# matthewygf/Tiresias

Measured on AMD Instinct MI355X. Metric: avg JCT + makespan on NSDI'19 Microsoft trace, 8×MI355X cluster, lower is better.
Workload: dtype bf16

## Files before the change

### csrc/bindings/ops.cpp

```cpp
#include <array>
#include <ATen/ATen.h>
#include <c10/hip/HIPStream.h>
#include <torch/library.h>

#include <functional>
#include <map>
#include <mutex>
#include <sstream>
#include <tuple>
#include <vector>

#include "tam/kernels.h"
#include "tam/launch.h"
#include "tam/gemm8p.h"

using at::Tensor;
using c10::optional;

namespace {

hipStream_t cur_stream(const Tensor& t) {
  return c10::hip::getCurrentHIPStream(t.device().index()).stream();
}

// ... 287 lines not shown
      t[0] = std::min(t[0], time_ms(s, [&] { run_mfma(a, a_kmajor, b, b_kmajor, M, N, K, es, allow_split, 0); }));
      for (const auto& c : cands) {
        const float ms = time_ms(s, [&] { run_p8(a, a_kmajor, b, b_kmajor, M, N, K, es, allow_split, c.first,
                                                 c.second); });
        if (ms < t[3]) { t[3] = ms; p8c = c; }
      }
      if (dma_ok)
        t[2] = std::min(t[2], time_ms(s, [&] { run_mfma(a, a_kmajor, b, b_kmajor, M, N, K, es, allow_split, 2); }));
      if (lib_ok && round == 0) {
        try {
          t[1] = time_ms(s, [&] { run_lib(a, a_kmajor, b, b_kmajor, scratch, mode, bias); });
        } catch (const std::exception&) {
          t[1] = 1e30f;
        }
      }
    }
    route = 0;
    if (t[2] < 0.95f * t[route]) route = 2;
    if (t[3] < 0.95f * t[route]) route = 3;
    if (t[1] < 0.95f * t[route]) route = 1;
    std::lock_guard<std::mutex> g(g_route_mu);
    g_route[key] = route;
    g_route_ms[key] = t;
    g_p8_cfg[key] = p8c;
  }
  if (route == 1 && !lib_ok) {
    std::lock_guard<std::mutex> g(g_route_mu);
    const auto t = g_route_ms[key];
    route = 0;
    if (dma_ok && t[2] < t[route]) route = 2;
    auto pc = g_p8_cfg.find(key);
    if (p8_ok && pc != g_p8_cfg.end() && pc->second.first > 0 && t[3] < t[route]) route = 3;
  }
  std::pair<int, int> p8c{-1, -1};
  if (route == 3) {
    std::lock_guard<std::mutex> g(g_route_mu);
    auto it = g_p8_cfg.find(key);
    if (it != g_p8_cfg.end()) p8c = it->second;
  }
  if (route == 1) run_lib(a, a_kmajor, b, b_kmajor, c, mode, bias);
  else if (route == 3) run_p8(a, a_kmajor, b, b_kmajor, M, N, K, ep, allow_split, p8c.first, p8c.second);
  else run_mfma(a, a_kmajor, b, b_kmajor, M, N, K, ep, allow_split, route);
}

void gemm_lib_policy_op(int64_t p) { g_lib_policy = (int)p; }

std::string gemm_routes_op() {
  std::lock_guard<std::mutex> g(g_route_mu);
  std::ostringstream o;
  for (const auto& kv : g_route) {
    const auto& k = kv.first;
    const auto t = g_route_ms[k];
    o << std::get<0>(k) << " " << std::get<1>(k) << " " << std::get<2>(k) << " "
      << (std::get<3>(k) ? "K" : "M") << (std::get<4>(k) ? "K" : "N") << " " << std::get<5>(k)
      << " " << std::get<6>(k) << " " << std::get<7>(k) << " "
      << (kv.second == 1 ? "lib" : kv.second == 2 ? "dma" : kv.second == 3 ? "p8" : "mfma") << " " << t[0]
      << " " << t[1] << " " << t[2] << " " << t[3];
    auto pc = g_p8_cfg.find(k);
    if (pc != g_p8_cfg.end()) o << " " << pc->second.first << " " << pc->second.second;
    o << "\n";
  }
  return o.str();
}

int64_t gemm_routes_load_op(const std::string& text) {
  std::istringstream in(text);
  std::string line;
  int64_t n = 0;
  std::lock_guard<std::mutex> g(g_route_mu);
  while (std::getline(in, line)) {
    std::istringstream ls(line);
    int64_t M, N, K, mode;
    std::string lay, rt;
    int f32, epi;
    std::array<float, 4> t{};
    if (!(ls >> M >> N >> K >> lay >> mode >> f32 >> epi >> rt >> t[0] >> t[1] >> t[2] >> t[3])) continue;
    if (lay.size() != 2 || M <= 0 || N <= 0 || K <= 0) continue;
    const int route = rt == "lib" ? 1 : rt == "dma" ? 2 : rt == "p8" ? 3 : rt == "mfma" ? 0 : -1;
    if (route < 0) continue;
    const GemmKey key{M, N, K, lay[0] == 'K', lay[1] == 'K', mode, (bool)f32, (bool)epi};
    if (g_route.count(key)) continue;
    int tile = -1, sp = -1;
    const bool has_cfg = (bool)(ls >> tile >> sp);
    const bool cfg_ok = has_cfg &&
                        (tile == 128 || tile == 256 || ((tile == 64 || tile == 65 || tile == 129) && lay[0] == 'K')) &&
                        sp >= (tile == 256 ? 0 : 1) && sp <= 16;
    if (route == 3 && !cfg_ok) continue;
    g_route[key] = route;
    g_route_ms[key] = t;
    if (cfg_ok) g_p8_cfg[key] = {tile, sp};
    ++n;
  }
  return n;
}

tam::ConvGeom geom(const Tensor& x, const Tensor& w, const Tensor& y, int64_t stride, int64_t pad,
                   int64_t dil) {
  tam::ConvGeom g;
  g.N = (int)x.size(0); g.H = (int)x.size(1); g.W = (int)x.size(2); g.C = (int)x.size(3);
  g.K = (int)w.size(0); g.R = (int)w.size(1); g.S = (int)w.size(2);
  g.P = (int)y.size(1); g.Q = (int)y.size(2);
  g.stride = (int)stride; g.pad = (int)pad; g.dil = (int)dil;
  TORCH_CHECK(w.size(3) == g.C, "tam.conv: weight C mismatch");
  TORCH_CHECK(y.size(0) == g.N && y.size(3) == g.K, "tam.conv: output shape mismatch");
  TORCH_CHECK(g.P == (g.H + 2 * g.pad - g.dil * (g.R - 1) - 1) / g.stride + 1 &&
                  g.Q == (g.W + 2 * g.pad - g.dil * (g.S - 1) - 1) / g.stride + 1,
              "tam.conv: output spatial size inconsistent with geometry");
  TORCH_CHECK(g.C % 8 == 0 && g.K % 8 == 0, "tam.conv: C and K must be multiples of 8");
  return g;
}

int64_t conv_fwd_op(const Tensor& x, const Tensor& w, const Tensor& y, int64_t stride, int64_t pad,
                    int64_t dil, const optional<Tensor>& bias, bool relu, const optional<Tensor>& stats) {
  check_bf16(x, "x"); check_bf16(w, "w"); check_bf16(y, "y");
  check_contig(x, "x"); check_contig(w, "w"); check_contig(y, "y");
  tam::ConvGeom g = geom(x, w, y, stride, pad, dil);
  tam::Epi ep;
  ep.c = y.data_ptr(); ep.ldc = g.K; ep.c_f32 = 0; ep.mode = 0;
  ep.bias = opt_ptr<const tam::bf16_t>(bias);
  ep.relu = relu;
  if (stats.has_value() && stats->defined()) {
    TORCH_CHECK(stats->is_cuda() && stats->scalar_type() == at::kDouble && stats->is_contiguous() &&
                stats->numel() == tam::BN_SHARDS * 2 * g.K,
                "tam.conv_fwd: stats must be a contiguous fp64 [BN_SHARDS * 2K] tensor");
    ep.stats = stats->data_ptr<double>();
  }
  const long wsf = tam::conv_fwd_split_ws(g);
  Tensor ws;
  if (wsf > 0) ws = at::empty({wsf}, x.options().dtype(at::kFloat));
  return tam::conv_fwd(bp(x), bp(w), g, ep, cur_stream(x), wsf > 0 ? ws.data_ptr<float>() : nullptr, wsf);
}

void conv_dgrad_op(const Tensor& dy, const Tensor& w, const Tensor& wt, const Tensor& dx,
                   int64_t stride, int64_t pad, int64_t dil, const optional<Tensor>& mask) {
  check_bf16(dy, "dy"); check_bf16(w, "w"); check_bf16(dx, "dx");
  check_contig(dy, "dy"); check_contig(w, "w"); check_contig(dx, "dx");
  tam::ConvGeom g = geom(dx, w, dy, stride, pad, dil);
  check_bf16(wt, "wt");
  TORCH_CHECK(wt.numel() == w.numel(), "tam.conv_dgrad: wt workspace size");
  tam::conv_weight_t(bp(w), bpm(wt), g, cur_stream(dy));
  tam::Epi ep;
  ep.c = dx.data_ptr(); ep.ldc = g.C; ep.c_f32 = 0; ep.mode = 0;
  if (mask.has_value() && mask->defined()) {
    check_bf16(*mask, "mask");
    TORCH_CHECK(mask->numel() == dx.numel(), "tam.conv_dgrad: mask size");
    ep.mask = bp(*mask); ep.ldm = g.C;
  }
  const long wsf = tam::conv_dgrad_split_ws(g);
  Tensor ws;
  if (wsf > 0) ws = at::empty({wsf}, dy.options().dtype(at::kFloat));
  tam::conv_dgrad(bp(dy), bp(w), bp(wt), g, ep, cur_stream(dy), wsf > 0 ? ws.data_ptr<float>() : nullptr, wsf);
}

void gemm_wgrad_grouped_op(at::TensorList dy, at::TensorList x, at::TensorList dw, at::TensorList db,
                           at::OptionalIntArrayRef modes) {
  TORCH_CHECK(dy.size() == x.size() && dy.size() == dw.size() && dy.size() == db.size(),
              "tam.gemm_wgrad_grouped: list sizes differ");
  TORCH_CHECK(!modes.has_value() || modes->size() == dy.size(), "tam.gemm_wgrad_grouped: modes size");
  if (dy.empty()) return;
  std::vector<tam::GGProblem> probs(dy.size());
  for (size_t i = 0; i < dy.size(); ++i) {
    const Tensor& a = dy[i];
    const Tensor& b = x[i];
    const Tensor& c = dw[i];
    check_bf16(a, "dy"); check_bf16(b, "x"); check_f32(c, "dw");
    check_contig(a, "dy"); check_contig(b, "x"); check_contig(c, "dw");
    TORCH_CHECK(a.dim() == 2 && b.dim() == 2 && c.dim() == 2 && a.size(0) == b.size(0) &&
                    c.size(0) == a.size(1) && c.size(1) == b.size(1),
                "tam.gemm_wgrad_grouped: shapes dy [T,M], x [T,N], dw [M,N] expected");
    TORCH_CHECK(a.device() == dy[0].device() && b.device() == a.device() && c.device() == a.device(),
                "tam.gemm_wgrad_grouped: all operands on one device");
    const int M = (int)a.size(1), N = (int)b.size(1), K = (int)a.size(0);
    TORCH_CHECK(tam::gemm_wgrad_grouped_ok(M, N, K, M, N),
                "tam.gemm_wgrad_grouped: problem ", i, " (", M, "x", N, "x", K,
                ") not eligible (K % 64, M/N >= 128 and % 8)");
    float* bias = nullptr;
    if (db[i].defined() && db[i].numel() > 0) {
      check_f32(db[i], "db");
      TORCH_CHECK(db[i].numel() == M && db[i].is_contiguous(), "tam.gemm_wgrad_grouped: db must be [M]");
      bias = db[i].data_ptr<float>();
    }
    const int mode = modes.has_value() ? (int)(*modes)[i] : 1;
    TORCH_CHECK(mode == 0 || mode == 1, "tam.gemm_wgrad_grouped: mode must be 0 (store) or 1 (accumulate)");
    probs[i] = tam::GGProblem{bp(a), bp(b), c.data_ptr<float>(), bias, M, N, K, M, N, mode};
  }
  tam::gemm_wgrad_grouped(probs.data(), (int)probs.size(), cur_stream(dy[0]));
}

void gemm_grouped_tile_op(int64_t t) { tam::gemm_grouped_tile((int)t); }

bool gemm_wgrad_grouped_ok_op(int64_t M, int64_t N, int64_t K) {
  return tam::gemm_wgrad_grouped_ok((int)M, (int)N, (int)K, M, N);
}

void conv_weight_t_batch_op(at::TensorList w, at::TensorList wt) {
  TORCH_CHECK(w.size() == wt.size(), "tam.conv_weight_t_batch: list sizes differ");
  if (w.empty()) return;
  hipStream_t st = cur_stream(w[0]);
  for (size_t base = 0; base < w.size(); base += tam::WT_MAX) {
    tam::WTBatch b{};
    b.n = (int)std::min<size_t>(tam::WT_MAX, w.size() - base);
    for (int i = 0; i < b.n; ++i) {
      const Tensor& a = w[base + i];
      const Tensor& t = wt[base + i];
      check_bf16(a, "w"); check_bf16(t, "wt"); check_contig(a, "w"); check_contig(t, "wt");
      TORCH_CHECK(a.dim() == 4 && t.numel() == a.numel(), "tam.conv_weight_t_batch: w must be [K,R,S,C]");
      b.e[i].w = bp(a); b.e[i].wt = bpm(t);
      b.e[i].K = (int)a.size(0); b.e[i].RS = (int)(a.size(1) * a.size(2)); b.e[i].C = (int)a.size(3);
    }
    tam::conv_weight_t_batch(b, st);
  }
}

int64_t conv_dgrad_pre_op(const Tensor& dy, const Tensor& w, const Tensor& wt, const Tensor& dx,
                          int64_t stride, int64_t pad, int64_t dil, const optional<Tensor>& mask,
                          const optional<Tensor>& stats, const optional<Tensor>& bnx,
                          const optional<Tensor>& bnmean, const optional<Tensor>& bnrstd) {
  check_bf16(dy, "dy"); check_bf16(w, "w"); check_bf16(dx, "dx"); check_bf16(wt, "wt");
  check_contig(dy, "dy"); check_contig(w, "w"); check_contig(dx, "dx"); check_contig(wt, "wt");
  TORCH_CHECK(wt.numel() == w.numel(), "tam.conv_dgrad_pre: wt size");
  tam::ConvGeom g = geom(dx, w, dy, stride, pad, dil);
  tam::Epi ep;
  ep.c = dx.data_ptr(); ep.ldc = g.C; ep.c_f32 = 0; ep.mode = 0;
  if (mask.has_value() && mask->defined()) {
    check_bf16(*mask, "mask");
    TORCH_CHECK(mask->numel() == dx.numel(), "tam.conv_dgrad_pre: mask size");
    ep.mask = bp(*mask); ep.ldm = g.C;
  }
  if (stats.has_value() && stats->defined()) {
    TORCH_CHECK(bnx.has_value() && bnmean.has_value() && bnrstd.has_value(),
                "tam.conv_dgrad_pre: stats needs bnx, bnmean, bnrstd");
    check_bf16(*bnx, "bnx"); check_f32(*bnmean, "bnmean"); check_f32(*bnrstd, "bnrstd");
    check_contig(*bnx, "bnx");
    TORCH_CHECK(stats->is_cuda() && stats->scalar_type() == at::kDouble && stats->is_contiguous() &&
                stats->numel() == tam::BN_SHARDS * 2 * g.C && bnx->numel() == dx.numel() && bnmean->numel() == g.C &&
                bnrstd->numel() == g.C, "tam.conv_dgrad_pre: BN-backward operand shapes");
    ep.stats = stats->data_ptr<double>();
    ep.bnx = bp(*bnx);
    ep.bnmean = bnmean->data_ptr<float>();
    ep.bnrstd = bnrstd->data_ptr<float>();
  }
  const long wsf = ep.bnx ? 0 : tam::conv_dgrad_split_ws(g);
  Tensor ws;
  if (wsf > 0) ws = at::empty({wsf}, dy.options().dtype(at::kFloat));
  return tam::conv_dgrad(bp(dy), bp(w), bp(wt), g, ep, cur_stream(dy), wsf > 0 ? ws.data_ptr<float>() : nullptr,
                         wsf);
}

std::tuple<Tensor, int64_t> conv_wgrad_deferred_op(const Tensor& dy, const Tensor& x, const Tensor& dw,
                                                   int64_t stride, int64_t pad, int64_t dil, int64_t mode,
                                                   const optional<Tensor>& dbias, bool patch) {
  check_bf16(dy, "dy"); check_bf16(x, "x"); check_f32(dw, "dw");
  check_contig(dy, "dy"); check_contig(x, "x"); check_contig(dw, "dw");
  TORCH_CHECK(dw.dim() == 4, "tam.conv_wgrad_deferred: dw must be [K,R,S,C]");
  tam::ConvGeom g = geom(x, dw, dy, stride, pad, dil);
  tam::Epi ep;
  ep.c = dw.data_ptr(); ep.ldc = g.R * g.S * g.C; ep.c_f32 = 1; ep.mode = (int)mode;
  float* db = nullptr;
  if (dbias.has_value() && dbias->defined()) {
    check_f32(*dbias, "dbias");
    TORCH_CHECK(dbias->numel() == g.K && dbias->is_contiguous(), "tam.conv_wgrad_deferred: dbias size");
    db = dbias->data_ptr<float>();
  }
  const long wsf = tam::conv_wgrad_split_ws(g);
  Tensor wsl = at::empty({wsf > 0 ? wsf : 0}, dy.options().dtype(at::kFloat));
  int sp = 0;
  const int fused = tam::conv_wgrad(bp(dy), bp(x), g, ep, cur_stream(dy), db, patch,
                                    wsf > 0 ? wsl.data_ptr<float>() : nullptr, wsf, &sp);
  if (db && !fused) {
    const long R = (long)g.N * g.P * g.Q;
    Tensor ws = at::empty({g.K % 8 == 0 ? (int64_t)tam::COLSUM_MAX_BLOCKS * g.K : 1}, dy.options().dtype(at::kFloat));
    tam::colsum(bp(dy), db, ws.data_ptr<float>(), R, g.K, cur_stream(dy));
  }
  return {sp > 0 ? wsl : at::empty({0}, dy.options().dtype(at::kFloat)), (int64_t)sp};
}

void wgrad_slab_reduce_many_op(at::TensorList slabs, at::IntArrayRef sp, at::TensorList dw, at::IntArrayRef mode) {
  const size_t n = slabs.size();
  TORCH_CHECK(sp.size() == n && dw.size() == n && mode.size() == n, "tam.wgrad_slab_reduce_many: list sizes");
  if (n == 0) return;
  std::vector<const float*> ws(n);
  std::vector<float*> out(n);
  std::vector<int> s(n), md(n);
  std::vector<long> mn(n);
  for (size_t i = 0; i < n; ++i) {
    check_f32(slabs[i], "slab"); check_f32(dw[i], "dw");
    TORCH_CHECK(dw[i].is_contiguous() && dw[i].numel() % 4 == 0 && sp[i] > 0 &&
                    slabs[i].numel() >= sp[i] * dw[i].numel(),
                "tam.wgrad_slab_reduce_many: entry ", i);
    ws[i] = slabs[i].data_ptr<float>();
    out[i] = dw[i].data_ptr<float>();
    s[i] = (int)sp[i];
    md[i] = (int)mode[i];
    mn[i] = (long)dw[i].numel();
  }
  tam::wgrad_slab_reduce_many(ws.data(), s.data(), mn.data(), out.data(), md.data(), (int)n, cur_stream(dw[0]));
}

void conv_wgrad_op(const Tensor& dy, const Tensor& x, const Tensor& dw, int64_t stride, int64_t pad,
                   int64_t dil, int64_t mode, const optional<Tensor>& dbias, bool patch) {
  check_bf16(dy, "dy"); check_bf16(x, "x"); check_f32(dw, "dw");
  check_contig(dy, "dy"); check_contig(x, "x"); check_contig(dw, "dw");
  TORCH_CHECK(dw.dim() == 4, "tam.conv_wgrad: dw must be [K,R,S,C]");
  tam::ConvGeom g = geom(x, dw, dy, stride, pad, dil);
  tam::Epi ep;
  ep.c = dw.data_ptr(); ep.ldc = g.R * g.S * g.C; ep.c_f32 = 1; ep.mode = (int)mode;
  float* db = nullptr;
  if (dbias.has_value() && dbias->defined()) {
    check_f32(*dbias, "dbias");
    TORCH_CHECK(dbias->numel() == g.K && dbias->is_contiguous(), "tam.conv_wgrad: dbias size");
    db = dbias->data_ptr<float>();
  }
  const long wsf = tam::conv_wgrad_split_ws(g);
  Tensor wsl;
  if (wsf > 0) wsl = at::empty({wsf}, dy.options().dtype(at::kFloat));
  const int fused = tam::conv_wgrad(bp(dy), bp(x), g, ep, cur_stream(dy), db, patch,
                                    wsf > 0 ? wsl.data_ptr<float>() : nullptr, wsf);
  if (db && !fused) {
    const long R = (long)g.N * g.P * g.Q;
    Tensor ws = at::empty({g.K % 8 == 0 ? (int64_t)tam::COLSUM_MAX_BLOCKS * g.K : 1}, dy.options().dtype(at::kFloat));
    tam::colsum(bp(dy), db, ws.data_ptr<float>(), R, g.K, cur_stream(dy));
  }
}

static double* bn_sums(const optional<Tensor>& sums, const Tensor& x, int64_t C, Tensor& tmp,
                       const char* what) {
  if (sums.has_value() && sums->defined()) {
    TORCH_CHECK(sums->is_cuda() && sums->scalar_type() == at::kDouble && sums->is_contiguous() &&
                sums->numel() == tam::BN_SHARDS * 2 * C, what,
                ": sums must be a contiguous fp64 [BN_SHARDS * 2C] tensor");
    return sums->data_ptr<double>();
  }
  tmp = at::zeros({tam::BN_SHARDS * 2 * C}, x.options().dtype(at::kDouble));
  return tmp.data_ptr<double>();
}

void bn_forward_op(const Tensor& x, const optional<Tensor>& res, const Tensor& y, const Tensor& gamma,
                   const Tensor& beta, const optional<Tensor>& run_mean,
                   const optional<Tensor>& run_var, const Tensor& save_mean,
// ... 196 lines not shown
  TORCH_CHECK(tm_b <= 0 || ids.numel() % tm_b == 0, "tam.embedding: tm_b must divide the ids");
  const tam::bf16_t* pp = nullptr;
  int64_t prow = 0;
  if (pos.has_value() && pos->defined()) {
    check_bf16(*pos, "pos"); check_contig(*pos, "pos");
    TORCH_CHECK(pos->dim() == 2 && pos->size(1) == D, "tam.embedding: pos must be [S][D]");
    prow = pos->size(0);
    TORCH_CHECK(prow > 0 && (tm_b > 0 ? ids.numel() / tm_b == prow : ids.numel() % prow == 0),
                "tam.embedding: pos rows must equal the sequence length");
    pp = bp(*pos);
  }
  tam::embedding_forward(bp(table), ids.data_ptr<int64_t>(), bpm(out), ids.numel(), (int)D,
                         (float)scale, cur_stream(table), table.size(0), tm_b, pp, prow);
}
void embedding_backward_op(const Tensor& dout, const Tensor& ids, const Tensor& gtable, double scale, int64_t tm_b) {
  check_bf16(dout, "dout"); check_f32(gtable, "gtable"); check_contig(dout, "dout");
  TORCH_CHECK(ids.scalar_type() == at::kLong && ids.is_contiguous() && gtable.dim() == 2 &&
                  dout.numel() == ids.numel() * gtable.size(1), "tam.embedding_backward: shapes");
  TORCH_CHECK(tm_b <= 0 || ids.numel() % tm_b == 0, "tam.embedding_backward: tm_b must divide the ids");
  tam::embedding_backward(bp(dout), ids.data_ptr<int64_t>(), gtable.data_ptr<float>(), ids.numel(),
                          (int)gtable.size(1), (float)scale, cur_stream(dout), gtable.size(0), tm_b);
}

void conv_dma_policy_op(int64_t p) { tam::conv_dma_policy((int)p); }
void conv_halo_policy_op(int64_t p) { tam::conv_halo_policy((int)p); }
void colsum_policy_op(int64_t p) { tam::colsum_policy((int)p); }
void attn_short_policy_op(int64_t p) { tam::attn_short_policy((int)p); }
void conv_wgrad_c64_policy_op(int64_t p) { tam::conv_wgrad_c64_policy((int)p); }
void conv_wgrad_order_op(int64_t p) { tam::conv_wgrad_order((int)p); }
void conv_stem_policy_op(int64_t p) { tam::conv_stem_policy((int)p); }
void conv_wgrad_slab_policy_op(int64_t p) { tam::conv_wgrad_slab_policy((int)p); }
void conv_wgrad_force_op(int64_t bm, int64_t bn, int64_t splits, int64_t noatomic) {
  tam::conv_wgrad_force((int)bm, (int)bn, (int)splits, (int)noatomic);
}
int g_dma_policy = 1;
TAM_KNOB(g_dma_policy)
void gemm_dma_policy_op(int64_t p, int64_t cfg) {
  g_dma_policy = (int)p;
  tam::gemm_dma_policy(p == 2 ? 1 : 0, (int)cfg);
}

void gemm8p_policy_op(int64_t mode, int64_t tile) { tam::gemm8p_policy((int)mode, (int)tile); }
void gemm_pw_policy_op(int64_t on) { tam::gemm_pw_policy((int)on); }

std::string policy_names_op() {
  std::string out;
  for (const auto& k : tam::knob_registry()) {
    if (!out.empty()) out += ",";
    out += k.name;
  }
  return out;
}
std::vector<int64_t> policy_state_op() {
  std::vector<int64_t> v;
  for (const auto& k : tam::knob_registry()) v.push_back(*k.p);
  return v;
}
void policy_load_op(std::vector<int64_t> v) {
  auto& reg = tam::knob_registry();
  TORCH_CHECK(v.size() == reg.size(), "policy_load: ", v.size(), " values for ", reg.size(), " knobs");
  for (size_t i = 0; i < reg.size(); ++i) *reg[i].p = (int)v[i];
}
void gemm8p_group_op(int64_t g) { tam::gemm8p_group((int)g); }
void gemm8p_slab_force_op(int64_t sp) { tam::gemm8p_slab_force((int)sp); }
void gemm8p_sk_force_op(int64_t on) { g_sk_force = on != 0; }
void conv_split_policy_op(int64_t p) { tam::conv_split_policy((int)p); }
void optim_grid_op(int64_t b) { tam::optim_grid((int)b); }
void optim_variant_op(int64_t v) { tam::optim_variant((int)v); }
void gemm_skinny_policy_op(int64_t on, int64_t sp, int64_t nst) {
  tam::gemm_skinny_policy((int)on, (int)sp, (int)nst);
}

void gemm_force_op(int64_t cfg, int64_t splits) {
  tam::gemm_force((int)cfg, (int)splits);
  g_forced = cfg >= 0 || splits >= 1;
}

void colsum_op(const Tensor& x, const Tensor& out) {
  check_bf16(x, "x"); check_f32(out, "out"); check_contig(x, "x");
  const int64_t C = x.size(-1);
  Tensor ws = at::empty({C % 8 == 0 ? (int64_t)tam::COLSUM_MAX_BLOCKS * C : 1},
                        x.options().dtype(at::kFloat));
  tam::colsum(bp(x), out.data_ptr<float>(), ws.data_ptr<float>(), x.numel() / C, (int)C,
              cur_stream(x));
}
void relu_backward_op(const Tensor& dy, const Tensor& y, const Tensor& dx) {
  check_bf16(dy, "dy"); check_bf16(y, "y"); check_bf16(dx, "dx");
  tam::relu_backward(bp(dy), bp(y), bpm(dx), dy.numel(), cur_stream(dy));
}
void sum_scale_op(const Tensor& x, const Tensor& out, double scale) {
  check_f32(x, "x"); check_f32(out, "out"); check_contig(x, "x");
  TORCH_CHECK(out.numel() >= 1, "tam.sum_scale: out");
  tam::sum_scale(x.data_ptr<float>(), x.numel(), out.data_ptr<float>(), (float)scale, cur_stream(x));
}
static std::pair<int64_t, int64_t> row_view(const Tensor& t, const char* what) {
  TORCH_CHECK(t.is_cuda() && t.scalar_type() == at::kBFloat16 && t.dim() >= 1 && t.stride(-1) == 1,
              "tam.rows_sum: ", what, " must be a bf16 CUDA tensor with unit last stride");
  const int64_t C = t.size(-1);
  int64_t ld = t.dim() >= 2 ? t.stride(-2) : C;
  for (int64_t d = t.dim() - 2; d >= 1; --d)
    TORCH_CHECK(t.size(d) == 1 || t.size(d - 1) == 1 || t.stride(d - 1) == t.stride(d) * t.size(d),
                "tam.rows_sum: ", what, " leading dims do not collapse to one row pitch");
  TORCH_CHECK(C % 8 == 0 && ld % 8 == 0 && (((uintptr_t)t.data_ptr()) & 15) == 0,
              "tam.rows_sum: ", what, " needs C % 8 == 0 and 16-B aligned rows");
  return {C, ld};
}
void rows_sum_op(at::TensorList outs, at::TensorList ins, at::IntArrayRef n_in) {
  TORCH_CHECK(!outs.empty() && outs.size() <= 4 && outs.size() == n_in.size(), "tam.rows_sum: 1-4 jobs");
  const int64_t R = outs[0].numel() / outs[0].size(-1);
  tam::RowJobs jb{};
  size_t q = 0;
  for (size_t j = 0; j < outs.size(); ++j) {
    auto [C, ld] = row_view(outs[j], "out");
    TORCH_CHECK(outs[j].numel() / C == R, "tam.rows_sum: every job needs the same row count");
    TORCH_CHECK(n_in[j] >= 1 && n_in[j] <= 4 && q + n_in[j] <= ins.size(), "tam.rows_sum: n_in");
    tam::RowJob& r = jb.job[j];
    r.out = bpm(outs[j]); r.ld_out = ld; r.C = (int)C; r.n_in = (int)n_in[j];
    for (int k = 0; k < r.n_in; ++k, ++q) {
      auto [Ci, ldi] = row_view(ins[q], "in");
      TORCH_CHECK(Ci == C && ins[q].numel() / Ci == R, "tam.rows_sum: input shape");
      r.in[k] = bp(ins[q]); r.ld_in[k] = ldi;
    }
  }
  TORCH_CHECK(q == ins.size(), "tam.rows_sum: unused inputs");
  tam::rows_sum(jb, (int)outs.size(), R, cur_stream(outs[0]));
}
void zero_op(const Tensor& t) {
  TORCH_CHECK(t.is_cuda() && t.is_contiguous(), "tam.zero_: contiguous CUDA tensor");
  tam::zero_async(t.data_ptr(), t.numel() * t.element_size(), cur_stream(t));
}
void add_op(const Tensor& a, const Tensor& b, const Tensor& y) {
  check_bf16(a, "a"); check_bf16(b, "b"); check_bf16(y, "y");
  TORCH_CHECK(a.numel() % 8 == 0, "tam.add: numel % 8");
  tam::add_bf16(bp(a), bp(b), bpm(y), a.numel(), cur_stream(a));
}
void cast_op(const Tensor& x, const Tensor& y) {
  check_f32(x, "x"); check_bf16(y, "y");
  tam::cast_f32_bf16(x.data_ptr<float>(), bpm(y), x.numel(), cur_stream(x));
}

static const unsigned* guard_ptr(const optional<Tensor>& guard, const Tensor& like) {
  if (!(guard.has_value() && guard->defined())) return nullptr;
  TORCH_CHECK(guard->scalar_type() == at::kInt && guard->numel() >= 2 && guard->device() == like.device(),
              "tam: guard must be an int32 [2] tensor on the parameters' device");
  return (const unsigned*)guard->data_ptr<int>();
}
static const float* clip_ptr(const optional<Tensor>& clip, const Tensor& like) {
  if (!(clip.has_value() && clip->defined())) return nullptr;
  TORCH_CHECK(clip->scalar_type() == at::kFloat && clip->numel() >= 4 && clip->is_contiguous() &&
                  clip->device() == like.device() && (((uintptr_t)clip->data_ptr()) & 15) == 0,
              "tam: clip must be a 16-B aligned float32 [4] tensor on the parameters' device");
  return clip->data_ptr<float>();
}
void sgd_op(const Tensor& w, const Tensor& g, const Tensor& mom, const Tensor& wb, double lr,
            double momentum, double wd, double gscale, bool nesterov, bool zero_grad,
            const optional<Tensor>& guard, int64_t zero_from, int64_t wd_until,
            const optional<Tensor>& clip) {
  check_f32(w, "w"); check_f32(g, "g"); check_f32(mom, "mom"); check_bf16(wb, "wb");
  TORCH_CHECK(w.numel() % 4 == 0 && g.numel() == w.numel() && mom.numel() == w.numel() &&
                  wb.numel() == w.numel(),
              "tam.sgd: sizes");
  TORCH_CHECK(zero_from % 4 == 0 && (wd_until < 0 || wd_until % 4 == 0), "tam.sgd: region bounds % 4");
  tam::sgd_step(w.data_ptr<float>(), g.data_ptr<float>(), mom.data_ptr<float>(), bpm(wb), w.numel(),
                (float)lr, (float)momentum, (float)wd, (float)gscale, nesterov, zero_grad,
                cur_stream(w), guard_ptr(guard, w), (long)zero_from, (long)wd_until, clip_ptr(clip, w));
}
void adam_op(const Tensor& w, const Tensor& g, const Tensor& m, const Tensor& v, const Tensor& wb,
             double lr, double b1, double b2, double eps, double wd, int64_t step, double gscale,
             bool zero_grad, const optional<Tensor>& guard, int64_t zero_from, int64_t wd_until,
             const optional<Tensor>& clip) {
  check_f32(w, "w"); check_f32(g, "g"); check_f32(m, "m"); check_f32(v, "v"); check_bf16(wb, "wb");
  TORCH_CHECK(w.numel() % 4 == 0, "tam.adam: numel % 4");
  TORCH_CHECK(zero_from % 4 == 0 && (wd_until < 0 || wd_until % 4 == 0), "tam.adam: region bounds % 4");
  tam::adam_step(w.data_ptr<float>(), g.data_ptr<float>(), m.data_ptr<float>(), v.data_ptr<float>(),
                 bpm(wb), w.numel(), (float)lr, (float)b1, (float)b2, (float)eps, (float)wd,
                 (int)step, (float)gscale, zero_grad, cur_stream(w), guard_ptr(guard, w), (long)zero_from,
                 (long)wd_until, clip_ptr(clip, w));
}
void grad_sumsq_op(const Tensor& g, const Tensor& partials) {
  check_f32(g, "g"); check_contig(g, "g"); check_dev(partials, "partials"); check_contig(partials, "partials");
  TORCH_CHECK(partials.scalar_type() == at::kDouble && partials.device() == g.device(),
              "tam.grad_sumsq: partials must be float64 on the gradient's device");
  TORCH_CHECK(g.numel() % 4 == 0 && (((uintptr_t)g.data_ptr()) & 15) == 0,
              "tam.grad_sumsq: numel % 4 and a 16-B aligned gradient");
  const int blocks = tam::grad_sumsq_blocks(g.numel());
  TORCH_CHECK(partials.numel() >= blocks && partials.numel() <= (1 << 20), "tam.grad_sumsq: partials holds ",
              partials.numel(), " slots, the grid needs ", blocks);
  tam::grad_sumsq(g.data_ptr<float>(), g.numel(), partials.data_ptr<double>(), (int)partials.numel(),
                  cur_stream(g));
}
void grad_clip_finalize_op(const Tensor& partials, double max_norm, double gscale, const Tensor& clip) {
  check_dev(partials, "partials"); check_contig(partials, "partials"); check_f32(clip, "clip");
  TORCH_CHECK(partials.scalar_type() == at::kDouble && partials.numel() >= 1 && partials.numel() <= (1 << 20),
              "tam.grad_clip_finalize: partials must be a float64 tensor of the grad_sumsq slots");
  TORCH_CHECK(max_norm > 0.0, "tam.grad_clip_finalize: max_norm must be > 0");
  tam::grad_clip_finalize(partials.data_ptr<double>(), (int)partials.numel(), (float)max_norm, (float)gscale,
                          const_cast<float*>(clip_ptr(clip, partials)), cur_stream(partials));
}
int64_t grad_sumsq_blocks_op(int64_t n) { return tam::grad_sumsq_blocks((long)n); }
void lstm_guard_step_op(const Tensor& err) {
  TORCH_CHECK(err.is_cuda() && err.scalar_type() == at::kInt && err.numel() >= 2,
              "tam.lstm_guard_step: err must be an int32 [2] GPU tensor");
  tam::lstm_guard_step((unsigned*)err.data_ptr<int>(), cur_stream(err));
}

void check_attn_view(const Tensor& t, const char* name) {
  check_bf16(t, name);
  TORCH_CHECK(t.dim() == 4 && t.size(3) == 64 && t.stride(3) == 1 && t.stride(2) == 64,
              "tam.attn: ", name, " must be a [B,S,H,64] view with packed heads");
  TORCH_CHECK(t.stride(1) % 8 == 0 && t.stride(0) % 8 == 0, "tam.attn: ", name, " stride alignment");
}
void attn_forward_op(const Tensor& q, const Tensor& k, const Tensor& v, const Tensor& o,
                     const Tensor& lse, bool causal, double scale, const optional<Tensor>& kv_len) {
  check_attn_view(q, "q"); check_attn_view(k, "k"); check_attn_view(v, "v"); check_attn_view(o, "o");
  TORCH_CHECK(k.stride(1) == v.stride(1), "tam.attn: k/v token strides differ");
  check_f32(lse, "lse");
  const int B = (int)q.size(0), Sq = (int)q.size(1), H = (int)q.size(2), Sk = (int)k.size(1);
  TORCH_CHECK(lse.numel() == (int64_t)B * H * Sq, "tam.attn: lse size");
  TORCH_CHECK(k.stride(0) == v.stride(0), "tam.attn: k/v batch strides differ");
  tam::attn_forward(bp(q), bp(k), bp(v), bpm(o), lse.data_ptr<float>(), B, H, Sq, Sk, q.stride(1),
                    k.stride(1), o.stride(1), q.stride(0), k.stride(0), o.stride(0), causal, (float)scale,
                    opt_ptr<const int>(kv_len), cur_stream(q));
}
void attn_backward_op(const Tensor& q, const Tensor& k, const Tensor& v, const Tensor& o,
                      const Tensor& dout, const Tensor& lse, const Tensor& dq, const Tensor& dk,
                      const Tensor& dv, const Tensor& dq_acc, const Tensor& delta, bool causal,
                      double scale, const optional<Tensor>& kv_len) {
  check_attn_view(q, "q"); check_attn_view(k, "k"); check_attn_view(v, "v"); check_attn_view(o, "o");
  check_attn_view(dout, "dout"); check_attn_view(dq, "dq"); check_attn_view(dk, "dk");
  check_attn_view(dv, "dv");
  TORCH_CHECK(dout.stride(1) == o.stride(1) && dout.stride(0) == o.stride(0), "tam.attn_bwd: dout must match o layout");
  TORCH_CHECK(dq.stride(1) == q.stride(1) && dk.stride(1) == k.stride(1) && dv.stride(1) == k.stride(1) &&
                  dq.stride(0) == q.stride(0) && dk.stride(0) == k.stride(0) && dv.stride(0) == k.stride(0) &&
                  v.stride(0) == k.stride(0) && v.stride(1) == k.stride(1),
              "tam.attn_bwd: grads must match input layouts");
  const int B = (int)q.size(0), Sq = (int)q.size(1), H = (int)q.size(2), Sk = (int)k.size(1);
  check_f32(dq_acc, "dq_acc"); check_f32(delta, "delta");
  TORCH_CHECK(dq_acc.numel() >= (int64_t)B * Sq * H * 64 && delta.numel() >= (int64_t)B * H * Sq,
              "tam.attn_bwd: workspace sizes");
  tam::attn_backward(bp(q), bp(k), bp(v), bp(o), bp(dout), lse.data_ptr<float>(), bpm(dq), bpm(dk),
                     bpm(dv), dq_acc.data_ptr<float>(), delta.data_ptr<float>(), B, H, Sq, Sk,
                     q.stride(1), k.stride(1), o.stride(1), q.stride(0), k.stride(0), o.stride(0), causal,
                     (float)scale,
                     opt_ptr<const int>(kv_len), cur_stream(q));
}

void lstm_fwd_op(const Tensor& gates, const optional<Tensor>& c_prev, const Tensor& c_out,
                 const Tensor& h_out, const optional<Tensor>& h_f32, const Tensor& act) {
  check_f32(gates, "gates"); check_f32(c_out, "c_out"); check_bf16(h_out, "h_out"); check_f32(act, "act");
  const int B = (int)gates.size(0), Hd = (int)(gates.size(1) / 4);
  tam::lstm_cell_forward(gates.data_ptr<float>(), opt_ptr<const float>(c_prev), c_out.data_ptr<float>(),
                         bpm(h_out), opt_ptr<float>(h_f32), act.data_ptr<float>(), B, Hd,
                         cur_stream(gates));
}
void lstm_step_fwd_op(const Tensor& gx, const Tensor& w_hh, const optional<Tensor>& h_prev,
                      const optional<Tensor>& c_prev, const Tensor& c_out, const Tensor& h_out,
                      const Tensor& act) {
  check_f32(gx, "gx"); check_bf16(w_hh, "w_hh"); check_f32(c_out, "c_out"); check_bf16(h_out, "h_out");
  check_f32(act, "act");
  const int64_t B = gx.size(0), Hd = w_hh.size(1);
  TORCH_CHECK(gx.dim() == 2 && gx.size(1) == 4 * Hd && gx.stride(1) == 1 && gx.stride(0) == 4 * Hd,
              "tam.lstm_step_forward: gx must be contiguous [B][4*Hd]");
  TORCH_CHECK(w_hh.is_contiguous() && w_hh.size(0) == 4 * Hd, "tam.lstm_step_forward: w_hh [4Hd][Hd]");
  TORCH_CHECK(B % 16 == 0 && Hd % 256 == 0, "tam.lstm_step_forward: needs B % 16 == 0, Hd % 256 == 0");
  TORCH_CHECK(c_out.numel() == B * Hd && h_out.numel() == B * Hd && act.numel() == 5 * B * Hd &&
              c_out.is_contiguous() && h_out.is_contiguous() && act.is_contiguous(),
              "tam.lstm_step_forward: output shapes");
  if (h_prev.has_value() && h_prev->defined()) {
    check_bf16(*h_prev, "h_prev");
    TORCH_CHECK(h_prev->is_contiguous() && h_prev->numel() == B * Hd, "tam.lstm_step_forward: h_prev");
  }
  if (c_prev.has_value() && c_prev->defined()) {
    check_f32(*c_prev, "c_prev");
    TORCH_CHECK(c_prev->is_contiguous() && c_prev->numel() == B * Hd, "tam.lstm_step_forward: c_prev");
  }
  tam::lstm_step_forward(gx.data_ptr<float>(), bp(w_hh), opt_ptr<const tam::bf16_t>(h_prev),
                         opt_ptr<const float>(c_prev), c_out.data_ptr<float>(), bpm(h_out),
                         act.data_ptr<float>(), (int)B, (int)Hd, cur_stream(gx));
}

static void check_sync(const Tensor& sync, int64_t B) {
  TORCH_CHECK(sync.is_cuda() && sync.scalar_type() == at::kInt && sync.is_contiguous() &&
              sync.numel() >= 32 * (4 * (B / 16) + 1),
              "tam.lstm_seq: sync must be a contiguous int32 tensor of >= 32 * (4 * B/16 + 1) elements");
}
static tam::PLOpts pl_opts(const optional<Tensor>& job_err, int64_t grids, int64_t rsv, bool zeroed) {
  tam::PLOpts o;
  o.grids = (int)grids;
  o.rsv = (int)rsv;
  o.zeroed = zeroed ? 1 : 0;
  if (job_err.has_value() && job_err->defined()) {
    TORCH_CHECK(job_err->is_cuda() && job_err->scalar_type() == at::kInt && job_err->numel() >= 2,
                "tam.lstm_seq: job_err must be an int32 [2] GPU tensor");
    o.job_err = (unsigned*)job_err->data_ptr<int>();
  }
  return o;
}
bool lstm_seq_fwd_op(const Tensor& gx, const Tensor& w_hh, const Tensor& hs, const Tensor& cs,
                     const Tensor& act, bool reverse, const Tensor& sync, const optional<Tensor>& job_err,
                     int64_t grids, int64_t rsv, bool zeroed) {
  check_f32(gx, "gx"); check_bf16(w_hh, "w_hh"); check_bf16(hs, "hs"); check_f32(cs, "cs");
  check_f32(act, "act");
  TORCH_CHECK(hs.dim() == 3 && hs.is_contiguous(), "tam.lstm_seq_forward: hs [T][B][Hd]");
  const int64_t T = hs.size(0), B = hs.size(1), Hd = hs.size(2);
  check_sync(sync, B);
  TORCH_CHECK(w_hh.is_contiguous() && w_hh.size(0) == 4 * Hd && w_hh.size(1) == Hd,
              "tam.lstm_seq_forward: w_hh [4Hd][Hd]");
  TORCH_CHECK(gx.is_contiguous() && gx.numel() == T * B * 4 * Hd, "tam.lstm_seq_forward: gx [T][B][4Hd]");
  TORCH_CHECK(cs.is_contiguous() && cs.numel() == T * B * Hd && act.is_contiguous() &&
              act.numel() == T * B * 5 * Hd, "tam.lstm_seq_forward: cs / act shapes");
  int* sp = sync.data_ptr<int>();
  return tam::lstm_seq_forward(gx.data_ptr<float>(), bp(w_hh), bpm(hs), cs.data_ptr<float>(),
                               act.data_ptr<float>(), (int)T, (int)B, (int)Hd, reverse ? 1 : 0,
                               (unsigned*)sp, cur_stream(gx), pl_opts(job_err, grids, rsv, zeroed));
}
bool lstm_seq_bwd_op(const Tensor& act, const Tensor& cs, const Tensor& dH, const Tensor& w_hh,
                     const Tensor& dG, bool reverse, const Tensor& sync, const optional<Tensor>& job_err,
                     int64_t grids, int64_t rsv, bool zeroed) {
  check_f32(act, "act"); check_f32(cs, "cs"); check_bf16(w_hh, "w_hh");
  TORCH_CHECK(dH.is_cuda() && (dH.scalar_type() == at::kFloat || dH.scalar_type() == at::kBFloat16),
              "tam.lstm_seq_backward: dH must be an f32 or bf16 CUDA tensor");
  const int dh_bf16 = dH.scalar_type() == at::kBFloat16 ? 1 : 0;
  check_bf16(dG, "dG");
  TORCH_CHECK(cs.dim() == 3 && cs.is_contiguous(), "tam.lstm_seq_backward: cs [T][B][Hd]");
  const int64_t T = cs.size(0), B = cs.size(1), Hd = cs.size(2);
  check_sync(sync, B);
  TORCH_CHECK(w_hh.is_contiguous() && w_hh.size(0) == 4 * Hd && w_hh.size(1) == Hd,
              "tam.lstm_seq_backward: w_hh [4Hd][Hd]");
  TORCH_CHECK(dH.dim() == 3 && dH.size(0) == T && dH.size(1) == B && dH.size(2) == Hd && dH.stride(2) == 1 &&
                  dH.stride(1) >= Hd && dH.stride(0) == B * dH.stride(1),
              "tam.lstm_seq_backward: dH [T][B][Hd] with unit column stride and uniform row pitch");
  TORCH_CHECK(act.is_contiguous() && act.numel() == T * B * 5 * Hd && dG.is_contiguous() &&
                  dG.numel() == T * B * 4 * Hd,
              "tam.lstm_seq_backward: act / dG shapes");
  int* sp = sync.data_ptr<int>();
  return tam::lstm_seq_backward(act.data_ptr<float>(), cs.data_ptr<float>(), (const float*)dH.data_ptr(),
                                bp(w_hh), bpm(dG), (int)T, (int)B, (int)Hd, reverse ? 1 : 0, (unsigned*)sp,
                                dh_bf16, (int)dH.stride(1), cur_stream(act), pl_opts(job_err, grids, rsv, zeroed));
}

void lstm_seq_policy_op(int64_t ch) { tam::lstm_seq_policy((int)ch); }
void lstm_seq_shards_op(int64_t ns) { tam::lstm_seq_shards((int)ns); }
void lstm_seq_residency_op(int64_t grids, int64_t rsv) { tam::lstm_seq_residency((int)grids, (int)rsv); }
int64_t lstm_persist_timeouts_op(bool reset) { return tam::lstm_persist_timeouts(reset); }
void lstm_seq_spin_limit_op(int64_t polls) { tam::lstm_seq_spin_limit(polls); }

void lstm_bwd_op(const Tensor& act, const optional<Tensor>& c_prev, const optional<Tensor>& dh,
                 const optional<Tensor>& dc_next, const optional<Tensor>& dgates,
                 const optional<Tensor>& dc_prev, const optional<Tensor>& dgates_bf16) {
  check_f32(act, "act");
  const int B = (int)act.size(0), Hd = (int)(act.size(1) / 5);
  tam::lstm_cell_backward(act.data_ptr<float>(), opt_ptr<const float>(c_prev), nullptr,
                          opt_ptr<const float>(dh), opt_ptr<const float>(dc_next),
                          opt_ptr<float>(dgates), opt_ptr<float>(dc_prev),
                          opt_ptr<tam::bf16_t>(dgates_bf16), B, Hd, c10::hip::getCurrentHIPStream(act.device().index()).stream());
}

}

TORCH_LIBRARY(tam, m) {
  m.def("gemm(Tensor a, bool a_kmajor, Tensor b, bool b_kmajor, Tensor(a!) c, int mode, Tensor? bias, bool relu, Tensor? mask, float alpha, bool allow_split, Tensor(b!)? colsum=None) -> ()", &gemm_op);
  m.def("conv_fwd(Tensor x, Tensor w, Tensor(a!) y, int stride, int pad, int dil, Tensor? bias, bool relu, Tensor(b!)? stats=None) -> int", &conv_fwd_op);
  m.def("conv_dgrad(Tensor dy, Tensor w, Tensor(a!) wt, Tensor(b!) dx, int stride, int pad, int dil, Tensor? mask) -> ()", &conv_dgrad_op);
  m.def("conv_weight_t_batch(Tensor[] w, Tensor(a!)[] wt) -> ()", &conv_weight_t_batch_op);
  m.def("gemm_wgrad_grouped(Tensor[] dy, Tensor[] x, Tensor(a!)[] dw, Tensor(b!)[] db, int[]? modes=None) -> ()", &gemm_wgrad_grouped_op);
  m.def("gemm_wgrad_grouped_ok(int M, int N, int K) -> bool", &gemm_wgrad_grouped_ok_op);
  m.def("gemm_grouped_tile(int tile) -> ()", &gemm_grouped_tile_op);
  m.def("conv_dgrad_pre(Tensor dy, Tensor w, Tensor wt, Tensor(a!) dx, int stride, int pad, int dil, Tensor? mask, Tensor(b!)? stats=None, Tensor? bnx=None, Tensor? bnmean=None, Tensor? bnrstd=None) -> int", &conv_dgrad_pre_op);
  m.def("conv_wgrad(Tensor dy, Tensor x, Tensor(a!) dw, int stride, int pad, int dil, int mode, Tensor(b!)? dbias=None, bool patch=True) -> ()", &conv_wgrad_op);
  m.def("conv_wgrad_deferred(Tensor dy, Tensor x, Tensor(a!) dw, int stride, int pad, int dil, int mode, Tensor(b!)? dbias, bool patch) -> (Tensor, int)", &conv_wgrad_deferred_op);
  m.def("wgrad_slab_reduce_many(Tensor[] slabs, int[] sp, Tensor(a!)[] dw, int[] mode) -> ()", &wgrad_slab_reduce_many_op);
  m.def("bn_forward(Tensor x, Tensor? res, Tensor(a!) y, Tensor gamma, Tensor beta, Tensor(b!)? run_mean, Tensor(c!)? run_var, Tensor(d!) save_mean, Tensor(e!) save_rstd, float eps, float momentum, bool relu, Tensor(f!)? sums=None, bool sums_ready=False, Tensor(g!)? ymask=None) -> ()", &bn_forward_op);
  m.def("bn_backward(Tensor dy, Tensor? y, Tensor x, Tensor mean, Tensor rstd, Tensor gamma, Tensor(a!) dx, Tensor(b!)? dres, Tensor(c!)? dgamma, Tensor(d!)? dbeta, bool relu, Tensor? addend=None, Tensor(e!)? sums=None, bool sums_ready=False, Tensor? ymask=None) -> ()", &bn_backward_op);
  m.def("ln_forward(Tensor x, Tensor g, Tensor b, Tensor(a!) y, Tensor(b!) mean, Tensor(c!) rstd, float eps, Tensor? addend=None, Tensor(d!)? sum_out=None) -> ()", &ln_forward_op);
  m.def("ln_backward(Tensor dy, Tensor x, Tensor g, Tensor mean, Tensor rstd, Tensor(a!) dx, Tensor(b!) dg, Tensor(c!) db, Tensor? addend=None) -> ()", &ln_backward_op);
  m.def("ln_backward_split(Tensor dy, Tensor x, Tensor g, Tensor mean, Tensor rstd, Tensor(a!) dx, Tensor(b!) ws, Tensor? addend=None) -> int", &ln_backward_split_op);
  m.def("col_reduce_acc(Tensor part, int nblk, int W, Tensor(a!) out0, Tensor(b!) out1, int split) -> ()", &col_reduce_acc_op);
  m.def("col_reduce_acc_batch(Tensor[] parts, int[] nblk, Tensor(a!)[] out0, Tensor(b!)[] out1) -> ()", &col_reduce_acc_batch_op);
  m.def("maxpool_forward(Tensor x, Tensor(a!) y, Tensor(b!) idx, int R, int S, int stride, int pad) -> ()", &maxpool_forward_op);
  m.def("maxpool_backward(Tensor dy, Tensor idx, Tensor(a!) dx, int R, int S, int stride, int pad) -> ()", &maxpool_backward_op);
  m.def("maxpool_k3s2_policy(int policy) -> ()", &maxpool_k3s2_policy_op);
  m.def("avgpool_forward(Tensor x, Tensor(a!) y) -> ()", &avgpool_forward_op);
  m.def("avgpool_backward(Tensor dy, Tensor(a!) dx) -> ()", &avgpool_backward_op);
  m.def("softmax_xent(Tensor logits, Tensor labels, Tensor(a!)? dlogits, Tensor(b!) loss_rows, float smoothing, float grad_scale, int ignore_index, int tm_b=0) -> ()", &softmax_xent_op);
  m.def("embedding_forward(Tensor table, Tensor ids, Tensor(a!) out, float scale, int tm_b=0, Tensor? pos=None) -> ()", &embedding_forward_op);
  m.def("embedding_backward(Tensor dout, Tensor ids, Tensor(a!) gtable, float scale, int tm_b=0) -> ()", &embedding_backward_op);
  m.def("sum_scale(Tensor x, Tensor(a!) out, float scale) -> ()", &sum_scale_op);
  m.def("rows_sum(Tensor[] outs, Tensor[] ins, int[] n_in) -> ()", &rows_sum_op);
  m.def("zero_(Tensor(a!) t) -> ()", &zero_op);
  m.def("colsum(Tensor x, Tensor(a!) out) -> ()", &colsum_op);
  m.def("gemm_force(int cfg, int splits) -> ()", &gemm_force_op);
  m.def("gemm8p_policy(int mode, int tile) -> ()", &gemm8p_policy_op);
  m.def("gemm_pw_policy(int on) -> ()", &gemm_pw_policy_op);
  m.def("policy_names() -> str", &policy_names_op);
  m.def("policy_state() -> int[]", &policy_state_op);
  m.def("policy_load(int[] v) -> ()", &policy_load_op);
  m.def("gemm8p_group(int g) -> ()", &gemm8p_group_op);
  m.def("gemm8p_slab_force(int sp) -> ()", &gemm8p_slab_force_op);
  m.def("gemm_skinny_policy(int on, int force_splits, int nst) -> ()", &gemm_skinny_policy_op);
  m.def("gemm8p_sk_force(int on) -> ()", &gemm8p_sk_force_op);
  m.def("conv_split_policy(int p) -> ()", &conv_split_policy_op);
  m.def("optim_variant(int v) -> ()", &optim_variant_op);
  m.def("optim_grid(int blocks) -> ()", &optim_grid_op);
  m.def("gemm_lib_policy(int policy) -> ()", &gemm_lib_policy_op);
  m.def("conv_dma_policy(int policy) -> ()", &conv_dma_policy_op);
  m.def("conv_wgrad_force(int bm, int bn, int splits, int noatomic=0) -> ()", &conv_wgrad_force_op);
  m.def("conv_wgrad_c64_policy(int policy) -> ()", &conv_wgrad_c64_policy_op);
  m.def("conv_wgrad_order(int flat) -> ()", &conv_wgrad_order_op);
  m.def("conv_stem_policy(int policy) -> ()", &conv_stem_policy_op);
  m.def("conv_wgrad_slab_policy(int policy) -> ()", &conv_wgrad_slab_policy_op);
  m.def("conv_halo_policy(int policy) -> ()", &conv_halo_policy_op);
  m.def("colsum_policy(int policy) -> ()", &colsum_policy_op);
  m.def("attn_short_policy(int policy) -> ()", &attn_short_policy_op);
  m.def("gemm_dma_policy(int policy, int cfg) -> ()", &gemm_dma_policy_op);
  m.def("gemm_routes() -> str", &gemm_routes_op);
  m.def("relu_backward(Tensor dy, Tensor y, Tensor(a!) dx) -> ()", &relu_backward_op);
  m.def("add(Tensor a, Tensor b, Tensor(a!) y) -> ()", &add_op);
  m.def("cast_f32_bf16(Tensor x, Tensor(a!) y) -> ()", &cast_op);
  m.def("sgd_step(Tensor(a!) w, Tensor(b!) g, Tensor(c!) mom, Tensor(d!) wb, float lr, float momentum, float wd, float gscale, bool nesterov, bool zero_grad, Tensor? guard=None, int zero_from=0, int wd_until=-1, Tensor? clip=None) -> ()", &sgd_op);
  m.def("adam_step(Tensor(a!) w, Tensor(b!) g, Tensor(c!) m, Tensor(d!) v, Tensor(e!) wb, float lr, float b1, float b2, float eps, float wd, int step, float gscale, bool zero_grad, Tensor? guard=None, int zero_from=0, int wd_until=-1, Tensor? clip=None) -> ()", &adam_op);
  m.def("grad_sumsq(Tensor g, Tensor(a!) partials) -> ()", &grad_sumsq_op);
  m.def("grad_clip_finalize(Tensor partials, float max_norm, float gscale, Tensor(a!) clip) -> ()", &grad_clip_finalize_op);
  m.def("grad_sumsq_blocks(int n) -> int", &grad_sumsq_blocks_op);
  m.def("lstm_guard_step(Tensor(a!) err) -> ()", &lstm_guard_step_op);
  m.def("attn_forward(Tensor q, Tensor k, Tensor v, Tensor(a!) o, Tensor(b!) lse, bool causal, float scale, Tensor? kv_len) -> ()", &attn_forward_op);
  m.def("attn_backward(Tensor q, Tensor k, Tensor v, Tensor o, Tensor dout, Tensor lse, Tensor(a!) dq, Tensor(b!) dk, Tensor(c!) dv, Tensor(d!) dq_acc, Tensor(e!) delta, bool causal, float scale, Tensor? kv_len) -> ()", &attn_backward_op);
  m.def("lstm_step_forward(Tensor gx, Tensor w_hh, Tensor? h_prev, Tensor? c_prev, Tensor(a!) c_out, Tensor(b!) h_out, Tensor(c!) act) -> ()", &lstm_step_fwd_op);
  m.def("lstm_seq_forward(Tensor gx, Tensor w_hh, Tensor(a!) hs, Tensor(b!) cs, Tensor(c!) act, bool reverse, Tensor(d!) sync, Tensor(e!)? job_err=None, int grids=-1, int reserved_cus=0, bool zeroed=False) -> bool", &lstm_seq_fwd_op);
  m.def("lstm_seq_backward(Tensor act, Tensor cs, Tensor dH, Tensor w_hh, Tensor(a!) dG, bool reverse, Tensor(b!) sync, Tensor(c!)? job_err=None, int grids=-1, int reserved_cus=0, bool zeroed=False) -> bool", &lstm_seq_bwd_op);
  m.def("lstm_seq_policy(int ch) -> ()", &lstm_seq_policy_op);
  m.def("lstm_seq_shards(int ns) -> ()", &lstm_seq_shards_op);
  m.def("gemm_routes_load(str text) -> int", &gemm_routes_load_op);
  m.def("lstm_seq_residency(int grids, int reserved_cus) -> ()", &lstm_seq_residency_op);
  m.def("lstm_persist_timeouts(bool reset) -> int", &lstm_persist_timeouts_op);
  m.def("lstm_seq_spin_limit(int polls) -> ()", &lstm_seq_spin_limit_op);
  m.def("lstm_cell_forward(Tensor gates, Tensor? c_prev, Tensor(a!) c_out, Tensor(b!) h_out, Tensor(c!)? h_f32, Tensor(d!) act) -> ()", &lstm_fwd_op);
  m.def("lstm_cell_backward(Tensor act, Tensor? c_prev, Tensor? dh, Tensor? dc_next, Tensor(a!)? dgates, Tensor(b!)? dc_prev, Tensor(c!)? dgates_bf16) -> ()", &lstm_bwd_op);
}
```

### csrc/include/tam/gemm8p.h

```cpp
#pragma once
#include "tam/igemm.h"

namespace tam {

constexpr int P8_BK = 64;

typedef __attribute__((address_space(3))) void p8_lds_t;

struct P8Args {
  const bf16_t* A;
  long lda;
  const bf16_t* B;
  long ldb;
  int M, N, K;
  int kps;
  int group = 4;
};

template <int BM, int BN, int WNW>
struct P8Geo {
  static constexpr int NW = 2 * WNW, THREADS = 64 * NW;
  static constexpr int WTM = BM / 2, WTN = BN / WNW;
  static constexpr int QM = WTM / 2, QN = WTN / 2;
  static constexpr int FI = QM / 16, FJ = QN / 16;
  static constexpr int AROWS = BM / 2, BCOLS = BN / 2;
  static constexpr int AHALF = AROWS * P8_BK * 2, BHALF = BCOLS * P8_BK * 2;
  static constexpr int STAGE = 2 * AHALF + 2 * BHALF;
  static constexpr int LDS = 2 * STAGE;
  static constexpr int DA = AHALF / (THREADS * 16), DB = BHALF / (THREADS * 16);
  static_assert(DA >= 1 && DB >= 1 && AHALF == THREADS * 16 * DA && BHALF == THREADS * 16 * DB,
                "whole DMA instructions per half");
  static constexpr int INFLIGHT = DA + 2 * DB;
};

template <int N>
__device__ __forceinline__ void p8_vmcnt() {
  static_assert(N >= 0 && N <= 8, "p8_vmcnt: 0..8");
  if constexpr (N == 0) asm volatile("s_waitcnt vmcnt(0)" ::: "memory");
  else if constexpr (N == 1) asm volatile("s_waitcnt vmcnt(1)" ::: "memory");
  else if constexpr (N == 2) asm volatile("s_waitcnt vmcnt(2)" ::: "memory");
  else if constexpr (N == 3) asm volatile("s_waitcnt vmcnt(3)" ::: "memory");
  else if constexpr (N == 4) asm volatile("s_waitcnt vmcnt(4)" ::: "memory");
  else if constexpr (N == 5) asm volatile("s_waitcnt vmcnt(5)" ::: "memory");
  else if constexpr (N == 6) asm volatile("s_waitcnt vmcnt(6)" ::: "memory");
  else if constexpr (N == 7) asm volatile("s_waitcnt vmcnt(7)" ::: "memory");
  else asm volatile("s_waitcnt vmcnt(8)" ::: "memory");
}

template <int Q>
__device__ __forceinline__ int p8_row(int lr, int h) {
  return (lr / Q) * (2 * Q) + h * Q + (lr % Q);
}

template <int Q, int EXT, int NW, bool KMAJ, int D = 2>
__device__ __forceinline__ void p8_issue(const bf16_t* __restrict__ base, long ld, int extent, int o0,
                                         int k0, char* half, int h, int wid, int lane) {
#pragma unroll
  for (int j = 0; j < D; ++j) {
    const int g = j * NW + wid;
    if constexpr (KMAJ) {
      const int lr = g * 8 + (lane >> 3);
      const int c = (lane & 7) ^ ((lr >> 1) & 7);
      int r = o0 + p8_row<Q>(lr, h);
      r = r < extent ? r : extent - 1;
      const bf16_t* src = base + (long)r * ld + k0 + c * 8;
      __builtin_amdgcn_global_load_lds((const void*)src, (p8_lds_t*)(half + g * 1024), 16, 0, 0);
    } else {
      constexpr int GPR = EXT / 8, RPG = 64 / GPR;
      const int kr = g * RPG + lane / GPR;
      const int gran = (lane % GPR) ^ (mnmaj_swz<EXT>(kr) >> 1);
      int col = o0 + p8_row<Q>(gran * 8, h);
      col = col + 8 <= extent ? col : extent - 8;
      const bf16_t* src = base + (long)(k0 + kr) * ld + col;
      __builtin_amdgcn_global_load_lds((const void*)src, (p8_lds_t*)(half + g * 1024), 16, 0, 0);
    }
  }
}

template <bool KMAJ, int EXT>
__device__ __forceinline__ s16x8_t p8_frag(const char* half, int lane, int lbase, int kk) {
  if constexpr (KMAJ) return read_frag_k(half, lane, lbase, kk);
  else return read_frag_mn<EXT>(half, lane, 32 * kk, lbase);
}

__device__ __forceinline__ void p8_barrier() {
  asm volatile("" ::: "memory");
  __builtin_amdgcn_s_barrier();
  asm volatile("" ::: "memory");
}

template <int I0, int J0, bool FINE = false, int FI, int FJ, int TI, int TJ>
__device__ __forceinline__ void p8_mfma(f32x4_t (&acc)[TI][TJ], const s16x8_t (&fa)[FI][2],
                                        const s16x8_t (&fb)[FJ][2]) {
  if constexpr (!FINE) {
    asm volatile("s_waitcnt lgkmcnt(0)" ::: "memory");
    __builtin_amdgcn_sched_barrier(0);
  }
  __builtin_amdgcn_s_setprio(1);
#pragma unroll
  for (int kk = 0; kk < 2; ++kk)
#pragma unroll
    for (int i = 0; i < FI; ++i)
#pragma unroll
      for (int j = 0; j < FJ; ++j)
        acc[I0 + i][J0 + j] = __builtin_amdgcn_mfma_f32_16x16x32_bf16(
            __builtin_bit_cast(bf16x8_t, fa[i][kk]), __builtin_bit_cast(bf16x8_t, fb[j][kk]),
            acc[I0 + i][J0 + j], 0, 0, 0);
  __builtin_amdgcn_s_setprio(0);
  __builtin_amdgcn_sched_barrier(0);
}

template <int BM, int BN, int WNW, int TI, int TJ, int J0 = 0, int NJ = TJ>
__device__ __forceinline__ void p8_epilogue(const P8Args& a, const Epi& ep, f32x4_t (&acc)[TI][TJ], char* smem,
                                            const int m0, const int n0, const int kz, const int wid,
                                            const int lane) {
  using G = P8Geo<BM, BN, WNW>;
  const int wm = wid / WNW, wn = wid % WNW;

  const bool add_bias = ep.bias != nullptr && kz == 0;
  static_assert(J0 >= 0 && NJ >= 1 && J0 + NJ <= TJ, "fragment column range");
  const int rbase = m0 + wm * G::WTM, cbase = n0 + wn * G::WTN + 16 * J0;
  constexpr int WTN = 16 * NJ;
  float bv[TJ];
#pragma unroll
  for (int j = 0; j < TJ; ++j) {
    if (j < J0 || j >= J0 + NJ) continue;
    const int col = cbase + 16 * (j - J0) + (lane & 15);
    bv[j] = (add_bias && col < a.N) ? bf2f(ep.bias[col]) : 0.f;
  }
  const bool mask16 = ep.mask == nullptr || ((ep.ldm & 7) == 0 && (((uintptr_t)ep.mask) & 15) == 0);
  if (!ep.c_f32 && mask16 && (ep.ldc & 7) == 0 && (((uintptr_t)ep.c) & 15) == 0) {
    constexpr int LDW = WTN + 8, CPR = WTN / 8;
    bf16_t* slab = (bf16_t*)(smem + wid * (32 * LDW * 2));
#pragma unroll
    for (int h = 0; h < TI / 2; ++h) {
#pragma unroll
      for (int ii = 0; ii < 2; ++ii)
#pragma unroll
        for (int j = J0; j < J0 + NJ; ++j)
#pragma unroll
          for (int r = 0; r < 4; ++r) {
            float v = acc[2 * h + ii][j][r] * ep.alpha + bv[j];
            if (ep.relu) v = fmaxf(v, 0.f);
            slab[(16 * ii + 4 * (lane >> 4) + r) * LDW + 16 * (j - J0) + (lane & 15)] = f2bf(v);
          }
      asm volatile("s_waitcnt lgkmcnt(0)" ::: "memory");
#pragma unroll
      for (int u = 0; u < 32 * CPR / 64; ++u) {
        const int idx = u * 64 + lane, lr = idx / CPR, ch = idx % CPR;
        const int row = rbase + 32 * h + lr, col = cbase + ch * 8;
        if (row >= a.M || col >= a.N) continue;
        bf16_t* dst = (bf16_t*)ep.c + (long)row * ep.ldc + col;
        const bf16_t* src = slab + lr * LDW + ch * 8;
        if (col + 8 <= a.N) {
          uint4 v = *(const uint4*)src;
          if (ep.mask) {
            const uint4 mk = *(const uint4*)(ep.mask + (long)row * ep.ldm + col);
            const uint32_t* mw = (const uint32_t*)&mk;
            uint32_t* vw = (uint32_t*)&v;
#pragma unroll
            for (int e = 0; e < 4; ++e) {
              const uint32_t m2 = mw[e];
              const bool lo = (m2 & 0x8000u) == 0 && (m2 & 0x7fffu) != 0;
              const bool hi = (m2 & 0x80000000u) == 0 && (m2 & 0x7fff0000u) != 0;
              vw[e] &= (lo ? 0x0000ffffu : 0u) | (hi ? 0xffff0000u : 0u);
            }
          }
          if (ep.mode == 1) {
            uint32_t* vw = (uint32_t*)&v;
            const uint4 o = *(const uint4*)dst;
            const uint32_t* ow = (const uint32_t*)&o;
#pragma unroll
            for (int e = 0; e < 4; ++e)
              vw[e] = pack_bf2(bf2f((bf16_t)(vw[e] & 0xffff)) + bf2f((bf16_t)(ow[e] & 0xffff)),
                               bf2f((bf16_t)(vw[e] >> 16)) + bf2f((bf16_t)(ow[e] >> 16)));
          }
          *(uint4*)dst = v;
        } else {
          for (int e = 0; e < 8 && col + e < a.N; ++e) {
            float v = bf2f(src[e]);
            if (ep.mask && bf2f(ep.mask[(long)row * ep.ldm + col + e]) <= 0.f) v = 0.f;
            if (ep.mode == 1) v += bf2f(dst[e]);
            dst[e] = f2bf(v);
          }
        }
      }
      asm volatile("s_waitcnt lgkmcnt(0)" ::: "memory");
    }
    return;
  }
  if (ep.c_f32 && ep.mode != 2 && !ep.mask && (ep.ldc & 3) == 0 && (((uintptr_t)ep.c) & 15) == 0 &&
      (ep.mode != 3 || (ep.zstride & 3) == 0)) {
    constexpr int LDF = WTN + 4, CPR = WTN / 4;
    float* slab = (float*)(smem + wid * (32 * LDF * 4));
    float* cz = (float*)ep.c + (ep.mode == 3 ? kz * ep.zstride : 0);
#pragma unroll
    for (int h = 0; h < TI / 2; ++h) {
#pragma unroll
      for (int ii = 0; ii < 2; ++ii)
#pragma unroll
        for (int j = J0; j < J0 + NJ; ++j)
#pragma unroll
          for (int r = 0; r < 4; ++r) {
            float v = acc[2 * h + ii][j][r] * ep.alpha + bv[j];
            if (ep.relu) v = fmaxf(v, 0.f);
            slab[(16 * ii + 4 * (lane >> 4) + r) * LDF + 16 * (j - J0) + (lane & 15)] = v;
          }
      asm volatile("s_waitcnt lgkmcnt(0)" ::: "memory");
#pragma unroll
      for (int u = 0; u < 32 * CPR / 64; ++u) {
        const int idx = u * 64 + lane, lr = idx / CPR, ch = idx % CPR;
        const int row = rbase + 32 * h + lr, col = cbase + ch * 4;
        if (row >= a.M || col >= a.N) continue;
        float* dst = cz + (long)row * ep.ldc + col;
        const float* src = slab + lr * LDF + ch * 4;
        if (col + 4 <= a.N) {
          float4 v = *(const float4*)src;
          if (ep.mode == 1) {
            const float4 o = *(const float4*)dst;
            v.x += o.x; v.y += o.y; v.z += o.z; v.w += o.w;
          }
          *(float4*)dst = v;
        } else {
          for (int e = 0; e < 4 && col + e < a.N; ++e) dst[e] = ep.mode == 1 ? dst[e] + src[e] : src[e];
        }
      }
      asm volatile("s_waitcnt lgkmcnt(0)" ::: "memory");
    }
    return;
  }
#pragma unroll
  for (int j = J0; j < J0 + NJ; ++j) {
    const int col = cbase + 16 * (j - J0) + (lane & 15);
    if (col >= a.N) continue;
#pragma unroll
    for (int i = 0; i < TI; ++i) {
#pragma unroll
      for (int r = 0; r < 4; ++r) {
        const int row = rbase + 16 * i + 4 * (lane >> 4) + r;
        if (row >= a.M) continue;
        float v = acc[i][j][r] * ep.alpha + bv[j];
        if (ep.relu) v = fmaxf(v, 0.f);
        if (ep.mask && bf2f(ep.mask[(long)row * ep.ldm + col]) <= 0.f) v = 0.f;
        const long off = (long)row * ep.ldc + col;
        if (ep.c_f32) {
          float* c = (float*)ep.c;
          if (ep.mode == 3) c[off + kz * ep.zstride] = v;
          else if (ep.mode == 2) atomicAdd(c + off, v);
          else if (ep.mode == 1) c[off] += v;
          else c[off] = v;
        } else {
          bf16_t* c = (bf16_t*)ep.c;
          if (ep.mode == 1) v += bf2f(c[off]);
          c[off] = f2bf(v);
        }
      }
    }
  }
}

template <int BM, int BN>
__device__ __forceinline__ void p8_tile_origin(const P8Args& a, const int bid, int& m0, int& n0) {
  const int tiles_m = (a.M + BM - 1) / BM, tiles_n = (a.N + BN - 1) / BN;
  const int GROUP = a.group;
  const int per_group = GROUP * tiles_n;
  const int grp = bid / per_group;
  const int first_m = grp * GROUP;
  const int gsize = min(tiles_m - first_m, GROUP);
  m0 = (first_m + (bid % per_group) % gsize) * BM;
  n0 = ((bid % per_group) / gsize) * BN;
}

template <int BM, int BN, int WNW, bool AK, bool BK, int KS = 1>
__device__ __forceinline__ void gemm8p_body(const P8Args& a, const Epi& ep, const int bid, const int kz,
                                            const int kt_lo = -1, const int kt_hi = -1) {
  using G = P8Geo<BM, BN, WNW>;
  constexpr bool FINE = true;
  constexpr int FI = G::FI, FJ = G::FJ, TI = 2 * FI, TJ = 2 * FJ;
  __shared__ __attribute__((aligned(1024))) char smem_all[G::LDS * KS];
  const int grp = KS == 1 ? 0 : __builtin_amdgcn_readfirstlane((int)threadIdx.x / G::THREADS);
  const int tid = KS == 1 ? (int)threadIdx.x : (int)threadIdx.x % G::THREADS, lane = tid & 63, wid = tid >> 6;
  const int wm = wid / WNW, wn = wid % WNW;
  char* smem = smem_all + grp * G::LDS;

  int m0, n0;
  p8_tile_origin<BM, BN>(a, bid, m0, n0);

  const int ktiles = a.K / P8_BK;
  int kt0 = kt_lo >= 0 ? kt_lo : kz * a.kps;
  int kt1 = kt_lo >= 0 ? kt_hi : min(ktiles, kt0 + a.kps);
  if constexpr (KS > 1) {
    const int part = (kt1 - kt0) / KS;
    kt0 += grp * part;
    kt1 = kt0 + part;
  }
  const int nk = kt1 - kt0;

  f32x4_t acc[TI][TJ];
#pragma unroll
  for (int i = 0; i < TI; ++i)
#pragma unroll
    for (int j = 0; j < TJ; ++j) acc[i][j] = f32x4_t{0.f, 0.f, 0.f, 0.f};

  auto aptr = [&](int t, int h) { return smem + (t & 1) * G::STAGE + h * G::AHALF; };
  auto bptr = [&](int t, int h) { return smem + (t & 1) * G::STAGE + 2 * G::AHALF + h * G::BHALF; };
  auto issA = [&](int t, int h) {
    p8_issue<G::QM, G::AROWS, G::NW, AK, G::DA>(a.A, a.lda, a.M, m0, (kt0 + t) * P8_BK, aptr(t, h), h, wid, lane);
  };
  auto issB = [&](int t, int h) {
    p8_issue<G::QN, G::BCOLS, G::NW, BK, G::DB>(a.B, a.ldb, a.N, n0, (kt0 + t) * P8_BK, bptr(t, h), h, wid, lane);
  };

  if (nk > 0) {
    issA(0, 0); issB(0, 0); issB(0, 1); issA(0, 1);
    if (nk > 1) {
      issA(1, 0); issB(1, 0); issB(1, 1);
      p8_vmcnt<G::INFLIGHT>();
    } else {
      asm volatile("s_waitcnt vmcnt(0)" ::: "memory");
    }
    p8_barrier();

    const int arow = wm * G::QM, bcol = wn * G::QN;
    s16x8_t fa[FI][2], fb0[FJ][2], fb1[FJ][2];
    for (int t = 0; t < nk; ++t) {
      const char* AL = aptr(t, 0);
      const char* AH = aptr(t, 1);
      const char* BL = bptr(t, 0);
      const char* BH = bptr(t, 1);
      const bool n1 = t + 1 < nk, n2 = t + 2 < nk;
#pragma unroll
      for (int kk = 0; kk < 2; ++kk)
#pragma unroll
        for (int j = 0; j < FJ; ++j) fb0[j][kk] = p8_frag<BK, G::BCOLS>(BL, lane, bcol + 16 * j, kk);
      __builtin_amdgcn_sched_barrier(0);
#pragma unroll
      for (int kk = 0; kk < 2; ++kk)
#pragma unroll
        for (int i = 0; i < FI; ++i) fa[i][kk] = p8_frag<AK, G::AROWS>(AL, lane, arow + 16 * i, kk);
      if (n1) issA(t + 1, 1);
      p8_mfma<0, 0, FINE>(acc, fa, fb0);
      p8_barrier();
#pragma unroll
      for (int kk = 0; kk < 2; ++kk)
#pragma unroll
        for (int j = 0; j < FJ; ++j) fb1[j][kk] = p8_frag<BK, G::BCOLS>(BH, lane, bcol + 16 * j, kk);
      p8_mfma<0, FJ, FINE>(acc, fa, fb1);
      p8_barrier();
#pragma unroll
      for (int kk = 0; kk < 2; ++kk)
#pragma unroll
        for (int i = 0; i < FI; ++i) fa[i][kk] = p8_frag<AK, G::AROWS>(AH, lane, arow + 16 * i, kk);
      if (n2) issA(t + 2, 0);
      p8_mfma<FI, FJ, FINE>(acc, fa, fb1);
      p8_barrier();
      if (n2) {
        issB(t + 2, 0);
        issB(t + 2, 1);
        p8_vmcnt<G::INFLIGHT>();
      } else {
        asm volatile("s_waitcnt vmcnt(0)" ::: "memory");
      }
      p8_mfma<FI, 0, FINE>(acc, fa, fb0);
      p8_barrier();
    }
  }
  __syncthreads();
  if constexpr (KS > 1) {
    static_assert(KS == 2 && TJ % 2 == 0, "two K groups, two fragment-column halves");
    constexpr int JH = TJ / 2;
    static_assert(G::NW * TI * JH * 4 * 64 * 4 <= G::LDS, "half a partial tile fits a group's LDS");
    float* mine = (float*)(smem_all + grp * G::LDS);
    const float* other = (const float*)(smem_all + (grp ^ 1) * G::LDS);
#pragma unroll
    for (int i = 0; i < TI; ++i)
#pragma unroll
      for (int j = 0; j < JH; ++j)
#pragma unroll
        for (int r = 0; r < 4; ++r)
          mine[(((wid * TI + i) * JH + j) * 4 + r) * 64 + lane] = grp == 0 ? acc[i][JH + j][r] : acc[i][j][r];
    __syncthreads();
#pragma unroll
    for (int i = 0; i < TI; ++i)
#pragma unroll
      for (int j = 0; j < JH; ++j)
#pragma unroll
        for (int r = 0; r < 4; ++r) {
          const float o = other[(((wid * TI + i) * JH + j) * 4 + r) * 64 + lane];
          if (grp == 0) acc[i][j][r] += o;
          else acc[i][JH + j][r] += o;
        }
    __syncthreads();
    if (grp == 0) p8_epilogue<BM, BN, WNW, TI, TJ, 0, JH>(a, ep, acc, smem_all, m0, n0, kz, wid, lane);
    else p8_epilogue<BM, BN, WNW, TI, TJ, JH, JH>(a, ep, acc, smem_all + G::LDS, m0, n0, kz, wid, lane);
    return;
  }
  p8_epilogue<BM, BN, WNW>(a, ep, acc, smem_all, m0, n0, kz, wid, lane);
}

template <int BM, int BN, int WNW, bool AK, bool BK>
__global__ void __launch_bounds__(2 * 128 * WNW, 1) gemm8p_ks2_kernel(P8Args a, Epi ep) {
  gemm8p_body<BM, BN, WNW, AK, BK, 2>(a, ep, xcd_remap(blockIdx.x, gridDim.x), blockIdx.z);
}

template <int BM, int BN, int WNW, bool AK, bool BK>
void p8_launch_ks2(const P8Args& g, const Epi& ep, dim3 grid, hipStream_t s) {
  hipLaunchKernelGGL((gemm8p_ks2_kernel<BM, BN, WNW, AK, BK>), grid, dim3(2 * P8Geo<BM, BN, WNW>::THREADS), 0, s,
                     g, ep);
}

template <int BM, int BN, int WNW, bool AK, bool BK>
__global__ void __launch_bounds__(128 * WNW, (BM == 256 ? 1 : BM == 128 ? 2 : 3))
gemm8p_kernel(P8Args a, Epi ep) {
  gemm8p_body<BM, BN, WNW, AK, BK>(a, ep, xcd_remap(blockIdx.x, gridDim.x), blockIdx.z);
}

template <int BM, int BN, int WNW, bool AK, bool BK>
void p8_launch_one(const P8Args& g, const Epi& ep, dim3 grid, hipStream_t s) {
  hipLaunchKernelGGL((gemm8p_kernel<BM, BN, WNW, AK, BK>), grid, dim3(P8Geo<BM, BN, WNW>::THREADS), 0, s,
                     g, ep);
}

#define TAM_P8_VARIANTS(X)                                                                     \
  X(256, 256, 4, true, true) X(256, 256, 4, true, false)                                       \
  X(256, 256, 4, false, true) X(256, 256, 4, false, false)                                     \
  X(128, 128, 2, true, true) X(128, 128, 2, true, false)                                       \
  X(128, 128, 2, false, true) X(128, 128, 2, false, false)                                     \
  X(64, 128, 2, true, true) X(64, 128, 2, true, false)
#define TAM_P8_EXTERN(BM, BN, W, AK, BK) \
  extern template void p8_launch_one<BM, BN, W, AK, BK>(const P8Args&, const Epi&, dim3, hipStream_t);
#define TAM_P8_KS2_VARIANTS(X) \
  X(64, 128, 2, true, true) X(64, 128, 2, true, false) X(128, 128, 2, true, true) X(128, 128, 2, true, false)
#define TAM_P8_KS2_EXTERN(BM, BN, W, AK, BK) \
  extern template void p8_launch_ks2<BM, BN, W, AK, BK>(const P8Args&, const Epi&, dim3, hipStream_t);
#define TAM_P8_KS2_INST(BM, BN, W, AK, BK) \
  template void p8_launch_ks2<BM, BN, W, AK, BK>(const P8Args&, const Epi&, dim3, hipStream_t);
#define TAM_P8_INST(BM, BN, W, AK, BK) \
  template void p8_launch_one<BM, BN, W, AK, BK>(const P8Args&, const Epi&, dim3, hipStream_t);

inline bool gemm8p_ok(bool ak, bool bk, int M, int N, int K, long lda, long ldb) {
  if (K % P8_BK != 0 || K < P8_BK || M < 128 || N < 128) return false;
  if (lda % 8 != 0 || ldb % 8 != 0) return false;
  if (!ak && M % 8 != 0) return false;
  if (!bk && N % 8 != 0) return false;
  return true;
}

inline bool gemm8p_tile_ok(int tile, bool ak) { return (tile != 64 && tile != 65 && tile != 129) || ak; }
void launch_gemm8p(const bf16_t* A, long lda, bool ak, const bf16_t* B, long ldb, bool bk, int M,
                   int N, int K, const Epi& ep, int splits, hipStream_t s, int tile = 256);
void gemm8p_splitk(const bf16_t* A, long lda, bool ak, const bf16_t* B, long ldb, bool bk, int M,
                   int N, int K, const Epi& ep, int splits, float* ws, hipStream_t s, int tile = 256);
int gemm8p_slab_splits(int M, int N, int K, int tile = 256);
void gemm8p_slab_force(int sp);
int gemm8p_tile(int M, int N, int K);
bool gemm8p_sk_ok(bool ak, bool bk, int M, int N, int K, long lda, long ldb);
long gemm8p_sk_ws_floats(int M, int N, int K);
void gemm8p_streamk(const bf16_t* A, long lda, bool ak, const bf16_t* B, long ldb, bool bk, int M, int N, int K,
                    const Epi& ep, float* ws, hipStream_t s);

}
```

### csrc/include/tam/kernels.h

```cpp
#pragma once
#include <hip/hip_runtime.h>
#include <stdint.h>
#include "tam/common.h"

namespace tam {

constexpr int BN_MAX_BLOCKS = 512;
constexpr int LN_MAX_BLOCKS = 512;
constexpr int COLSUM_MAX_BLOCKS = 256;
void col_reduce_f64(const float* part, int nblk, int W, double* out, hipStream_t s);
constexpr int CR_BATCH_MAX = 48;
void col_reduce_acc_batch(const float* const* part, const int* nblk, const int* W, float* const* out0,
                          float* const* out1, const int* split, int n, hipStream_t s);
void col_reduce_acc(const float* part, int nblk, int W, float* out0, float* out1, int split,
                    hipStream_t s);
void bn_forward(const bf16_t* x, const bf16_t* res, bf16_t* y, long M, int C, float eps,
                float momentum, const float* gamma, const float* beta, float* run_mean,
                float* run_var, float* save_mean, float* save_rstd, int relu, double* sums,
                int sums_ready, uint8_t* ymask, hipStream_t s);
void bn_infer(const bf16_t* x, const bf16_t* res, bf16_t* y, long M, int C, const float* scale,
              const float* shift, int relu, hipStream_t s);
struct WTEntry {
  const bf16_t* w;
  bf16_t* wt;
  int K, RS, C, tile0;
};
constexpr int WT_MAX = 64;
struct WTBatch {
  int n;
  WTEntry e[WT_MAX];
};
void conv_weight_t_batch(WTBatch& b, hipStream_t s);
void bn_backward(const bf16_t* dy, const bf16_t* addend, const bf16_t* y, const bf16_t* x, const float* mean,
                 const float* rstd, const float* gamma, long M, int C, int relu, bf16_t* dx,
                 bf16_t* dres, float* dgamma, float* dbeta, double* sums, int sums_ready,
                 const uint8_t* ymask, hipStream_t s);

void ln_forward(const bf16_t* x, const float* g, const float* b, bf16_t* y, float* mean,
                float* rstd, long rows, int D, float eps, hipStream_t s, const bf16_t* addend = nullptr,
                bf16_t* sum_out = nullptr);
void ln_backward(const bf16_t* dy, const bf16_t* x, const float* g, const float* mean,
                 const float* rstd, bf16_t* dx, const bf16_t* addend, float* dg, float* db,
                 float* ws, long rows, int D, hipStream_t s);
int ln_backward_partial(const bf16_t* dy, const bf16_t* x, const float* g, const float* mean,
                        const float* rstd, bf16_t* dx, const bf16_t* addend, float* ws, long rows, int D,
                        hipStream_t s);

void maxpool_forward(const bf16_t* x, bf16_t* y, uint8_t* idx, int N, int H, int W, int C, int P,
                     int Q, int R, int S, int st, int pad, hipStream_t s);
void maxpool_k3s2_policy(int p);
void maxpool_backward(const bf16_t* dy, const uint8_t* idx, bf16_t* dx, int N, int H, int W, int C,
                      int P, int Q, int R, int S, int st, int pad, hipStream_t s);
void avgpool_forward(const bf16_t* x, bf16_t* y, int N, int HW, int C, hipStream_t s);
void avgpool_backward(const bf16_t* dy, bf16_t* dx, int N, int HW, int C, hipStream_t s);

void softmax_xent(const bf16_t* logits, const long* labels, bf16_t* dlogits, float* loss_rows,
                  long rows, int V, float smoothing, float grad_scale, long ignore_index,
                  hipStream_t s, long tm_b = 0);
void sum_scale(const float* x, long n, float* out, float scale, hipStream_t s);

void embedding_forward(const bf16_t* table, const long* ids, bf16_t* out, long T, int D,
                       float scale, hipStream_t s, long V, long tm_b = 0, const bf16_t* pos = nullptr,
                       long pos_rows = 0);
void embedding_backward(const bf16_t* dout, const long* ids, float* gtable, long T, int D,
                        float scale, hipStream_t s, long V, long tm_b = 0);

struct RowJob {
  const bf16_t* in[4];
  long ld_in[4];
  bf16_t* out;
  long ld_out;
  int C, n_in;
};
struct RowJobs {
  RowJob job[4];
};
void rows_sum(const RowJobs& jb, int njobs, long R, hipStream_t s);

void colsum(const bf16_t* x, float* out, float* ws, long R, int C, hipStream_t s);
void colsum_policy(int p);
void relu_backward(const bf16_t* dy, const bf16_t* y, bf16_t* dx, long n, hipStream_t s);
void add_bf16(const bf16_t* a, const bf16_t* b, bf16_t* y, long n, hipStream_t s);
void cast_f32_bf16(const float* x, bf16_t* y, long n, hipStream_t s);

void optim_grid(int blocks);
void sgd_step(float* w, float* g, float* mom, bf16_t* wb, long n, float lr, float momentum,
              float wd, float gscale, int nesterov, int zero_grad, hipStream_t s,
              const unsigned* guard = nullptr, long zero_from = 0, long wd_until = -1,
              const float* clip = nullptr);
void optim_variant(int v);
void adam_step(float* w, float* g, float* m, float* v, bf16_t* wb, long n, float lr, float b1,
               float b2, float eps, float wd, int step, float gscale, int zero_grad,
               hipStream_t s, const unsigned* guard = nullptr, long zero_from = 0, long wd_until = -1,
               const float* clip = nullptr);
int grad_sumsq_blocks(long n);
void grad_sumsq(const float* g, long n, double* partials, int slots, hipStream_t s);
void grad_clip_finalize(const double* partials, int slots, float max_norm, float gscale, float* clip,
                        hipStream_t s);

void attn_forward(const bf16_t* q, const bf16_t* k, const bf16_t* v, bf16_t* o, float* lse, int B,
                  int H, int Sq, int Sk, long q_stride, long kv_stride, long o_stride, long q_bstride,
                  long kv_bstride, long o_bstride, int causal, float scale, const int* kv_len, hipStream_t s);
void attn_short_policy(int p);
void attn_backward(const bf16_t* q, const bf16_t* k, const bf16_t* v, const bf16_t* o,
                   const bf16_t* dout, const float* lse, bf16_t* dq, bf16_t* dk, bf16_t* dv,
                   float* dq_acc, float* delta, int B, int H, int Sq, int Sk, long q_stride,
                   long kv_stride, long o_stride, long q_bstride, long kv_bstride, long o_bstride, int causal,
                   float scale, const int* kv_len, hipStream_t s);

void lstm_cell_forward(const float* gates, const float* c_prev, float* c_out, bf16_t* h_out,
                       float* h_out_f32, float* act_cache, int B, int Hd, hipStream_t s);
void lstm_step_forward(const float* gx, const bf16_t* w_hh, const bf16_t* h_prev, const float* c_prev,
                       float* c_out, bf16_t* h_out, float* act, int B, int Hd, hipStream_t s);
struct PLOpts {
  int grids = -1, rsv = 0;
  unsigned* job_err = nullptr;
  int zeroed = 0;
};
bool lstm_seq_forward(const float* gx, const bf16_t* w_hh, bf16_t* hs, float* cs, float* act, int T,
                      int B, int Hd, int reverse, unsigned* sync, hipStream_t s, const PLOpts& o = PLOpts());
bool lstm_seq_backward(const float* act, const float* cs, const float* dH, const bf16_t* w_hh, bf16_t* dG,
                       int T, int B, int Hd, int reverse, unsigned* sync, int dh_bf16, int ldh, hipStream_t s,
                       const PLOpts& o = PLOpts());
void lstm_guard_step(unsigned* err, hipStream_t s);
void lstm_seq_policy(int ch);
void lstm_seq_shards(int ns);
void lstm_seq_residency(int grids, int reserved_cus);
int64_t lstm_persist_timeouts(bool reset);
void lstm_seq_spin_limit(int64_t polls);
const unsigned* lstm_timeout_word();
void lstm_cell_backward(const float* act_cache, const float* c_prev, const float* c_out,
                        const float* dh, const float* dc_next, float* dgates, float* dc_prev,
                        bf16_t* dgates_bf16, int B, int Hd, hipStream_t s);

}
```

### csrc/include/tam/launch.h

```cpp
#pragma once
#include <hip/hip_runtime.h>
#include "tam/igemm.h"

namespace tam {

void gemm_igemm(const bf16_t* A, long lda, bool a_kmajor, const bf16_t* B, long ldb, bool b_kmajor, int M,
                int N, int K, const Epi& ep, hipStream_t s);
void gemm(const bf16_t* A, long lda, bool a_kmajor, const bf16_t* B, long ldb, bool b_kmajor,
          int M, int N, int K, Epi ep, bool allow_split, hipStream_t s);
void gemm_select(const bf16_t* A, long lda, bool a_kmajor, const bf16_t* B, long ldb, bool b_kmajor,
                 int M, int N, int K, Epi ep, bool allow_split, hipStream_t s, int path);
void gemm_force(int cfg, int splits);
void gemm_dma_policy(int policy, int cfg);
void gemm8p_policy(int mode, int tile);
bool gemm_pw(const bf16_t* A, long lda, const bf16_t* B, long ldb, bf16_t* C, long ldc, long M, int N, int K,
             const bf16_t* mask, long ldm, double* stats, int relu, hipStream_t s);
bool gemm_pw_ok(long M, int N, int K, long lda, long ldb, long ldc);
void gemm_pw_policy(int on);
void gemm8p_group(int g);
int gemm8p_policy_mode();

struct GGProblem {
  const bf16_t* A;
  const bf16_t* B;
  float* C;
  float* bias;
  int M, N, K, lda, ldb;
  int mode = 1;
};
void gemm_wgrad_grouped(const GGProblem* probs, int n, hipStream_t s);
void wgrad_slab_reduce_many(const float* const* ws, const int* sp, const long* mn, float* const* dw,
                            const int* mode, int n, hipStream_t s);
bool gemm_wgrad_grouped_ok(int M, int N, int K, long lda, long ldb);
void gemm_grouped_tile(int t);

void gemm_slab_reduce(const float* ws, int sp, int M, int N, const Epi& ep, hipStream_t s);

bool gemm_skinny_ok(bool ak, bool bk, int M, int N, int K, long lda, long ldb);
int gemm_skinny_splits(int M, int N, int K);
void gemm_skinny(const bf16_t* A, long lda, const bf16_t* B, long ldb, bool bk, int M, int N, int K,
                 const Epi& ep, int sp, float* ws, hipStream_t s);
void gemm_skinny_policy(int on, int force_splits, int nst);

int conv_fwd(const bf16_t* x, const bf16_t* w, const ConvGeom& g, Epi ep, hipStream_t s, float* ws = nullptr,
             long ws_floats = 0);
long conv_fwd_split_ws(const ConvGeom& g);
bool conv_stem_fwd(const bf16_t* x, const bf16_t* w, const ConvGeom& g, const Epi& ep, hipStream_t s);
void conv_stem_policy(int p);
long conv_stem_wgrad_ws(const ConvGeom& g);
bool conv_stem_wgrad(const bf16_t* dy, const bf16_t* x, const ConvGeom& g, float* dw, int mode, float* ws,
                     long ws_floats, hipStream_t s);
long conv_dgrad_split_ws(const ConvGeom& g);
void conv_split_policy(int p);
int conv_dgrad(const bf16_t* dy, const bf16_t* w, const bf16_t* wt, const ConvGeom& g, Epi ep,
               hipStream_t s, float* ws = nullptr, long ws_floats = 0);
int conv_wgrad(const bf16_t* dy, const bf16_t* x, const ConvGeom& g, Epi ep, hipStream_t s,
               float* dbias = nullptr, bool allow_patch = true, float* ws = nullptr, long ws_floats = 0,
               int* slab_defer = nullptr);
long conv_wgrad_split_ws(const ConvGeom& g);
void conv_wgrad_slab_policy(int p);
void conv_weight_t(const bf16_t* w, bf16_t* wt, const ConvGeom& g, hipStream_t s);
void conv_dma_policy(int p);
void conv_wgrad_force(int bm, int bn, int splits, int noatomic = 0);
void conv_wgrad_order(int flat);
void conv_wgrad_c64_policy(int p);
void conv_halo_policy(int p);
bool gemm_select_big_p8(bool ak, bool bk, int M, int N, int K, long lda, long ldb);

}
```

### csrc/kernels/gemm_grouped.hip

```cpp
#include <cstdlib>

#include "tam/launch.h"
#include "tam/tiles.h"
#include "tam/gemm8p.h"

namespace tam {

constexpr int P8G_MAX = 64;

struct P8GProb {
  const bf16_t* A;
  const bf16_t* B;
  float* C;
  float* bias;
  int M, N, K;
  int t0;
  int c0;
  int mode;
  int ntiles;
  int kps;
};

struct P8Group {
  P8GProb p[P8G_MAX];
  int n;
  int ncs;
};

__device__ __forceinline__ void gg_colsum(const P8GProb& pr, int blk, float* red) {
  const int m0 = blk * 64;
  const int tid = threadIdx.x, cg = tid & 7, rl = tid >> 3;
  const int RL = blockDim.x >> 3;
  const int col = m0 + cg * 8;
  float s[8];
#pragma unroll
  for (int e = 0; e < 8; ++e) s[e] = 0.f;
  if (col < pr.M) {
    const bf16_t* p = pr.A + col;
    int r = rl;
    for (; r + 3 * RL < pr.K; r += 4 * RL) {
      uint4 v[4];
#pragma unroll
      for (int u = 0; u < 4; ++u) v[u] = *(const uint4*)(p + (long)(r + RL * u) * pr.M);
#pragma unroll
      for (int u = 0; u < 4; ++u) {
        const uint32_t w[4] = {v[u].x, v[u].y, v[u].z, v[u].w};
#pragma unroll
        for (int e = 0; e < 4; ++e) {
          s[2 * e] += bf2f((bf16_t)(w[e] & 0xffff));
          s[2 * e + 1] += bf2f((bf16_t)(w[e] >> 16));
        }
      }
    }
    for (; r < pr.K; r += RL) {
      const uint4 v = *(const uint4*)(p + (long)r * pr.M);
      const uint32_t w[4] = {v.x, v.y, v.z, v.w};
#pragma unroll
      for (int e = 0; e < 4; ++e) {
        s[2 * e] += bf2f((bf16_t)(w[e] & 0xffff));
        s[2 * e + 1] += bf2f((bf16_t)(w[e] >> 16));
      }
    }
  }
#pragma unroll
  for (int e = 0; e < 8; ++e) red[rl * 64 + cg * 8 + e] = s[e];
  __syncthreads();
  if (tid < 64 && m0 + tid < pr.M) {
    float t = 0.f;
    for (int k = 0; k < RL; ++k) t += red[k * 64 + tid];
    pr.bias[m0 + tid] += t;
  }
}

template <int BM, int BN, int WNW>
__global__ void __launch_bounds__(64 * 2 * WNW, (BM == 256 ? 1 : 2)) gemm8p_grouped_kernel(P8Group g) {
  const int bid = xcd_remap(blockIdx.x, gridDim.x);
  if (bid < g.ncs) {
    __shared__ float cs_red[64 * 64];
    int c = 0;
    while (c + 1 < g.n && bid >= g.p[c + 1].c0) ++c;
    gg_colsum(g.p[c], bid - g.p[c].c0, cs_red);
    return;
  }
  const int t = bid - g.ncs;
  int c = 0;
  while (c + 1 < g.n && t >= g.p[c + 1].t0) ++c;
  const P8GProb& pr = g.p[c];
  const int u = t - pr.t0;
  const int tile = u % pr.ntiles, kz = u / pr.ntiles;
  const bool split = pr.kps < pr.K / P8_BK;
  P8Args a{pr.A, (long)pr.M, pr.B, (long)pr.N, pr.M, pr.N, pr.K, pr.kps, 4};
  Epi ep;
  ep.c = pr.C;
  ep.ldc = pr.N;
  ep.c_f32 = 1;
  ep.mode = split ? 2 : pr.mode;
  gemm8p_body<BM, BN, WNW, false, false>(a, ep, tile, kz);
}

static int g_gg_tile = [] {
  const char* e = getenv("TAM_GROUPED_TILE");
  return e ? atoi(e) : 128;
}();
TAM_KNOB(g_gg_tile)
void gemm_grouped_tile(int t) { g_gg_tile = t == 256 ? 256 : 128; }

static int g_gg_split_kt = [] {
  const char* e = getenv("TAM_GROUPED_SPLIT_KT");
  return e ? atoi(e) : 64;
}();
TAM_KNOB(g_gg_split_kt)

static int gg_kps(int K, int mode) {
  const int kt = K / P8_BK;
  if (g_gg_split_kt <= 0 || mode != 1 || kt <= 2 * g_gg_split_kt) return kt;
  int sk = cdiv(kt, g_gg_split_kt);
  if (sk > 32) sk = 32;
  return cdiv(kt, sk);
}

void gemm_wgrad_grouped(const GGProblem* probs, int n, hipStream_t s) {
  const int T = g_gg_tile == 128 ? 128 : 256;
  for (int base = 0; base < n; base += P8G_MAX) {
    P8Group g{};
    const int m = n - base < P8G_MAX ? n - base : P8G_MAX;
    int tiles = 0, cs = 0;
    for (int i = 0; i < m; ++i) {
      const GGProblem& q = probs[base + i];
      P8GProb& p = g.p[i];
      p.A = q.A; p.B = q.B; p.C = q.C; p.bias = q.bias;
      p.M = q.M; p.N = q.N; p.K = q.K;
      p.mode = q.mode;
      p.t0 = tiles;
      p.c0 = cs;
      p.ntiles = cdiv(q.M, T) * cdiv(q.N, T);
      p.kps = gg_kps(q.K, q.mode);
      tiles += p.ntiles * cdiv(q.K / P8_BK, p.kps);
      if (q.bias) cs += cdiv(q.M, 64);
    }
    g.n = m;
    g.ncs = cs;
    if (tiles + cs == 0) continue;
    if (T == 128)
      hipLaunchKernelGGL((gemm8p_grouped_kernel<128, 128, 2>), dim3((unsigned)(tiles + cs)), dim3(256), 0, s, g);
    else
      hipLaunchKernelGGL((gemm8p_grouped_kernel<256, 256, 4>), dim3((unsigned)(tiles + cs)), dim3(512), 0, s, g);
  }
}

bool gemm_wgrad_grouped_ok(int M, int N, int K, long lda, long ldb) {
  return lda == M && ldb == N && gemm8p_ok(false, false, M, N, K, lda, ldb) &&
         (long)K * (M > N ? M : N) < (1L << 31);
}

}
```

### csrc/kernels/optim.hip

```cpp
#include <cmath>
#include <cstdlib>

#include "tam/common.h"
#include "tam/kernels.h"

namespace tam {

__global__ void __launch_bounds__(256) sgd_kernel(float* __restrict__ w, float* __restrict__ g,
                                                   float* __restrict__ mom,
                                                   bf16_t* __restrict__ wb, long n4, float lr,
                                                   float momentum, float wd0, float gscale,
                                                   int nesterov, int zero_grad, const unsigned* guard,
                                                   long zero_from4, long wd_until4, const float* clip) {
  if ((guard != nullptr && *guard != 0u) || (clip != nullptr && clip[0] < 0.f)) {
    for (long i = blockIdx.x * (long)blockDim.x + threadIdx.x; i < n4; i += (long)gridDim.x * blockDim.x)
      if (i >= zero_from4) ((float4*)g)[i] = make_float4(0.f, 0.f, 0.f, 0.f);
    return;
  }
  if (clip != nullptr) gscale *= clip[0];
  for (long i = blockIdx.x * (long)blockDim.x + threadIdx.x; i < n4;
       i += (long)gridDim.x * blockDim.x) {
    float4 wv = ((float4*)w)[i];
    float4 gv = ((float4*)g)[i];
    float4 mv = ((float4*)mom)[i];
    float* wp = (float*)&wv; float* gp = (float*)&gv; float* mp = (float*)&mv;
    const float wd = i < wd_until4 ? wd0 : 0.f;
#pragma unroll
    for (int k = 0; k < 4; ++k) {
      float d = __builtin_fmaf(wd, wp[k], gp[k] * gscale);
      mp[k] = __builtin_fmaf(momentum, mp[k], d);
      d = nesterov ? __builtin_fmaf(momentum, mp[k], d) : mp[k];
      wp[k] = __builtin_fmaf(-lr, d, wp[k]);
    }
    ((float4*)w)[i] = wv;
    ((float4*)mom)[i] = mv;
    if (zero_grad && i >= zero_from4) ((float4*)g)[i] = make_float4(0.f, 0.f, 0.f, 0.f);
    ((uint2*)wb)[i] = make_uint2(pack_bf2(wp[0], wp[1]), pack_bf2(wp[2], wp[3]));
  }
}

__global__ void __launch_bounds__(256) adam_kernel(float* __restrict__ w, float* __restrict__ g,
                                                    float* __restrict__ m, float* __restrict__ v,
                                                    bf16_t* __restrict__ wb, long n4, float lr,
                                                    float b1, float b2, float eps, float wd0,
                                                    float bc1, float bc2, float gscale,
                                                    int zero_grad, const unsigned* guard, long zero_from4,
                                                    long wd_until4, const float* clip) {
  if ((guard != nullptr && *guard != 0u) || (clip != nullptr && clip[0] < 0.f)) {
    for (long i = blockIdx.x * (long)blockDim.x + threadIdx.x; i < n4; i += (long)gridDim.x * blockDim.x)
      if (i >= zero_from4) ((float4*)g)[i] = make_float4(0.f, 0.f, 0.f, 0.f);
    return;
  }
  if (clip != nullptr) gscale *= clip[0];
  const float ib1 = 1.f / bc1, ib2 = 1.f / bc2;
  for (long i = blockIdx.x * (long)blockDim.x + threadIdx.x; i < n4;
       i += (long)gridDim.x * blockDim.x) {
    float4 wv = ((float4*)w)[i], gv = ((float4*)g)[i], mv = ((float4*)m)[i], vv = ((float4*)v)[i];
    float* wp = (float*)&wv; float* gp = (float*)&gv; float* mp = (float*)&mv; float* vp = (float*)&vv;
    const float wd = i < wd_until4 ? wd0 : 0.f;
#pragma unroll
    for (int k = 0; k < 4; ++k) {
      const float gr = gp[k] * gscale;
      mp[k] = __builtin_fmaf(b1, mp[k], (1.f - b1) * gr);
      vp[k] = __builtin_fmaf(b2, vp[k], (1.f - b2) * gr * gr);
      const float mh = mp[k] * ib1, vh = vp[k] * ib2;
      const float u = __builtin_fmaf(wd, wp[k], mh / (sqrtf(vh) + eps));
      wp[k] = __builtin_fmaf(-lr, u, wp[k]);
    }
    ((float4*)w)[i] = wv; ((float4*)m)[i] = mv; ((float4*)v)[i] = vv;
    if (zero_grad && i >= zero_from4) ((float4*)g)[i] = make_float4(0.f, 0.f, 0.f, 0.f);
    ((uint2*)wb)[i] = make_uint2(pack_bf2(wp[0], wp[1]), pack_bf2(wp[2], wp[3]));
  }
}

typedef unsigned u32x2_t __attribute__((ext_vector_type(2)));
template <int U, bool NT>
__device__ __forceinline__ float4 ld4(const float* p, long i) {
  if constexpr (NT) {
    const f32x4_t r = __builtin_nontemporal_load((const f32x4_t*)p + i);
    return make_float4(r[0], r[1], r[2], r[3]);
  } else {
    return ((const float4*)p)[i];
  }
}
template <bool NT>
__device__ __forceinline__ void st4(float* p, long i, float4 v) {
  if constexpr (NT) __builtin_nontemporal_store(f32x4_t{v.x, v.y, v.z, v.w}, (f32x4_t*)p + i);
  else ((float4*)p)[i] = v;
}
template <bool NT>
__device__ __forceinline__ void st2(bf16_t* p, long i, uint2 v) {
  if constexpr (NT) __builtin_nontemporal_store(u32x2_t{v.x, v.y}, (u32x2_t*)p + i);
  else ((uint2*)p)[i] = v;
}

template <int U, bool NT>
__global__ void __launch_bounds__(256) adam_stream_kernel(float* __restrict__ w, float* __restrict__ g,
                                                           float* __restrict__ m, float* __restrict__ v,
                                                           bf16_t* __restrict__ wb, long n4, float lr, float b1,
                                                           float b2, float eps, float wd0, float bc1, float bc2,
                                                           float gscale, int zero_grad, const unsigned* guard,
                                                           long zero_from4, long wd_until4, const float* clip) {
  const long stride = (long)gridDim.x * blockDim.x;
  if ((guard != nullptr && *guard != 0u) || (clip != nullptr && clip[0] < 0.f)) {
    for (long i = blockIdx.x * (long)blockDim.x + threadIdx.x; i < n4; i += stride)
      if (i >= zero_from4) st4<NT>(g, i, make_float4(0.f, 0.f, 0.f, 0.f));
    return;
  }
  if (clip != nullptr) gscale *= clip[0];
  const float ib1 = 1.f / bc1, ib2 = 1.f / bc2;
  auto body = [&](long i, float4 wv, float4 gv, float4 mv, float4 vv) {
    float* wp = (float*)&wv; float* gp = (float*)&gv; float* mp = (float*)&mv; float* vp = (float*)&vv;
    const float wd = i < wd_until4 ? wd0 : 0.f;
#pragma unroll
    for (int k = 0; k < 4; ++k) {
      const float gr = gp[k] * gscale;
      mp[k] = __builtin_fmaf(b1, mp[k], (1.f - b1) * gr);
      vp[k] = __builtin_fmaf(b2, vp[k], (1.f - b2) * gr * gr);
      const float mh = mp[k] * ib1, vh = vp[k] * ib2;
      const float u = __builtin_fmaf(wd, wp[k], mh / (sqrtf(vh) + eps));
      wp[k] = __builtin_fmaf(-lr, u, wp[k]);
    }
    st4<NT>(w, i, wv); st4<NT>(m, i, mv); st4<NT>(v, i, vv);
    if (zero_grad && i >= zero_from4) st4<NT>(g, i, make_float4(0.f, 0.f, 0.f, 0.f));
    st2<NT>(wb, i, make_uint2(pack_bf2(wp[0], wp[1]), pack_bf2(wp[2], wp[3])));
  };
  const long t = blockIdx.x * (long)blockDim.x + threadIdx.x;
  const long full = n4 / (U * stride) * (U * stride);
  for (long base = t; base < full; base += U * stride) {
    float4 wv[U], gv[U], mv[U], vv[U];
#pragma unroll
    for (int u = 0; u < U; ++u) {
      const long i = base + u * stride;
      wv[u] = ld4<U, NT>(w, i); gv[u] = ld4<U, NT>(g, i); mv[u] = ld4<U, NT>(m, i); vv[u] = ld4<U, NT>(v, i);
    }
#pragma unroll
    for (int u = 0; u < U; ++u) body(base + u * stride, wv[u], gv[u], mv[u], vv[u]);
  }
  for (long i = full + t; i < n4; i += stride)
    body(i, ld4<1, NT>(w, i), ld4<1, NT>(g, i), ld4<1, NT>(m, i), ld4<1, NT>(v, i));
}

template <int U, bool NT>
__global__ void __launch_bounds__(256) sgd_stream_kernel(float* __restrict__ w, float* __restrict__ g,
                                                          float* __restrict__ mom, bf16_t* __restrict__ wb, long n4,
                                                          float lr, float momentum, float wd0, float gscale,
                                                          int nesterov, int zero_grad, const unsigned* guard,
                                                          long zero_from4, long wd_until4, const float* clip) {
  const long stride = (long)gridDim.x * blockDim.x;
  if ((guard != nullptr && *guard != 0u) || (clip != nullptr && clip[0] < 0.f)) {
    for (long i = blockIdx.x * (long)blockDim.x + threadIdx.x; i < n4; i += stride)
      if (i >= zero_from4) st4<NT>(g, i, make_float4(0.f, 0.f, 0.f, 0.f));
    return;
  }
  if (clip != nullptr) gscale *= clip[0];
  auto body = [&](long i, float4 wv, float4 gv, float4 mv) {
    float* wp = (float*)&wv; float* gp = (float*)&gv; float* mp = (float*)&mv;
    const float wd = i < wd_until4 ? wd0 : 0.f;
#pragma unroll
    for (int k = 0; k < 4; ++k) {
      float d = __builtin_fmaf(wd, wp[k], gp[k] * gscale);
      mp[k] = __builtin_fmaf(momentum, mp[k], d);
      d = nesterov ? __builtin_fmaf(momentum, mp[k], d) : mp[k];
      wp[k] = __builtin_fmaf(-lr, d, wp[k]);
    }
    st4<NT>(w, i, wv); st4<NT>(mom, i, mv);
    if (zero_grad && i >= zero_from4) st4<NT>(g, i, make_float4(0.f, 0.f, 0.f, 0.f));
    st2<NT>(wb, i, make_uint2(pack_bf2(wp[0], wp[1]), pack_bf2(wp[2], wp[3])));
  };
  const long t = blockIdx.x * (long)blockDim.x + threadIdx.x;
  const long full = n4 / (U * stride) * (U * stride);
  for (long base = t; base < full; base += U * stride) {
    float4 wv[U], gv[U], mv[U];
#pragma unroll
    for (int u = 0; u < U; ++u) {
      const long i = base + u * stride;
      wv[u] = ld4<U, NT>(w, i); gv[u] = ld4<U, NT>(g, i); mv[u] = ld4<U, NT>(mom, i);
    }
#pragma unroll
    for (int u = 0; u < U; ++u) body(base + u * stride, wv[u], gv[u], mv[u]);
  }
  for (long i = full + t; i < n4; i += stride) body(i, ld4<1, NT>(w, i), ld4<1, NT>(g, i), ld4<1, NT>(mom, i));
}

static int g_optim_variant = [] {
  const char* e = getenv("TAM_OPTIM_VARIANT");
  return e ? atoi(e) : -1;
}();
TAM_KNOB(g_optim_variant)
void optim_variant(int v) { g_optim_variant = v; }
static int optim_pick(long, bool) {
  return g_optim_variant >= 0 ? g_optim_variant : 3;
}

static int g_optim_grid = [] {
  const char* e = getenv("TAM_OPTIM_GRID");
  return e ? atoi(e) : 0;
}();
TAM_KNOB(g_optim_grid)
void optim_grid(int blocks) { g_optim_grid = blocks > 0 ? blocks : 0; }

static int ogrid(long n4) {
  static int cus = 0;
  if (!cus) {
    int dev = 0;
    if (hipGetDevice(&dev) != hipSuccess ||
        hipDeviceGetAttribute(&cus, hipDeviceAttributeMultiprocessorCount, dev) != hipSuccess || cus < 1)
      cus = 256;
  }
  const long cap = g_optim_grid > 0 ? g_optim_grid : cus;
  long b = (n4 + 255) / 256;
  if (b > cap) b = cap;
  return (int)(b < 1 ? 1 : b);
}

void sgd_step(float* w, float* g, float* mom, bf16_t* wb, long n, float lr, float momentum,
              float wd, float gscale, int nesterov, int zero_grad, hipStream_t s, const unsigned* guard,
              long zero_from, long wd_until, const float* clip) {
  const dim3 grid(ogrid(n / 4));
  const long zf4 = zero_from / 4, wu4 = wd_until < 0 ? n / 4 : wd_until / 4;
  switch (optim_pick(n / 4, false)) {
    case 3:
      hipLaunchKernelGGL((sgd_stream_kernel<4, true>), grid, dim3(256), 0, s, w, g, mom, wb, n / 4, lr, momentum, wd,
                         gscale, nesterov, zero_grad, guard, zf4, wu4, clip);
      break;
    default:
      hipLaunchKernelGGL(sgd_kernel, grid, dim3(256), 0, s, w, g, mom, wb, n / 4, lr, momentum, wd, gscale, nesterov,
                         zero_grad, guard, zf4, wu4, clip);
  }
}

void adam_step(float* w, float* g, float* m, float* v, bf16_t* wb, long n, float lr, float b1,
               float b2, float eps, float wd, int step, float gscale, int zero_grad,
               hipStream_t s, const unsigned* guard, long zero_from, long wd_until, const float* clip) {
  const float bc1 = 1.f - powf(b1, (float)step), bc2 = 1.f - powf(b2, (float)step);
  const dim3 grid(ogrid(n / 4));
  const long zf4 = zero_from / 4, wu4 = wd_until < 0 ? n / 4 : wd_until / 4;
  switch (optim_pick(n / 4, true)) {
    case 3:
      hipLaunchKernelGGL((adam_stream_kernel<4, true>), grid, dim3(256), 0, s, w, g, m, v, wb, n / 4, lr, b1, b2, eps,
                         wd, bc1, bc2, gscale, zero_grad, guard, zf4, wu4, clip);
      break;
    default:
      hipLaunchKernelGGL(adam_kernel, grid, dim3(256), 0, s, w, g, m, v, wb, n / 4, lr, b1, b2, eps, wd, bc1, bc2,
                         gscale, zero_grad, guard, zf4, wu4, clip);
  }
}

template <int U>
__global__ void __launch_bounds__(256) grad_sumsq_kernel(const float* __restrict__ g, long n4,
                                                          double* __restrict__ partials, int slots) {
  const long stride = (long)gridDim.x * blockDim.x;
  const long t = blockIdx.x * (long)blockDim.x + threadIdx.x;
  const long full = n4 / (U * stride) * (U * stride);
  double a0 = 0., a1 = 0., a2 = 0., a3 = 0.;
  auto acc = [&](float4 v) {
    a0 = fma((double)v.x, (double)v.x, a0); a1 = fma((double)v.y, (double)v.y, a1);
    a2 = fma((double)v.z, (double)v.z, a2); a3 = fma((double)v.w, (double)v.w, a3);
  };
  for (long base = t; base < full; base += U * stride) {
    float4 gv[U];
#pragma unroll
    for (int u = 0; u < U; ++u) gv[u] = ((const float4*)g)[base + u * stride];
#pragma unroll
    for (int u = 0; u < U; ++u) acc(gv[u]);
  }
  for (long i = full + t; i < n4; i += stride) acc(((const float4*)g)[i]);
  double r = (a0 + a1) + (a2 + a3);
#pragma unroll
  for (int o = 32; o > 0; o >>= 1) r += __shfl_down(r, o, 64);
  __shared__ double wsum[4];
  if ((threadIdx.x & 63) == 0) wsum[threadIdx.x >> 6] = r;
  __syncthreads();
  if (threadIdx.x == 0) partials[blockIdx.x] = (wsum[0] + wsum[1]) + (wsum[2] + wsum[3]);
  for (long s = gridDim.x + t; s < slots; s += stride) partials[s] = 0.;
}

__global__ void __launch_bounds__(256) grad_clip_finalize_kernel(const double* __restrict__ partials, int P,
                                                                  float max_norm, float gscale, float* clip) {
  __shared__ double red[256];
  double a = 0.;
  for (int i = threadIdx.x; i < P; i += 256) a += partials[i];
  red[threadIdx.x] = a;
  __syncthreads();
  for (int o = 128; o > 0; o >>= 1) {
    if ((int)threadIdx.x < o) red[threadIdx.x] += red[threadIdx.x + o];
    __syncthreads();
  }
  if (threadIdx.x == 0) {
    const float norm = (float)((double)gscale * sqrt(red[0]));
    unsigned* cnt = (unsigned*)clip;
    float scale = -1.f;
    if (isfinite(norm)) {
      scale = fminf(1.f, (float)((double)max_norm / ((double)norm + 1e-6)));
      if (scale < 1.f) cnt[3] += 1u;
    } else {
      cnt[2] += 1u;
    }
    clip[0] = scale;
    clip[1] = norm;
  }
}

int grad_sumsq_blocks(long n) { return ogrid(n / 4); }

void grad_sumsq(const float* g, long n, double* partials, int slots, hipStream_t s) {
  hipLaunchKernelGGL((grad_sumsq_kernel<8>), dim3(ogrid(n / 4)), dim3(256), 0, s, g, n / 4, partials, slots);
}

void grad_clip_finalize(const double* partials, int slots, float max_norm, float gscale, float* clip,
                        hipStream_t s) {
  hipLaunchKernelGGL(grad_clip_finalize_kernel, dim3(1), dim3(256), 0, s, partials, slots, max_norm, gscale, clip);
}

__global__ void lstm_guard_step_kernel(unsigned* err) {
  if (threadIdx.x == 0 && err[0] != 0u) {
    err[1] += 1u;
    err[0] = 0u;
  }
}

void lstm_guard_step(unsigned* err, hipStream_t s) {
  hipLaunchKernelGGL(lstm_guard_step_kernel, dim3(1), dim3(64), 0, s, err);
}

}
```

### tiresias_amd/executor/trainer.py

```python
from __future__ import annotations

import os
import time
from typing import Dict, List, Optional

import torch

from ..models import MODELS, make_model, samples_per_batch, synthetic_batch
from ..ops import _lib
from ..ops import functional as Fx
from ..ops.arena import Arena
from ..parallel.ddp import GradBucketer
from ..parallel.gang import comm_size


class Trainer:
    def __init__(self, model: str, device, batch: Optional[int] = None, group=None, seed: int = 0,
                 data_seed: Optional[int] = None, use_graph: bool = False, bucket_mb: float = 32.0,
                 model_kwargs: Optional[dict] = None, lr: Optional[float] = None,
                 overlap_wgrad: Optional[bool] = None, branches: Optional[bool] = None,
                 ddp_shard: bool = False, ddp_wire: str = "fp32", grad_clip: Optional[float] = None):
        self.model_name = model
        self.spec = MODELS[model]
        if grad_clip is None:
            grad_clip = self.spec.clip
        if grad_clip is not None and ddp_shard and group is not None and comm_size(group) > 1:
            raise ValueError("grad_clip with ddp_shard is not supported: a sharded gang's global norm needs "
                             "the replicated tails counted once")
        self.device = torch.device(device)
        if self.device.type == "cuda":
            _lib.load(required=True)
        self.batch = batch or self.spec.batch
        self.arena = Arena(self.device, seed=seed)
        self.model = make_model(model, self.arena, **(model_kwargs or {}))
        self.arena.materialize()
        n = self.arena.numel
        self.opt = self.spec.opt
        self.lr = lr if lr is not None else self.spec.lr
        if self.opt == "sgd":
            self.opt_state = [torch.zeros(n, dtype=torch.float32, device=self.device)]
        else:
            self.opt_state = [torch.zeros(n, dtype=torch.float32, device=self.device),
                              torch.zeros(n, dtype=torch.float32, device=self.device)]
        self.step_count = 0
        self.data = synthetic_batch(model, self.batch, self.device,
                                    seed=seed if data_seed is None else data_seed)
        self.group = group
        self.ddp = None
        self._bucket_mb = bucket_mb
        self.ddp_shard, self.ddp_wire = ddp_shard, ddp_wire
        if group is not None and comm_size(group) > 1:
            self.ddp = GradBucketer(self.arena, group, bucket_mb=bucket_mb, shard=ddp_shard, wire=ddp_wire)
        from ..utils import debug

        self._want_graph = use_graph and self.device.type == "cuda" and debug.level() == 0
        self.use_graph = self._want_graph and self.ddp is None
        self._graph = None
        self._g_loss = None
        self._g_written = []
        self._warm = 0
        self.capture_s = 0.0
        self._side = None
        self._ws = None
        self._defer_n = 0
        self.overlap_wgrad = self.spec.overlap_wgrad if overlap_wgrad is None else overlap_wgrad
        self.group_wgrad = self.spec.group_wgrad and os.environ.get("TAM_GROUP_WGRAD", "1") != "0"
        self.branches = getattr(self.model, "branch_default", False) if branches is None else branches
        self._bs: List = []
        self.last_loss: Optional[torch.Tensor] = None
        self.grad_clip: Optional[float] = None
        self._clip = None
        self._clip_part = None
        self._clip_host = [1.0, 0.0, 0, 0]
        self.set_grad_clip(grad_clip)
        self._ready = None
        if self.device.type == "cuda":
            self._ready = torch.cuda.Event()
            self._ready.record(torch.cuda.current_stream(self.device))

    def _fwd_bwd(self) -> torch.Tensor:
        d = self.data
        ws = None
        if self.device.type == "cuda" and self.ddp is None and self.overlap_wgrad:
            if self._ws is None:
                self._ws = torch.cuda.Stream(self.device)
            ws = self._ws
        Fx.set_wgrad_stream(ws)
        nb = getattr(self.model, "branch_streams", 0) if self.branches else 0
        if self.device.type == "cuda" and self.ddp is None and nb:
            if len(self._bs) < nb:
                self._bs = [torch.cuda.Stream(self.device) for _ in range(nb)]
            Fx.set_branch_streams(self._bs)
        group = (self.device.type == "cuda" and self.ddp is None and self.group_wgrad)
        if group:
            Fx.defer_wgrad(True)
        try:
            if self.spec.kind == "image":
                logits = self.model.forward(d["x"])
            else:
                logits = self.model.forward(d)
            labels = d["labels"]
            rows = labels.numel()
            loss, dlog = Fx.softmax_xent(logits, labels, smoothing=self.spec.smoothing,
                                         ignore_index=-100, normalizer=rows,
                                         labels_time_major=getattr(self.model, "logits_time_major", False))
            logits.backward(dlog)
            if group:
                Fx.flush_wgrad()
                self._defer_n = Fx.deferred_count()
        finally:
            if group:
                Fx.defer_wgrad(False, discard=True)
            Fx.set_wgrad_stream(None)
            Fx.set_branch_streams(None)
        if ws is not None:
            torch.cuda.current_stream(self.device).wait_stream(ws)
        if self.device.type == "cuda" and self.ddp is None and nb:
            for s in self._bs:
                torch.cuda.current_stream(self.device).wait_stream(s)
        return loss

    def set_grad_clip(self, v: Optional[float]) -> None:
        if v is not None:
            v = float(v)
            if not (v > 0.0 and v != float("inf")):
                raise ValueError(f"grad_clip must be a finite number > 0, got {v}")
            if self.ddp is not None and self.ddp.shard:
                raise ValueError("grad_clip with ddp_shard is not supported: a sharded gang's global norm "
                                 "needs the replicated tails counted once")
            if self.device.type == "cuda" and self._clip is None:
                T = _lib.ops()
                self._clip = torch.zeros(4, dtype=torch.float32, device=self.device)
                self._clip_part = torch.zeros(int(T.grad_sumsq_blocks(self.arena.numel)), dtype=torch.float64,
                                              device=self.device)
        self.grad_clip = v

    def _clip_launch(self, gscale: float):
        if self.grad_clip is None:
            return None
        T = _lib.ops()
        T.grad_sumsq(self.arena.grad, self._clip_part)
        T.grad_clip_finalize(self._clip_part, self.grad_clip, gscale, self._clip)
        return self._clip

    def clip_stats(self) -> dict:
        if self._clip is not None:
            rec = self._clip.cpu()
            cnt = rec.view(torch.int32)
            st = [float(rec[0]), float(rec[1]), int(cnt[2]), int(cnt[3])]
        else:
            st = self._clip_host
        if self.step_count == 0:
            st = [1.0, 0.0, st[2], st[3]]
        return {"last_scale": st[0], "last_norm": st[1], "nonfinite_steps": st[2], "clipped_steps": st[3]}

    def _opt_step(self):
        A = self.arena
        gscale = self.ddp.grad_scale if self.ddp is not None else 1.0
        self.step_count += 1
        sharded = self.ddp is not None and self.ddp.shard
        if sharded:
            self.ddp.join_gather()
            regions = []
            for a, b in self.ddp.owned_ranges():
                if a < A.n_decay:
                    regions.append((a, min(b, A.n_decay), self.spec.wd))
                if b > A.n_decay:
                    regions.append((max(a, A.n_decay), b, 0.0))
        elif self.device.type == "cuda":
            for p in A.params:
                if p.store_grad and p.gw_epoch != A.grad_epoch:
                    p.grad.zero_()
            A.grad_epoch += 1
            T = _lib.ops()
            guard = self.model.err if self.uses_persist else None
            zf = A.n_store if Fx.STORE_GRAD else 0
            clip = self._clip_launch(gscale)
            if self.opt == "sgd":
                T.sgd_step(A.master, A.grad, self.opt_state[0], A.shadow, self.lr, 0.9, self.spec.wd, gscale, False,
                           True, guard, zf, A.n_decay, clip)
            else:
                T.adam_step(A.master, A.grad, self.opt_state[0], self.opt_state[1], A.shadow, self.lr, 0.9, 0.98,
                            1e-9, self.spec.wd, self.step_count, gscale, True, guard, zf, A.n_decay, clip)
            if self.uses_persist:
                _lib.ops().lstm_guard_step(self.model.err)
            return
        else:
            regions = [(0, A.n_decay, self.spec.wd), (A.n_decay, A.numel, 0.0)]
            if self.grad_clip is not None:
                norm = gscale * float(A.grad.double().norm())
                st = self._clip_host
                if norm == norm and abs(norm) != float("inf"):
                    scale = min(1.0, self.grad_clip / (norm + 1e-6))
                    st[3] += scale < 1.0
                    gscale = gscale * scale
                else:
                    scale = -1.0
                    st[2] += 1
                    A.grad.zero_()
                    regions = []
                st[0], st[1] = scale, norm
        clip = None
        A.grad_epoch += 1
        for reg in regions:
            lo, hi, wd = reg[:3]
            zero = (reg[3] if len(reg) > 3 else True) and not sharded
            if hi <= lo:
                continue
            w, g, wb = A.master[lo:hi], A.grad[lo:hi], A.shadow[lo:hi]
            if self.device.type == "cuda":
                T = _lib.ops()
                guard = self.model.err if self.uses_persist else None
                if self.opt == "sgd":
                    T.sgd_step(w, g, self.opt_state[0][lo:hi], wb, self.lr, 0.9, wd, gscale, False, zero, guard,
                               0, -1, clip)
                else:
                    T.adam_step(w, g, self.opt_state[0][lo:hi], self.opt_state[1][lo:hi], wb, self.lr,
                                0.9, 0.98, 1e-9, wd, self.step_count, gscale, zero, guard, 0, -1, clip)
            else:
                _cpu_opt(self.opt, w, g, self.opt_state, lo, hi, wb, self.lr, wd, gscale, self.step_count)
        if sharded:
            A.grad.zero_()
            self.ddp.gather_shadow()
        if self.uses_persist:
            _lib.ops().lstm_guard_step(self.model.err)

    def enable_graph(self) -> None:
        from ..utils import debug

        if self.device.type != "cuda" or debug.level() != 0 or self.ddp is not None:
            return
        self._want_graph = True
        self.use_graph = True
        self._graph = None
        self._warm = 0

    @property
    def uses_persist(self) -> bool:
        return (self.device.type == "cuda" and bool(getattr(self.model, "persist", False))
                and not getattr(self, "_persist_shared", False))

    def set_persist_shared(self, shared: bool) -> None:
        shared = bool(shared)
        if shared != getattr(self, "_persist_shared", False):
            self._persist_shared = shared
            if hasattr(self.model, "shared"):
                self.model.shared = shared
                self._graph = None
                self._g_loss = None

    def persist_skipped(self, reset: bool = True) -> int:
        if not self.uses_persist:
            return 0
        n = int(self.model.err[1].item())
        if reset and n:
            self.model.err.zero_()
        return n

    def disable_persist(self) -> None:
        if hasattr(self.model, "persist"):
            self.model.persist = False
        self._graph = None
        self._g_loss = None

    def step(self) -> torch.Tensor:
        if self.uses_persist:
            self.model.residency = (1, 64) if self.ddp is not None else (2, 0)
        if self._ready is not None:
            torch.cuda.current_stream(self.device).wait_event(self._ready)
            self._ready = None
        if self.use_graph and self._graph is None and self._warm < 2:
            s = self._side or torch.cuda.Stream(self.device)
            self._side = s
            s.wait_stream(torch.cuda.current_stream(self.device))
            with torch.cuda.stream(s):
                loss = self._fwd_bwd()
                self._opt_step()
            torch.cuda.current_stream(self.device).wait_stream(s)
            self._warm += 1
            self.last_loss = loss
            return loss
        if self.use_graph:
            loss = self._graph_step()
        else:
            loss = self._fwd_bwd()
            if self.ddp is not None:
                self.ddp.finish()
        self._opt_step()
        self.last_loss = loss
        return loss

    def _graph_step(self) -> torch.Tensor:
        if self._graph is None:
            s = self._side or torch.cuda.Stream(self.device)
            self._side = s
            cur = torch.cuda.current_stream(self.device)
            s.wait_stream(cur)
            tc = time.perf_counter()
            g = torch.cuda.CUDAGraph()
            with torch.cuda.stream(s):
                g.capture_begin()
                try:
                    self._g_loss = self._fwd_bwd()
                finally:
                    g.capture_end()
            cur.wait_stream(s)
            self._graph = g
            self.capture_s += time.perf_counter() - tc
            A = self.arena
            self._g_written = [p for p in A.params if p.store_grad and p.gw_epoch == A.grad_epoch]
        self._graph.replay()
        for p in self._g_written:
            p.gw_epoch = self.arena.grad_epoch
        return self._g_loss

    def run(self, iters: int) -> float:
        t0 = time.perf_counter()
        for _ in range(iters):
            self.step()
        if self.device.type == "cuda":
            torch.cuda.synchronize(self.device)
        return time.perf_counter() - t0

    def samples_per_step(self) -> int:
        return samples_per_batch(self.model_name, self.batch)

    def consolidate(self) -> int:
        if self.ddp is None or not self.ddp.shard:
            return 0
        return self.ddp.consolidate([self.arena.master] + list(self.opt_state))

    @property
    def state_sharded(self) -> bool:
        return self.ddp is not None and self.ddp.shard and self.ddp.dirty

    def state_tensors(self) -> Dict[str, torch.Tensor]:
        if self.state_sharded:
            raise RuntimeError("trainer state is sharded across its gang: consolidate() first")
        st = {"master": self.arena.master, "shadow": self.arena.shadow}
        for i, t in enumerate(self.opt_state):
            st[f"opt{i}"] = t
        for k, v in self.model.buffers().items():
            st["buf." + k] = v
        return st

    def state_bytes(self) -> int:
        return sum(t.numel() * t.element_size() for t in self.state_tensors().values())

    def _spill_buffers(self):
        bufs = [self.arena.master] + list(self.opt_state)
        bufs += [v for v in self.model.buffers().values()]
        return bufs

    def offload(self, engine) -> int:
        if getattr(self, "_spilled", None):
            return 0
        if self.state_sharded:
            raise RuntimeError("trainer state is sharded across its gang: consolidate() before offload()")
        self._release_host_copies()
        self._graph = None
        self._g_loss = None
        self.last_loss = None
        handles, nbytes = [], 0
        self._save_counted = False
        for b in self._spill_buffers():
            handles.append((b, engine.spill(b), b.untyped_storage().nbytes()))
            nbytes += b.numel() * b.element_size()
        if self.device.type == "cuda":
            side = torch.cuda.ExternalStream(engine.stream_handle(), device=self.device)
            for b, _, _ in handles:
                b.record_stream(side)
        for b in [self.arena.master, self.arena.shadow, self.arena.grad] + list(self.opt_state):
            b.untyped_storage().resize_(0)
        self._spilled = handles
        self._engine = engine
        return nbytes

    def restore(self) -> int:
        handles = getattr(self, "_spilled", None)
        if not handles:
            return 0
        A = self.arena
        for b, n in ((A.master, A.numel * 4), (A.shadow, A.numel * 2), (A.grad, A.numel * 4)):
            b.untyped_storage().resize_(n)
        for t in self.opt_state:
            t.untyped_storage().resize_(t.numel() * 4)
        nbytes = 0
        for b, h, _ in handles:
            self._engine.restore(h, b)
            nbytes += b.numel() * b.element_size()
        A.grad.zero_()
        A.shadow.copy_(A.master.to(torch.bfloat16))
        if hasattr(self._engine, "copy_ms"):
            self._restored = handles
        else:
            for _, h, _ in handles:
                self._engine.release(h)
        self._spilled = None
        return nbytes

    def ckpt_poll(self) -> dict:
        out = {"save_s": 0.0, "restore_s": 0.0}
        eng = getattr(self, "_engine", None)
        if eng is None or not hasattr(eng, "copy_ms"):
            return out
        for which in ("_spilled", "_restored"):
            hs = getattr(self, which, None) or []
            if hs and not getattr(self, "_save_counted", False):
                ms = [eng.copy_ms(h, 0) for _, h, _ in hs]
                if all(m >= 0 for m in ms):
                    out["save_s"] += sum(ms) / 1e3
                    self._save_counted = True
        restored = getattr(self, "_restored", None) or []
        if restored and getattr(self, "_save_counted", False):
            ms = [eng.copy_ms(h, 1) for _, h, _ in restored]
            if all(m >= 0 for m in ms):
                out["restore_s"] += sum(ms) / 1e3
                for _, h, _ in restored:
                    eng.release(h)
                self._restored = None
        return out

    def reset(self, seed: int, data_seed: Optional[int] = None, init: bool = True) -> "Trainer":
        if getattr(self, "_spilled", None):
            raise RuntimeError("reset of a spilled trainer")
        if self.ddp is not None:
            self.ddp.dirty = False
        if init:
            self.arena.reinit(seed)
            for t in self.opt_state:
                t.zero_()
            for k, v in self.model.buffers().items():
                if k.endswith(".var"):
                    v.fill_(1.0)
                else:
                    v.zero_()
        fresh = synthetic_batch(self.model_name, self.batch, self.device,
                                seed=seed if data_seed is None else data_seed)
        for k, v in fresh.items():
            self.data[k].copy_(v)
        self.step_count = 0
        self.last_loss = None
        if self._clip is not None:
            self._clip.zero_()
        self._clip_host = [1.0, 0.0, 0, 0]
        if self.device.type == "cuda":
            self._ready = torch.cuda.Event()
            self._ready.record(torch.cuda.current_stream(self.device))
        return self

    def rebind(self, group) -> None:
        if self.grad_clip is not None and self.ddp_shard and group is not None and comm_size(group) > 1:
            raise ValueError("grad_clip with ddp_shard is not supported")
        dirty = self.state_sharded
        old_ranks = tuple(getattr(self.ddp.comm, "ranks", ())) if self.ddp is not None else ()
        new_ranks = tuple(getattr(group, "ranks", ())) if group is not None else ()
        if dirty and old_ranks != new_ranks:
            raise RuntimeError(f"sharded trainer state on {old_ranks} cannot move to {new_ranks}: "
                               "consolidate() first")
        regather = self.ddp is not None and bool(self.ddp._gathers)
        if self.ddp is not None:
            self.ddp._gathers = {}
        self.group = group
        self.arena.on_grad_ready = None
# ... 50 lines not shown
```

### tiresias_amd/ops/arena.py

```python
from __future__ import annotations

import math
from dataclasses import dataclass, field
from typing import Callable, List, Optional, Sequence

import torch

_ALIGN = 64


@dataclass
class Param:
    name: str
    shape: tuple
    init: str = "normal"
    std: float = 0.02
    decay: bool = True
    fp32_compute: bool = False
    store_grad: bool = False
    gw_epoch: int = -1
    offset: int = 0
    numel: int = 0
    _w: Optional[torch.Tensor] = field(default=None, repr=False)
    master: Optional[torch.Tensor] = None
    grad: Optional[torch.Tensor] = None
    arena: Optional["Arena"] = field(default=None, repr=False)

    @property
    def w(self) -> Optional[torch.Tensor]:
        a = self.arena
        if a is not None and a.on_param_use is not None:
            a.on_param_use(self)
        return self._w

    @w.setter
    def w(self, t: Optional[torch.Tensor]) -> None:
        self._w = t

    @property
    def value(self) -> torch.Tensor:
        return self.master if self.fp32_compute else self.w

    def grad_ready(self) -> None:
        if self.arena is not None and self.arena.on_grad_ready is not None:
            self.arena.on_grad_ready(self)


def _padded(n: int) -> int:
    return (n + _ALIGN - 1) // _ALIGN * _ALIGN


class Arena:
    def __init__(self, device: torch.device | str = "cpu", seed: int = 0):
        self.device = torch.device(device)
        self.params: List[Param] = []
        self.seed = seed
        self.master = self.shadow = self.grad = None
        self.numel = 0
        self.n_decay = 0
        self.n_store = 0
        self.grad_epoch = 0
        self.on_grad_ready: Optional[Callable[[Param], None]] = None
        self.on_param_use: Optional[Callable[[Param], None]] = None
        self.token = torch.zeros(1, device=self.device, requires_grad=True)

    def add(self, name: str, shape: Sequence[int], init: str = "normal", std: float = 0.02,
            decay: bool = True, fp32_compute: bool = False, store_grad: bool = False) -> Param:
        p = Param(name=name, shape=tuple(int(s) for s in shape), init=init, std=std, decay=decay,
                  fp32_compute=fp32_compute, store_grad=store_grad and decay)
        p.numel = int(math.prod(p.shape))
        p.arena = self
        self.params.append(p)
        return p

    def _order(self) -> List[Param]:
        return ([p for p in self.params if p.store_grad] + [p for p in self.params if p.decay and not p.store_grad]
                + [p for p in self.params if not p.decay])

    def layout(self) -> List[Param]:
        off = 0
        order = self._order()
        for p in order:
            p.offset = off
            off += _padded(p.numel)
            if p.decay:
                self.n_decay = off
            if p.store_grad:
                self.n_store = off
        self.numel = max(off, _ALIGN)
        return order

    def materialize(self) -> "Arena":
        order = self.layout()
        dev = self.device
        self.master = torch.zeros(self.numel, dtype=torch.float32, device=dev)
        self.shadow = torch.zeros(self.numel, dtype=torch.bfloat16, device=dev)
        self.grad = torch.zeros(self.numel, dtype=torch.float32, device=dev)
        for p in order:
            p.master = self.master[p.offset:p.offset + p.numel].view(p.shape)
            p.w = self.shadow[p.offset:p.offset + p.numel].view(p.shape)
            p.grad = self.grad[p.offset:p.offset + p.numel].view(p.shape)
        self.reinit(self.seed)
        return self

    def reinit(self, seed: int) -> None:
        self.seed = seed
        g = torch.Generator(device=self.device)
        g.manual_seed(seed)
        for p in self._order():
            self._init_into(p, g)
        self.shadow.copy_(self.master.to(torch.bfloat16))
        self.grad.zero_()

    @staticmethod
    def _init_into(p: Param, g: torch.Generator) -> None:
        t = p.master
        if p.init == "zeros":
            t.zero_()
        elif p.init == "ones":
            t.fill_(1.0)
        elif p.init == "kaiming":
            fan_in = max(1, p.numel // p.shape[0])
            t.normal_(0.0, math.sqrt(2.0 / fan_in), generator=g)
        elif p.init == "xavier":
            fan_in = max(1, p.numel // p.shape[0])
            a = math.sqrt(6.0 / (fan_in + p.shape[0]))
            t.uniform_(-a, a, generator=g)
        elif p.init == "uniform":
            t.uniform_(-p.std, p.std, generator=g)
        else:
            t.normal_(0.0, p.std, generator=g)

    def zero_grad(self) -> None:
        self.grad.zero_()

    def state_bytes(self) -> int:
        return self.numel * (4 + 2 + 4)

    def named(self):
        return {p.name: p for p in self.params}

    def sync_shadow(self) -> None:
        self.shadow.copy_(self.master.to(torch.bfloat16))
```

### tiresias_amd/ops/functional.py

```python
from __future__ import annotations

import math
import os
from typing import List, Optional, Tuple

import torch
import torch.nn.functional as F
from torch.autograd import Function

from . import _lib
from .arena import Param

BF16 = torch.bfloat16


def _T():
    return _lib.ops()


def _cpu_gemm_f32(a: torch.Tensor, b: torch.Tensor) -> torch.Tensor:
    return a.float() @ b.float()


_WGRAD_STREAM = None


def set_wgrad_stream(stream) -> None:
    global _WGRAD_STREAM
    _WGRAD_STREAM = stream


class _OnWgrad:
    def __init__(self, *tensors, stream=None):
        self.s = (stream or _WGRAD_STREAM) if tensors[0].is_cuda else None
        self.ts = tensors
        self.ctx = None

    def __enter__(self):
        if self.s is None:
            return self
        self.s.wait_stream(torch.cuda.current_stream(self.ts[0].device))
        for t in self.ts:
            t.record_stream(self.s)
        self.ctx = torch.cuda.stream(self.s)
        self.ctx.__enter__()
        return self

    def __exit__(self, *exc):
        if self.ctx is not None:
            self.ctx.__exit__(*exc)
        return False


_DEFER_WGRAD: Optional[list] = None
_DEFER_CHUNK = int(os.environ.get("TAM_WGRAD_GROUP_CHUNK", "0") or 0)
_GROUP_OK: dict = {}
_DEFER_COUNT = 0


def defer_wgrad(on: bool, discard: bool = False) -> None:
    global _DEFER_WGRAD, _DEFER_COUNT
    _DEFER_COUNT = 0
    if not on and _DEFER_WGRAD and not discard:
        raise RuntimeError("defer_wgrad(False) with unflushed weight gradients")
    if not on:
        _DEFER_LNRED.clear()
    if not on and _DEFER_WGRAD:
        for it in _DEFER_WGRAD:
            it[2].gw_epoch = -1
    _DEFER_WGRAD = [] if on else None


GROUP_MAX_MNK = float(os.environ.get("TAM_GROUP_MAX_MNK", str(float(1 << 35))))


def _group_ok(M: int, N: int, K: int) -> bool:
    key = (M, N, K)
    ok = _GROUP_OK.get(key)
    if ok is None:
        ok = bool(_T().gemm_wgrad_grouped_ok(M, N, K)) and float(M) * N * K <= GROUP_MAX_MNK
        _GROUP_OK[key] = ok
    return ok


def defer_problems(probs) -> bool:
    if _DEFER_WGRAD is None:
        return False
    for it in probs:
        if any(p[2] is it[2] for p in _DEFER_WGRAD):
            flush_wgrad()
            break
    for it in probs:
        _DEFER_WGRAD.append(tuple(it))
        _deferred()
    return True


def deferred_count() -> int:
    return _DEFER_COUNT


def _deferred(pending_flush: bool = True) -> None:
    global _DEFER_COUNT
    _DEFER_COUNT += 1
    if _DEFER_CHUNK and len(_DEFER_WGRAD) >= _DEFER_CHUNK:
        flush_wgrad()


def flush_wgrad() -> int:
    if _DEFER_LNRED:
        lnr = list(_DEFER_LNRED)
        _DEFER_LNRED.clear()
        _T().col_reduce_acc_batch([e[0] for e in lnr], [e[1] for e in lnr], [e[2].grad for e in lnr],
                                  [e[3].grad for e in lnr])
        for _, _, g, b in lnr:
            g.grad_ready()
            b.grad_ready()
    pend = _DEFER_WGRAD
    if not pend:
        return 0
    items = list(pend)
    pend.clear()
    dys = [it[0] for it in items]
    with _OnWgrad(*dys, *[it[1] for it in items]):
        empty = torch.empty(0, dtype=torch.float32, device=dys[0].device)
        _T().gemm_wgrad_grouped(dys, [it[1] for it in items], [it[5] if len(it) > 5 else it[2].grad for it in items],
                                [it[3].grad if it[3] is not None else empty for it in items],
                                [it[4] for it in items])
    for it in items:
        it[2].grad_ready()
        if it[3] is not None:
            it[3].grad_ready()
    return len(items)


_BRANCH_STREAMS: list = []


def set_branch_streams(streams) -> None:
    global _BRANCH_STREAMS
    _BRANCH_STREAMS = list(streams or [])


class on_branch:

    def __init__(self, i: int, *inputs):
        self.s = _BRANCH_STREAMS[i] if i < len(_BRANCH_STREAMS) and inputs[0].is_cuda else None
        self.ts = inputs
        self.ctx = None

    def __enter__(self):
        if self.s is None:
            return self
        self.s.wait_stream(torch.cuda.current_stream(self.ts[0].device))
        for t in self.ts:
            t.record_stream(self.s)
        self.ctx = torch.cuda.stream(self.s)
        self.ctx.__enter__()
        return self

    def __exit__(self, *exc):
        if self.ctx is not None:
            self.ctx.__exit__(*exc)
        return False


def join_branch(i: int, *outputs):
    if i < len(_BRANCH_STREAMS) and outputs[0].is_cuda:
        cur = torch.cuda.current_stream(outputs[0].device)
        cur.wait_stream(_BRANCH_STREAMS[i])
        for t in outputs:
            t.record_stream(cur)
    return outputs if len(outputs) > 1 else outputs[0]


STORE_GRAD = os.environ.get("TAM_STORE_GRAD", "1") != "0"


def grad_mode(p: Param) -> int:
    A = p.arena
    first = p.gw_epoch != A.grad_epoch
    p.gw_epoch = A.grad_epoch
    return 0 if (first and STORE_GRAD) else 1


class _Linear(Function):
    @staticmethod
    def forward(ctx, x, token, w: Param, b: Optional[Param], relu: bool, in_relu: bool,
                mask_own_relu: bool):
        M = x.shape[0]
        out = w.shape[0]
        if x.is_cuda:
            y = torch.empty(M, out, dtype=BF16, device=x.device)
            _T().gemm(x, True, w.w, True, y, 0, b.w if b is not None else None, relu, None, 1.0, False)
        else:
            yf = _cpu_gemm_f32(x, w.w.t())
            if b is not None:
                yf = yf + b.w.float()
            if relu:
                yf = yf.clamp_min(0)
            y = yf.to(BF16)
        ctx.w, ctx.b, ctx.relu, ctx.in_relu, ctx.mask_own = w, b, relu, in_relu, mask_own_relu
        ctx.save_for_backward(x, y if (relu and mask_own_relu) else None)
        return y

    @staticmethod
    def backward(ctx, dy):
        x, y = ctx.saved_tensors
        w, b = ctx.w, ctx.b
        dy = dy.contiguous()
        if y is not None:
            if dy.is_cuda:
                dyr = torch.empty_like(dy)
                _T().relu_backward(dy, y, dyr)
                dy = dyr
            else:
                dy = (dy.float() * (y.float() > 0)).to(BF16)
        dx = None
        deferred = False
        if dy.is_cuda:
            if (_DEFER_WGRAD is not None and x.dim() == 2 and w.grad.is_contiguous()
                    and _group_ok(w.shape[0], w.shape[1], x.shape[0])):
                if any(it[2] is w for it in _DEFER_WGRAD):
                    flush_wgrad()
                if w.store_grad:
                    mode = grad_mode(w)
                else:
                    w.gw_epoch = w.arena.grad_epoch
                    mode = 1
                _DEFER_WGRAD.append((dy, x, w, b, mode))
                deferred = True
            else:
                if _DEFER_WGRAD is not None and any(it[2] is w for it in _DEFER_WGRAD):
                    flush_wgrad()
                with _OnWgrad(dy, x):
                    _T().gemm(dy, False, x, False, w.grad, grad_mode(w), None, False, None, 1.0, True,
                              b.grad if b is not None else None)
        if ctx.needs_input_grad[0]:
            if dy.is_cuda:
                dx = torch.empty_like(x)
                wk = weight_kmajor(w)
                if wk is not None:
                    _T().gemm(dy, True, wk, True, dx, 0, None, False, x if ctx.in_relu else None, 1.0, False)
                else:
                    _T().gemm(dy, True, w.w, False, dx, 0, None, False, x if ctx.in_relu else None, 1.0, False)
            else:
                dxf = _cpu_gemm_f32(dy, w.w)
                if ctx.in_relu:
                    dxf = dxf * (x.float() > 0)
                dx = dxf.to(BF16)
        if not dy.is_cuda:
            w.grad += _cpu_gemm_f32(dy.t(), x)
            if b is not None:
                b.grad += dy.float().sum(0)
        if deferred:
            _deferred()
        else:
            w.grad_ready()
            if b is not None:
                b.grad_ready()
        return dx, None, None, None, None, None, None


def linear(x: torch.Tensor, w: Param, b: Optional[Param] = None, relu: bool = False,
           in_relu: bool = False, mask_own_relu: bool = True) -> torch.Tensor:
    shp = x.shape
    x2 = x.reshape(-1, shp[-1])
    if not x2.is_contiguous():
        x2 = x2.contiguous()
    y = _Linear.apply(x2, w.arena.token, w, b, relu, in_relu, mask_own_relu)
    return y.view(*shp[:-1], w.shape[0])


def _conv_out(h: int, k: int, s: int, p: int, d: int = 1) -> int:
    return (h + 2 * p - d * (k - 1) - 1) // s + 1




BN_RELU_BITMASK = True

# ... 780 lines not shown
```

Baseline: 0.1343.

## Fuse optimizer update into grouped wgrad GEMM epilogue for final flush

On the last deferred weight-gradient flush, eligible store-mode GEMM problems apply the SGD/Adam update directly in the GEMM epilogue. It writes master weights, optimizer state and the bf16 shadow, reading hyperparameters from a device-side record. The standalone optimizer kernel then skips those arena ranges through a new skip list. The aim is to avoid re-reading and re-writing gradients and optimizer state for those parameters, at the cost of a heavier GEMM epilogue, extra record writes, and more complex graph-capture bookkeeping.

```diff
diff --git a/csrc/bindings/ops.cpp b/csrc/bindings/ops.cpp
--- a/csrc/bindings/ops.cpp
+++ b/csrc/bindings/ops.cpp
@@ -463,12 +463,14 @@
   tam::conv_dgrad(bp(dy), bp(w), bp(wt), g, ep, cur_stream(dy), wsf > 0 ? ws.data_ptr<float>() : nullptr, wsf);
 }
 
-void gemm_wgrad_grouped_op(at::TensorList dy, at::TensorList x, at::TensorList dw, at::TensorList db,
-                           at::OptionalIntArrayRef modes) {
+static std::vector<int64_t> gemm_wgrad_grouped_impl(at::TensorList dy, at::TensorList x, at::TensorList dw,
+                                                    at::TensorList db, at::OptionalIntArrayRef modes,
+                                                    at::OptionalIntArrayRef fuse, const tam::OptimApply* oa,
+                                                    long arena_n) {
   TORCH_CHECK(dy.size() == x.size() && dy.size() == dw.size() && dy.size() == db.size(),
               "tam.gemm_wgrad_grouped: list sizes differ");
   TORCH_CHECK(!modes.has_value() || modes->size() == dy.size(), "tam.gemm_wgrad_grouped: modes size");
-  if (dy.empty()) return;
+  if (dy.empty()) return {};
   std::vector<tam::GGProblem> probs(dy.size());
   for (size_t i = 0; i < dy.size(); ++i) {
     const Tensor& a = dy[i];
@@ -493,9 +495,49 @@
     }
     const int mode = modes.has_value() ? (int)(*modes)[i] : 1;
     TORCH_CHECK(mode == 0 || mode == 1, "tam.gemm_wgrad_grouped: mode must be 0 (store) or 1 (accumulate)");
-    probs[i] = tam::GGProblem{bp(a), bp(b), c.data_ptr<float>(), bias, M, N, K, M, N, mode};
-  }
-  tam::gemm_wgrad_grouped(probs.data(), (int)probs.size(), cur_stream(dy[0]));
+    probs[i] = tam::GGProblem{bp(a), bp(b), c.data_ptr<float>(), bias, M, N, K, M, N, mode,
+                              fuse.has_value() && (*fuse)[i] != 0 ? 1 : 0};
+  }
+  std::vector<int> fused(probs.size(), 0);
+  tam::gemm_wgrad_grouped(probs.data(), (int)probs.size(), cur_stream(dy[0]), oa, arena_n, fused.data());
+  return std::vector<int64_t>(fused.begin(), fused.end());
+}
+
+void gemm_wgrad_grouped_op(at::TensorList dy, at::TensorList x, at::TensorList dw, at::TensorList db,
+                           at::OptionalIntArrayRef modes) {
+  gemm_wgrad_grouped_impl(dy, x, dw, db, modes, c10::nullopt, nullptr, 0);
+}
+
+std::vector<int64_t> gemm_wgrad_grouped_apply_op(at::TensorList dy, at::TensorList x, at::TensorList dw,
+                                                 at::TensorList db, at::IntArrayRef modes, at::IntArrayRef fuse,
+                                                 const Tensor& rec, const Tensor& g, const Tensor& w,
+                                                 const Tensor& s0, const optional<Tensor>& s1, const Tensor& wb) {
+  TORCH_CHECK(fuse.size() == dy.size() && modes.size() == dy.size(), "tam.gemm_wgrad_grouped_apply: list sizes");
+  check_f32(g, "g"); check_f32(w, "w"); check_f32(s0, "s0"); check_bf16(wb, "wb");
+  check_contig(g, "g"); check_contig(w, "w"); check_contig(s0, "s0"); check_contig(wb, "wb");
+  const bool adam = s1.has_value() && s1->defined();
+  if (adam) { check_f32(*s1, "s1"); check_contig(*s1, "s1"); }
+  TORCH_CHECK(w.numel() == g.numel() && s0.numel() == g.numel() && wb.numel() == g.numel() &&
+                  (!adam || s1->numel() == g.numel()),
+              "tam.gemm_wgrad_grouped_apply: the arenas must be parallel (same numel)");
+  TORCH_CHECK(w.device() == g.device() && s0.device() == g.device() && wb.device() == g.device() &&
+                  rec.device() == g.device() && (!adam || s1->device() == g.device()),
+              "tam.gemm_wgrad_grouped_apply: all arenas on one device");
+  TORCH_CHECK(rec.is_contiguous() && rec.numel() * rec.element_size() >= (int64_t)sizeof(tam::OptimRec) &&
+                  (((uintptr_t)rec.data_ptr()) & 15) == 0,
+              "tam.gemm_wgrad_grouped_apply: rec must be a 16-B aligned buffer of >= 64 B");
+  tam::OptimApply oa;
+  oa.rec = (const tam::OptimRec*)rec.data_ptr();
+  oa.g = g.data_ptr<float>();
+  oa.w = w.data_ptr<float>();
+  oa.s0 = s0.data_ptr<float>();
+  oa.s1 = adam ? s1->data_ptr<float>() : nullptr;
+  oa.wb = bpm(wb);
+  oa.kind = adam ? 2 : 1;
+  TORCH_CHECK(((((uintptr_t)oa.g) | ((uintptr_t)oa.w) | ((uintptr_t)oa.s0) | ((uintptr_t)oa.s1)) & 15) == 0 &&
+                  (((uintptr_t)oa.wb) & 7) == 0,
+              "tam.gemm_wgrad_grouped_apply: arenas must be 16-B aligned");
+  return gemm_wgrad_grouped_impl(dy, x, dw, db, modes, fuse, &oa, (long)g.numel());
 }
 
 void gemm_grouped_tile_op(int64_t t) { tam::gemm_grouped_tile((int)t); }
@@ -998,30 +1040,52 @@
               "tam: clip must be a 16-B aligned float32 [4] tensor on the parameters' device");
   return clip->data_ptr<float>();
 }
+static std::vector<long> skip_list(at::OptionalIntArrayRef skip) {
+  std::vector<long> sk;
+  if (skip.has_value()) {
+    TORCH_CHECK(skip->size() % 2 == 0, "tam: skip must hold (lo, hi) pairs");
+    sk.assign(skip->begin(), skip->end());
+  }
+  return sk;
+}
 void sgd_op(const Tensor& w, const Tensor& g, const Tensor& mom, const Tensor& wb, double lr,
             double momentum, double wd, double gscale, bool nesterov, bool zero_grad,
             const optional<Tensor>& guard, int64_t zero_from, int64_t wd_until,
-            const optional<Tensor>& clip) {
+            const optional<Tensor>& clip, at::OptionalIntArrayRef skip) {
   check_f32(w, "w"); check_f32(g, "g"); check_f32(mom, "mom"); check_bf16(wb, "wb");
   TORCH_CHECK(w.numel() % 4 == 0 && g.numel() == w.numel() && mom.numel() == w.numel() &&
                   wb.numel() == w.numel(),
               "tam.sgd: sizes");
   TORCH_CHECK(zero_from % 4 == 0 && (wd_until < 0 || wd_until % 4 == 0), "tam.sgd: region bounds % 4");
-  tam::sgd_step(w.data_ptr<float>(), g.data_ptr<float>(), mom.data_ptr<float>(), bpm(wb), w.numel(),
-                (float)lr, (float)momentum, (float)wd, (float)gscale, nesterov, zero_grad,
-                cur_stream(w), guard_ptr(guard, w), (long)zero_from, (long)wd_until, clip_ptr(clip, w));
+  const std::vector<long> sk = skip_list(skip);
+  TORCH_CHECK(tam::sgd_step(w.data_ptr<float>(), g.data_ptr<float>(), mom.data_ptr<float>(), bpm(wb), w.numel(),
+                            (float)lr, (float)momentum, (float)wd, (float)gscale, nesterov, zero_grad,
+                            cur_stream(w), guard_ptr(guard, w), (long)zero_from, (long)wd_until, clip_ptr(clip, w),
+                            sk.data(), (int)(sk.size() / 2)),
+              "tam.sgd: skip must be sorted, disjoint ranges of multiples of 4 inside the arena");
 }
 void adam_op(const Tensor& w, const Tensor& g, const Tensor& m, const Tensor& v, const Tensor& wb,
              double lr, double b1, double b2, double eps, double wd, int64_t step, double gscale,
              bool zero_grad, const optional<Tensor>& guard, int64_t zero_from, int64_t wd_until,
-             const optional<Tensor>& clip) {
+             const optional<Tensor>& clip, at::OptionalIntArrayRef skip) {
   check_f32(w, "w"); check_f32(g, "g"); check_f32(m, "m"); check_f32(v, "v"); check_bf16(wb, "wb");
   TORCH_CHECK(w.numel() % 4 == 0, "tam.adam: numel % 4");
   TORCH_CHECK(zero_from % 4 == 0 && (wd_until < 0 || wd_until % 4 == 0), "tam.adam: region bounds % 4");
-  tam::adam_step(w.data_ptr<float>(), g.data_ptr<float>(), m.data_ptr<float>(), v.data_ptr<float>(),
-                 bpm(wb), w.numel(), (float)lr, (float)b1, (float)b2, (float)eps, (float)wd,
-                 (int)step, (float)gscale, zero_grad, cur_stream(w), guard_ptr(guard, w), (long)zero_from,
-                 (long)wd_until, clip_ptr(clip, w));
+  const std::vector<long> sk = skip_list(skip);
+  TORCH_CHECK(tam::adam_step(w.data_ptr<float>(), g.data_ptr<float>(), m.data_ptr<float>(), v.data_ptr<float>(),
+                             bpm(wb), w.numel(), (float)lr, (float)b1, (float)b2, (float)eps, (float)wd,
+                             (int)step, (float)gscale, zero_grad, cur_stream(w), guard_ptr(guard, w),
+                             (long)zero_from, (long)wd_until, clip_ptr(clip, w), sk.data(), (int)(sk.size() / 2)),
+              "tam.adam: skip must be sorted, disjoint ranges of multiples of 4 inside the arena");
+}
+void optim_record_op(const Tensor& rec, double lr, double b1, double b2, double eps, double wd, int64_t step,
+                     double gscale, bool nesterov, const optional<Tensor>& guard) {
+  check_dev(rec, "rec");
+  TORCH_CHECK(rec.is_contiguous() && rec.numel() * rec.element_size() >= (int64_t)sizeof(tam::OptimRec) &&
+                  (((uintptr_t)rec.data_ptr()) & 15) == 0,
+              "tam.optim_record: rec must be a 16-B aligned buffer of >= 64 B");
+  tam::optim_record((tam::OptimRec*)rec.data_ptr(), (float)lr, (float)b1, (float)b2, (float)eps, (float)wd,
+                    (int)step, (float)gscale, nesterov, guard_ptr(guard, rec), cur_stream(rec));
 }
 void grad_sumsq_op(const Tensor& g, const Tensor& partials) {
   check_f32(g, "g"); check_contig(g, "g"); check_dev(partials, "partials"); check_contig(partials, "partials");
@@ -1211,6 +1275,7 @@
   m.def("conv_weight_t_batch(Tensor[] w, Tensor(a!)[] wt) -> ()", &conv_weight_t_batch_op);
   m.def("gemm_wgrad_grouped(Tensor[] dy, Tensor[] x, Tensor(a!)[] dw, Tensor(b!)[] db, int[]? modes=None) -> ()", &gemm_wgrad_grouped_op);
   m.def("gemm_wgrad_grouped_ok(int M, int N, int K) -> bool", &gemm_wgrad_grouped_ok_op);
+  m.def("gemm_wgrad_grouped_apply(Tensor[] dy, Tensor[] x, Tensor(a!)[] dw, Tensor(b!)[] db, int[] modes, int[] fuse, Tensor rec, Tensor g, Tensor(c!) w, Tensor(d!) s0, Tensor(e!)? s1, Tensor(f!) wb) -> int[]", &gemm_wgrad_grouped_apply_op);
   m.def("gemm_grouped_tile(int tile) -> ()", &gemm_grouped_tile_op);
   m.def("conv_dgrad_pre(Tensor dy, Tensor w, Tensor wt, Tensor(a!) dx, int stride, int pad, int dil, Tensor? mask, Tensor(b!)? stats=None, Tensor? bnx=None, Tensor? bnmean=None, Tensor? bnrstd=None) -> int", &conv_dgrad_pre_op);
   m.def("conv_wgrad(Tensor dy, Tensor x, Tensor(a!) dw, int stride, int pad, int dil, int mode, Tensor(b!)? dbias=None, bool patch=True) -> ()", &conv_wgrad_op);
@@ -1263,8 +1328,9 @@
   m.def("relu_backward(Tensor dy, Tensor y, Tensor(a!) dx) -> ()", &relu_backward_op);
   m.def("add(Tensor a, Tensor b, Tensor(a!) y) -> ()", &add_op);
   m.def("cast_f32_bf16(Tensor x, Tensor(a!) y) -> ()", &cast_op);
-  m.def("sgd_step(Tensor(a!) w, Tensor(b!) g, Tensor(c!) mom, Tensor(d!) wb, float lr, float momentum, float wd, float gscale, bool nesterov, bool zero_grad, Tensor? guard=None, int zero_from=0, int wd_until=-1, Tensor? clip=None) -> ()", &sgd_op);
-  m.def("adam_step(Tensor(a!) w, Tensor(b!) g, Tensor(c!) m, Tensor(d!) v, Tensor(e!) wb, float lr, float b1, float b2, float eps, float wd, int step, float gscale, bool zero_grad, Tensor? guard=None, int zero_from=0, int wd_until=-1, Tensor? clip=None) -> ()", &adam_op);
+  m.def("sgd_step(Tensor(a!) w, Tensor(b!) g, Tensor(c!) mom, Tensor(d!) wb, float lr, float momentum, float wd, float gscale, bool nesterov, bool zero_grad, Tensor? guard=None, int zero_from=0, int wd_until=-1, Tensor? clip=None, int[]? skip=None) -> ()", &sgd_op);
+  m.def("adam_step(Tensor(a!) w, Tensor(b!) g, Tensor(c!) m, Tensor(d!) v, Tensor(e!) wb, float lr, float b1, float b2, float eps, float wd, int step, float gscale, bool zero_grad, Tensor? guard=None, int zero_from=0, int wd_until=-1, Tensor? clip=None, int[]? skip=None) -> ()", &adam_op);
+  m.def("optim_record(Tensor(a!) rec, float lr, float b1, float b2, float eps, float wd, int step, float gscale, bool nesterov, Tensor? guard=None) -> ()", &optim_record_op);
   m.def("grad_sumsq(Tensor g, Tensor(a!) partials) -> ()", &grad_sumsq_op);
   m.def("grad_clip_finalize(Tensor partials, float max_norm, float gscale, Tensor(a!) clip) -> ()", &grad_clip_finalize_op);
   m.def("grad_sumsq_blocks(int n) -> int", &grad_sumsq_blocks_op);
diff --git a/csrc/include/tam/gemm8p.h b/csrc/include/tam/gemm8p.h
--- a/csrc/include/tam/gemm8p.h
+++ b/csrc/include/tam/gemm8p.h
@@ -1,5 +1,6 @@
 #pragma once
 #include "tam/igemm.h"
+#include "tam/optim_update.h"
 
 namespace tam {
 
@@ -110,10 +111,42 @@
   __builtin_amdgcn_sched_barrier(0);
 }
 
-template <int BM, int BN, int WNW, int TI, int TJ, int J0 = 0, int NJ = TJ>
+constexpr int P8_MODE_APPLY = 4;
+
+typedef unsigned p8_u32x2_t __attribute__((ext_vector_type(2)));
+
+__device__ __forceinline__ void p8_apply4(const OptimApply& oa, const OptimRec& h, const float ib1, const float ib2,
+                                          const long off, const float4 g) {
+  f32x4_t wv = __builtin_nontemporal_load((const f32x4_t*)(oa.w + off));
+  f32x4_t mv = __builtin_nontemporal_load((const f32x4_t*)(oa.s0 + off));
+  const float gp[4] = {g.x, g.y, g.z, g.w};
+  if (oa.kind == 2) {
+    f32x4_t vv = __builtin_nontemporal_load((const f32x4_t*)(oa.s1 + off));
+#pragma unroll
+    for (int k = 0; k < 4; ++k) {
+      float w = wv[k], m = mv[k], v = vv[k];
+      adam_update(w, gp[k], m, v, h.lr, h.b1, h.b2, h.eps, h.wd, ib1, ib2, h.gscale);
+      wv[k] = w; mv[k] = m; vv[k] = v;
+    }
+    __builtin_nontemporal_store(vv, (f32x4_t*)(oa.s1 + off));
+  } else {
+#pragma unroll
+    for (int k = 0; k < 4; ++k) {
+      float w = wv[k], m = mv[k];
+      sgd_update(w, gp[k], m, h.lr, h.b1, h.wd, h.gscale, h.nesterov);
+      wv[k] = w; mv[k] = m;
+    }
+  }
+  __builtin_nontemporal_store(wv, (f32x4_t*)(oa.w + off));
+  __builtin_nontemporal_store(mv, (f32x4_t*)(oa.s0 + off));
+  __builtin_nontemporal_store(p8_u32x2_t{pack_bf2(wv[0], wv[1]), pack_bf2(wv[2], wv[3])},
+                              (p8_u32x2_t*)(oa.wb + off));
+}
+
+template <int BM, int BN, int WNW, int TI, int TJ, int J0 = 0, int NJ = TJ, bool APPLY = false>
 __device__ __forceinline__ void p8_epilogue(const P8Args& a, const Epi& ep, f32x4_t (&acc)[TI][TJ], char* smem,
                                             const int m0, const int n0, const int kz, const int wid,
-                                            const int lane) {
+                                            const int lane, const OptimApply* oa = nullptr) {
   using G = P8Geo<BM, BN, WNW>;
   const int wm = wid / WNW, wn = wid % WNW;
 
@@ -194,6 +227,18 @@
     constexpr int LDF = WTN + 4, CPR = WTN / 4;
     float* slab = (float*)(smem + wid * (32 * LDF * 4));
     float* cz = (float*)ep.c + (ep.mode == 3 ? kz * ep.zstride : 0);
+    OptimRec hyp{};
+    float ib1 = 0.f, ib2 = 0.f;
+    bool apply = false;
+    if constexpr (APPLY) {
+      if (ep.mode == P8_MODE_APPLY) {
+        hyp = *oa->rec;
+        if (hyp.guard != nullptr && *hyp.guard != 0u) return;
+        ib1 = 1.f / hyp.bc1;
+        ib2 = 1.f / hyp.bc2;
+        apply = true;
+      }
+    }
 #pragma unroll
     for (int h = 0; h < TI / 2; ++h) {
 #pragma unroll
@@ -216,6 +261,12 @@
         const float* src = slab + lr * LDF + ch * 4;
         if (col + 4 <= a.N) {
           float4 v = *(const float4*)src;
+          if constexpr (APPLY) {
+            if (apply) {
+              p8_apply4(*oa, hyp, ib1, ib2, dst - oa->g, v);
+              continue;
+            }
+          }
           if (ep.mode == 1) {
             const float4 o = *(const float4*)dst;
             v.x += o.x; v.y += o.y; v.z += o.z; v.w += o.w;
@@ -271,9 +322,10 @@
   n0 = ((bid % per_group) / gsize) * BN;
 }
 
-template <int BM, int BN, int WNW, bool AK, bool BK, int KS = 1>
+template <int BM, int BN, int WNW, bool AK, bool BK, int KS = 1, bool APPLY = false>
 __device__ __forceinline__ void gemm8p_body(const P8Args& a, const Epi& ep, const int bid, const int kz,
-                                            const int kt_lo = -1, const int kt_hi = -1) {
+                                            const int kt_lo = -1, const int kt_hi = -1,
+                                            const OptimApply* oa = nullptr) {
   using G = P8Geo<BM, BN, WNW>;
   constexpr bool FINE = true;
   constexpr int FI = G::FI, FJ = G::FJ, TI = 2 * FI, TJ = 2 * FJ;
@@ -395,7 +447,7 @@
     else p8_epilogue<BM, BN, WNW, TI, TJ, JH, JH>(a, ep, acc, smem_all + G::LDS, m0, n0, kz, wid, lane);
     return;
   }
-  p8_epilogue<BM, BN, WNW>(a, ep, acc, smem_all, m0, n0, kz, wid, lane);
+  p8_epilogue<BM, BN, WNW, TI, TJ, 0, TJ, APPLY>(a, ep, acc, smem_all, m0, n0, kz, wid, lane, oa);
 }
 
 template <int BM, int BN, int WNW, bool AK, bool BK>
diff --git a/csrc/include/tam/kernels.h b/csrc/include/tam/kernels.h
--- a/csrc/include/tam/kernels.h
+++ b/csrc/include/tam/kernels.h
@@ -84,15 +84,18 @@
 void cast_f32_bf16(const float* x, bf16_t* y, long n, hipStream_t s);
 
 void optim_grid(int blocks);
-void sgd_step(float* w, float* g, float* mom, bf16_t* wb, long n, float lr, float momentum,
+bool sgd_step(float* w, float* g, float* mom, bf16_t* wb, long n, float lr, float momentum,
               float wd, float gscale, int nesterov, int zero_grad, hipStream_t s,
               const unsigned* guard = nullptr, long zero_from = 0, long wd_until = -1,
-              const float* clip = nullptr);
+              const float* clip = nullptr, const long* skip = nullptr, int nskip = 0);
 void optim_variant(int v);
-void adam_step(float* w, float* g, float* m, float* v, bf16_t* wb, long n, float lr, float b1,
+bool adam_step(float* w, float* g, float* m, float* v, bf16_t* wb, long n, float lr, float b1,
                float b2, float eps, float wd, int step, float gscale, int zero_grad,
                hipStream_t s, const unsigned* guard = nullptr, long zero_from = 0, long wd_until = -1,
-               const float* clip = nullptr);
+               const float* clip = nullptr, const long* skip = nullptr, int nskip = 0);
+struct OptimRec;
+void optim_record(OptimRec* rec, float lr, float b1, float b2, float eps, float wd, int step, float gscale,
+                  int nesterov, const unsigned* guard, hipStream_t s);
 int grad_sumsq_blocks(long n);
 void grad_sumsq(const float* g, long n, double* partials, int slots, hipStream_t s);
 void grad_clip_finalize(const double* partials, int slots, float max_norm, float gscale, float* clip,
diff --git a/csrc/include/tam/launch.h b/csrc/include/tam/launch.h
--- a/csrc/include/tam/launch.h
+++ b/csrc/include/tam/launch.h
@@ -27,8 +27,11 @@
   float* bias;
   int M, N, K, lda, ldb;
   int mode = 1;
+  int fuse = 0;
 };
-void gemm_wgrad_grouped(const GGProblem* probs, int n, hipStream_t s);
+struct OptimApply;
+void gemm_wgrad_grouped(const GGProblem* probs, int n, hipStream_t s, const OptimApply* oa = nullptr,
+                        long arena_n = 0, int* fused = nullptr);
 void wgrad_slab_reduce_many(const float* const* ws, const int* sp, const long* mn, float* const* dw,
                             const int* mode, int n, hipStream_t s);
 bool gemm_wgrad_grouped_ok(int M, int N, int K, long lda, long ldb);
diff --git a/csrc/include/tam/optim_update.h b/csrc/include/tam/optim_update.h
--- /dev/null
+++ b/csrc/include/tam/optim_update.h
@@ -0,0 +1,73 @@
+#pragma once
+#include <cstdint>
+
+namespace tam {
+
+struct OptimRec {
+  float lr;
+  float b1;
+  float b2;
+  float eps;
+  float wd;
+  float bc1, bc2;
+  float gscale;
+  int nesterov;
+  int pad_;
+  const unsigned* guard;
+  uint64_t pad2_[2];
+};
+static_assert(sizeof(OptimRec) == 64, "OptimRec: 64 B");
+
+struct OptimApply {
+  const OptimRec* rec = nullptr;
+  const float* g = nullptr;
+  float* w = nullptr;
+  float* s0 = nullptr;
+  float* s1 = nullptr;
+  uint16_t* wb = nullptr;
+  int kind = 0;
+};
+
+inline int optim_split_skip(long n, const long* skip, int nskip, long* seg) {
+  long at = 0;
+  int ns = 0;
+  for (int i = 0; i < nskip; ++i) {
+    const long lo = skip[2 * i], hi = skip[2 * i + 1];
+    if (lo < at || hi < lo || hi > n || (lo & 3) != 0 || (hi & 3) != 0) return -1;
+    if (lo > at) {
+      seg[2 * ns] = at;
+      seg[2 * ns + 1] = lo;
+      ++ns;
+    }
+    at = hi;
+  }
+  if (at < n) {
+    seg[2 * ns] = at;
+    seg[2 * ns + 1] = n;
+    ++ns;
+  }
+  return ns;
+}
+
+#if defined(__HIPCC__)
+__device__ __forceinline__ void sgd_update(float& w, const float g, float& m, const float lr, const float momentum,
+                                           const float wd, const float gscale, const int nesterov) {
+  float d = __builtin_fmaf(wd, w, g * gscale);
+  m = __builtin_fmaf(momentum, m, d);
+  d = nesterov ? __builtin_fmaf(momentum, m, d) : m;
+  w = __builtin_fmaf(-lr, d, w);
+}
+
+__device__ __forceinline__ void adam_update(float& w, const float g, float& m, float& v, const float lr,
+                                            const float b1, const float b2, const float eps, const float wd,
+                                            const float ib1, const float ib2, const float gscale) {
+  const float gr = g * gscale;
+  m = __builtin_fmaf(b1, m, (1.f - b1) * gr);
+  v = __builtin_fmaf(b2, v, (1.f - b2) * gr * gr);
+  const float mh = m * ib1, vh = v * ib2;
+  const float u = __builtin_fmaf(wd, w, mh / (sqrtf(vh) + eps));
+  w = __builtin_fmaf(-lr, u, w);
+}
+#endif
+
+}
diff --git a/csrc/kernels/gemm_grouped.hip b/csrc/kernels/gemm_grouped.hip
--- a/csrc/kernels/gemm_grouped.hip
+++ b/csrc/kernels/gemm_grouped.hip
@@ -25,6 +25,7 @@
   P8GProb p[P8G_MAX];
   int n;
   int ncs;
+  OptimApply oa;
 };
 
 __device__ __forceinline__ void gg_colsum(const P8GProb& pr, int blk, float* red) {
@@ -95,7 +96,7 @@
   ep.ldc = pr.N;
   ep.c_f32 = 1;
   ep.mode = split ? 2 : pr.mode;
-  gemm8p_body<BM, BN, WNW, false, false>(a, ep, tile, kz);
+  gemm8p_body<BM, BN, WNW, false, false, 1, true>(a, ep, tile, kz, -1, -1, &g.oa);
 }
 
 static int g_gg_tile = [] {
@@ -119,10 +120,12 @@
   return cdiv(kt, sk);
 }
 
-void gemm_wgrad_grouped(const GGProblem* probs, int n, hipStream_t s) {
+void gemm_wgrad_grouped(const GGProblem* probs, int n, hipStream_t s, const OptimApply* oa, long arena_n,
+                        int* fused) {
   const int T = g_gg_tile == 128 ? 128 : 256;
   for (int base = 0; base < n; base += P8G_MAX) {
     P8Group g{};
+    if (oa) g.oa = *oa;
     const int m = n - base < P8G_MAX ? n - base : P8G_MAX;
     int tiles = 0, cs = 0;
     for (int i = 0; i < m; ++i) {
@@ -135,6 +138,13 @@
       p.c0 = cs;
       p.ntiles = cdiv(q.M, T) * cdiv(q.N, T);
       p.kps = gg_kps(q.K, q.mode);
+      bool fuse = false;
+      if (q.fuse && oa && oa->kind != 0 && oa->rec && q.mode == 0 && p.kps == q.K / P8_BK && (q.N & 3) == 0) {
+        const long off = q.C - oa->g;
+        fuse = q.C >= oa->g && (off & 3) == 0 && off + (long)q.M * q.N <= arena_n;
+      }
+      if (fuse) p.mode = P8_MODE_APPLY;
+      if (fused) fused[base + i] = fuse ? 1 : 0;
       tiles += p.ntiles * cdiv(q.K / P8_BK, p.kps);
       if (q.bias) cs += cdiv(q.M, 64);
     }
diff --git a/csrc/kernels/optim.hip b/csrc/kernels/optim.hip
--- a/csrc/kernels/optim.hip
+++ b/csrc/kernels/optim.hip
@@ -1,8 +1,10 @@
 #include <cmath>
 #include <cstdlib>
+#include <vector>
 
 #include "tam/common.h"
 #include "tam/kernels.h"
+#include "tam/optim_update.h"
 
 namespace tam {
 
@@ -26,12 +28,7 @@
     float* wp = (float*)&wv; float* gp = (float*)&gv; float* mp = (float*)&mv;
     const float wd = i < wd_until4 ? wd0 : 0.f;
 #pragma unroll
-    for (int k = 0; k < 4; ++k) {
-      float d = __builtin_fmaf(wd, wp[k], gp[k] * gscale);
-      mp[k] = __builtin_fmaf(momentum, mp[k], d);
-      d = nesterov ? __builtin_fmaf(momentum, mp[k], d) : mp[k];
-      wp[k] = __builtin_fmaf(-lr, d, wp[k]);
-    }
+    for (int k = 0; k < 4; ++k) sgd_update(wp[k], gp[k], mp[k], lr, momentum, wd, gscale, nesterov);
     ((float4*)w)[i] = wv;
     ((float4*)mom)[i] = mv;
     if (zero_grad && i >= zero_from4) ((float4*)g)[i] = make_float4(0.f, 0.f, 0.f, 0.f);
@@ -59,14 +56,7 @@
     float* wp = (float*)&wv; float* gp = (float*)&gv; float* mp = (float*)&mv; float* vp = (float*)&vv;
     const float wd = i < wd_until4 ? wd0 : 0.f;
 #pragma unroll
-    for (int k = 0; k < 4; ++k) {
-      const float gr = gp[k] * gscale;
-      mp[k] = __builtin_fmaf(b1, mp[k], (1.f - b1) * gr);
-      vp[k] = __builtin_fmaf(b2, vp[k], (1.f - b2) * gr * gr);
-      const float mh = mp[k] * ib1, vh = vp[k] * ib2;
-      const float u = __builtin_fmaf(wd, wp[k], mh / (sqrtf(vh) + eps));
-      wp[k] = __builtin_fmaf(-lr, u, wp[k]);
-    }
+    for (int k = 0; k < 4; ++k) adam_update(wp[k], gp[k], mp[k], vp[k], lr, b1, b2, eps, wd, ib1, ib2, gscale);
     ((float4*)w)[i] = wv; ((float4*)m)[i] = mv; ((float4*)v)[i] = vv;
     if (zero_grad && i >= zero_from4) ((float4*)g)[i] = make_float4(0.f, 0.f, 0.f, 0.f);
     ((uint2*)wb)[i] = make_uint2(pack_bf2(wp[0], wp[1]), pack_bf2(wp[2], wp[3]));
@@ -113,14 +103,7 @@
     float* wp = (float*)&wv; float* gp = (float*)&gv; float* mp = (float*)&mv; float* vp = (float*)&vv;
     const float wd = i < wd_until4 ? wd0 : 0.f;
 #pragma unroll
-    for (int k = 0; k < 4; ++k) {
-      const float gr = gp[k] * gscale;
-      mp[k] = __builtin_fmaf(b1, mp[k], (1.f - b1) * gr);
-      vp[k] = __builtin_fmaf(b2, vp[k], (1.f - b2) * gr * gr);
-      const float mh = mp[k] * ib1, vh = vp[k] * ib2;
-      const float u = __builtin_fmaf(wd, wp[k], mh / (sqrtf(vh) + eps));
-      wp[k] = __builtin_fmaf(-lr, u, wp[k]);
-    }
+    for (int k = 0; k < 4; ++k) adam_update(wp[k], gp[k], mp[k], vp[k], lr, b1, b2, eps, wd, ib1, ib2, gscale);
     st4<NT>(w, i, wv); st4<NT>(m, i, mv); st4<NT>(v, i, vv);
     if (zero_grad && i >= zero_from4) st4<NT>(g, i, make_float4(0.f, 0.f, 0.f, 0.f));
     st2<NT>(wb, i, make_uint2(pack_bf2(wp[0], wp[1]), pack_bf2(wp[2], wp[3])));
@@ -158,12 +141,7 @@
     float* wp = (float*)&wv; float* gp = (float*)&gv; float* mp = (float*)&mv;
     const float wd = i < wd_until4 ? wd0 : 0.f;
 #pragma unroll
-    for (int k = 0; k < 4; ++k) {
-      float d = __builtin_fmaf(wd, wp[k], gp[k] * gscale);
-      mp[k] = __builtin_fmaf(momentum, mp[k], d);
-      d = nesterov ? __builtin_fmaf(momentum, mp[k], d) : mp[k];
-      wp[k] = __builtin_fmaf(-lr, d, wp[k]);
-    }
+    for (int k = 0; k < 4; ++k) sgd_update(wp[k], gp[k], mp[k], lr, momentum, wd, gscale, nesterov);
     st4<NT>(w, i, wv); st4<NT>(mom, i, mv);
     if (zero_grad && i >= zero_from4) st4<NT>(g, i, make_float4(0.f, 0.f, 0.f, 0.f));
     st2<NT>(wb, i, make_uint2(pack_bf2(wp[0], wp[1]), pack_bf2(wp[2], wp[3])));
@@ -214,9 +192,9 @@
   return (int)(b < 1 ? 1 : b);
 }
 
-void sgd_step(float* w, float* g, float* mom, bf16_t* wb, long n, float lr, float momentum,
-              float wd, float gscale, int nesterov, int zero_grad, hipStream_t s, const unsigned* guard,
-              long zero_from, long wd_until, const float* clip) {
+static void sgd_launch(float* w, float* g, float* mom, bf16_t* wb, long n, float lr, float momentum, float wd,
+                       float gscale, int nesterov, int zero_grad, hipStream_t s, const unsigned* guard,
+                       long zero_from, long wd_until, const float* clip) {
   const dim3 grid(ogrid(n / 4));
   const long zf4 = zero_from / 4, wu4 = wd_until < 0 ? n / 4 : wd_until / 4;
   switch (optim_pick(n / 4, false)) {
@@ -230,10 +208,9 @@
   }
 }
 
-void adam_step(float* w, float* g, float* m, float* v, bf16_t* wb, long n, float lr, float b1,
-               float b2, float eps, float wd, int step, float gscale, int zero_grad,
-               hipStream_t s, const unsigned* guard, long zero_from, long wd_until, const float* clip) {
-  const float bc1 = 1.f - powf(b1, (float)step), bc2 = 1.f - powf(b2, (float)step);
+static void adam_launch(float* w, float* g, float* m, float* v, bf16_t* wb, long n, float lr, float b1, float b2,
+                        float eps, float wd, float bc1, float bc2, float gscale, int zero_grad, hipStream_t s,
+                        const unsigned* guard, long zero_from, long wd_until, const float* clip) {
   const dim3 grid(ogrid(n / 4));
   const long zf4 = zero_from / 4, wu4 = wd_until < 0 ? n / 4 : wd_until / 4;
   switch (optim_pick(n / 4, true)) {
@@ -245,6 +222,65 @@
       hipLaunchKernelGGL(adam_kernel, grid, dim3(256), 0, s, w, g, m, v, wb, n / 4, lr, b1, b2, eps, wd, bc1, bc2,
                          gscale, zero_grad, guard, zf4, wu4, clip);
   }
+}
+
+template <typename F>
+static bool for_segments(long n, long zero_from, long wd_until, const long* skip, int nskip, F&& launch) {
+  if (nskip <= 0) {
+    launch(0L, n, zero_from, wd_until);
+    return true;
+  }
+  std::vector<long> seg(2 * (size_t)(nskip + 1));
+  const int ns = optim_split_skip(n, skip, nskip, seg.data());
+  if (ns < 0) return false;
+  const long wu = wd_until < 0 ? n : wd_until;
+  for (int j = 0; j < ns; ++j) {
+    const long lo = seg[2 * j], hi = seg[2 * j + 1];
+    const long zf = zero_from > lo ? zero_from - lo : 0;
+    const long wuj = wu > lo ? (wu < hi ? wu : hi) - lo : 0;
+    launch(lo, hi - lo, zf, wuj);
+  }
+  return true;
+}
+
+bool sgd_step(float* w, float* g, float* mom, bf16_t* wb, long n, float lr, float momentum,
+              float wd, float gscale, int nesterov, int zero_grad, hipStream_t s, const unsigned* guard,
+              long zero_from, long wd_until, const float* clip, const long* skip, int nskip) {
+  return for_segments(n, zero_from, wd_until, skip, nskip, [&](long lo, long len, long zf, long wu) {
+    sgd_launch(w + lo, g + lo, mom + lo, wb + lo, len, lr, momentum, wd, gscale, nesterov, zero_grad, s, guard, zf,
+               wu, clip);
+  });
+}
+
+static void adam_bias_corr(float b1, float b2, int step, float& bc1, float& bc2) {
+  bc1 = 1.f - powf(b1, (float)step);
+  bc2 = 1.f - powf(b2, (float)step);
+}
+
+bool adam_step(float* w, float* g, float* m, float* v, bf16_t* wb, long n, float lr, float b1,
+               float b2, float eps, float wd, int step, float gscale, int zero_grad,
+               hipStream_t s, const unsigned* guard, long zero_from, long wd_until, const float* clip,
+               const long* skip, int nskip) {
+  float bc1, bc2;
+  adam_bias_corr(b1, b2, step, bc1, bc2);
+  return for_segments(n, zero_from, wd_until, skip, nskip, [&](long lo, long len, long zf, long wu) {
+    adam_launch(w + lo, g + lo, m + lo, v + lo, wb + lo, len, lr, b1, b2, eps, wd, bc1, bc2, gscale, zero_grad, s,
+                guard, zf, wu, clip);
+  });
+}
+
+__global__ void optim_record_kernel(OptimRec* rec, OptimRec v) {
+  if (threadIdx.x == 0 && blockIdx.x == 0) *rec = v;
+}
+
+void optim_record(OptimRec* rec, float lr, float b1, float b2, float eps, float wd, int step, float gscale,
+                  int nesterov, const unsigned* guard, hipStream_t s) {
+  OptimRec v{};
+  v.lr = lr; v.b1 = b1; v.b2 = b2; v.eps = eps; v.wd = wd; v.gscale = gscale;
+  v.nesterov = nesterov;
+  v.guard = guard;
+  adam_bias_corr(b1, b2, step, v.bc1, v.bc2);
+  hipLaunchKernelGGL(optim_record_kernel, dim3(1), dim3(64), 0, s, rec, v);
 }
 
 template <int U>
diff --git a/csrc/sanitize/optim_skip_sanitize_main.cpp b/csrc/sanitize/optim_skip_sanitize_main.cpp
--- /dev/null
+++ b/csrc/sanitize/optim_skip_sanitize_main.cpp
@@ -0,0 +1,78 @@
+#include <cstdio>
+#include <cstdlib>
+#include <vector>
+
+#include "tam/optim_update.h"
+
+namespace {
+int errors = 0;
+
+void expect(bool ok, const char* what) {
+  if (!ok) {
+    std::fprintf(stderr, "FAIL: %s\n", what);
+    ++errors;
+  }
+}
+
+void check(long n, const std::vector<long>& skip) {
+  const int nskip = (int)(skip.size() / 2);
+  std::vector<long> seg(2 * (size_t)(nskip + 1));
+  const int ns = tam::optim_split_skip(n, skip.data(), nskip, seg.data());
+  expect(ns >= 0 && ns <= nskip + 1, "segment count");
+  if (ns < 0) return;
+  std::vector<char> cover((size_t)n, 0);
+  for (int i = 0; i < nskip; ++i)
+    for (long e = skip[2 * i]; e < skip[2 * i + 1]; ++e) cover[(size_t)e] += 1;
+  long prev = 0;
+  for (int j = 0; j < ns; ++j) {
+    expect(seg[2 * j] >= prev && seg[2 * j] < seg[2 * j + 1] && seg[2 * j + 1] <= n, "segment order / bounds");
+    expect((seg[2 * j] & 3) == 0 && (seg[2 * j + 1] & 3) == 0, "segment alignment");
+    prev = seg[2 * j + 1];
+    for (long e = seg[2 * j]; e < seg[2 * j + 1]; ++e) cover[(size_t)e] += 2;
+  }
+  for (long e = 0; e < n; ++e)
+    if (cover[(size_t)e] != 1 && cover[(size_t)e] != 2) {
+      expect(false, "every element in exactly one skip range or one segment");
+      break;
+    }
+}
+}
+
+int main() {
+  check(64, {});
+  check(64, {0, 64});
+  check(256, {0, 64});
+  check(256, {192, 256});
+  check(256, {64, 128, 128, 192});
+  check(4096, {4, 8, 100, 200, 4000, 4092});
+  check(128, {64, 64});
+  unsigned long long s = 0x9e3779b97f4a7c15ULL;
+  auto rnd = [&]() { s = s * 6364136223846793005ULL + 1442695040888963407ULL; return (unsigned)(s >> 33); };
+  for (int it = 0; it < 2000; ++it) {
+    const long n = 4 * (1 + rnd() % 512);
+    std::vector<long> skip;
+    long at = 0;
+    while (at < n && rnd() % 4 != 0) {
+      const long lo = at + 4 * (rnd() % 8), hi = lo + 4 * (rnd() % 16);
+      if (hi > n) break;
+      skip.push_back(lo);
+      skip.push_back(hi);
+      at = hi;
+    }
+    check(n, skip);
+  }
+  long seg[8] = {-7, -7, -7, -7, -7, -7, -7, -7};
+  const long unsorted[4] = {128, 192, 0, 64}, overlap[4] = {0, 128, 64, 192}, past[2] = {0, 512},
+             odd[2] = {2, 64}, rev[2] = {64, 32};
+  expect(tam::optim_split_skip(256, unsorted, 2, seg) == -1, "unsorted refused");
+  expect(tam::optim_split_skip(256, overlap, 2, seg) == -1, "overlap refused");
+  expect(tam::optim_split_skip(256, past, 1, seg) == -1, "range past the arena refused");
+  expect(tam::optim_split_skip(256, odd, 1, seg) == -1, "unaligned refused");
+  expect(tam::optim_split_skip(256, rev, 1, seg) == -1, "reversed refused");
+  if (errors) {
+    std::fprintf(stderr, "optim_skip_sanitize: %d error(s)\n", errors);
+    return 1;
+  }
+  std::printf("optim_skip_sanitize ok\n");
+  return 0;
+}
diff --git a/tiresias_amd/executor/trainer.py b/tiresias_amd/executor/trainer.py
--- a/tiresias_amd/executor/trainer.py
+++ b/tiresias_amd/executor/trainer.py
@@ -9,7 +9,7 @@
 from ..models import MODELS, make_model, samples_per_batch, synthetic_batch
 from ..ops import _lib
 from ..ops import functional as Fx
-from ..ops.arena import Arena
+from ..ops.arena import Arena, optim_epilogue_ok
 from ..parallel.ddp import GradBucketer
 from ..parallel.gang import comm_size
 
@@ -58,6 +58,10 @@
         self._graph = None
         self._g_loss = None
         self._g_written = []
+        self._opt_rec = None
+        self._rec_step = -1
+        self._fused: List[int] = []
+        self._g_fused: List[int] = []
         self._warm = 0
         self.capture_s = 0.0
         self._side = None
@@ -94,6 +98,10 @@
         group = (self.device.type == "cuda" and self.ddp is None and self.group_wgrad)
         if group:
             Fx.defer_wgrad(True)
+        fuse = group and self._fuse_ok() and self._rec_step == self.step_count + 1
+        self._fused = []
+        if fuse:
+            Fx.set_optim_epilogue(self._opt_rec, self.arena, self.opt_state)
         try:
             if self.spec.kind == "image":
                 logits = self.model.forward(d["x"])
@@ -106,9 +114,18 @@
                                          labels_time_major=getattr(self.model, "logits_time_major", False))
             logits.backward(dlog)
             if group:
+                if fuse and nb:
+                    for s in self._bs:
+                        torch.cuda.current_stream(self.device).wait_stream(s)
+                if fuse:
+                    Fx.final_flush()
                 Fx.flush_wgrad()
                 self._defer_n = Fx.deferred_count()
+                if fuse:
+                    self._fused = self.arena.epilogue_ranges(Fx.fused_params())
         finally:
+            if fuse:
+                Fx.set_optim_epilogue(None)
             if group:
                 Fx.defer_wgrad(False, discard=True)
             Fx.set_wgrad_stream(None)
@@ -119,6 +136,27 @@
             for s in self._bs:
                 torch.cuda.current_stream(self.device).wait_stream(s)
         return loss
+
+    def _fuse_ok(self) -> bool:
+        return (self.device.type == "cuda" and self.group_wgrad
+                and optim_epilogue_ok(self.ddp, self.ddp_shard and self.ddp is not None, self.grad_clip,
+                                      Fx.OPTIM_EPILOGUE))
+
+    def _opt_hyper(self):
+        return (0.9, 0.0, 0.0) if self.opt == "sgd" else (0.9, 0.98, 1e-9)
+
+    def _write_opt_record(self) -> None:
+        if not self._fuse_ok():
+            return
+        if self._graph is not None and not self._g_fused:
+            return
+        if self._opt_rec is None:
+            self._opt_rec = torch.zeros(16, dtype=torch.int64, device=self.device)
+        b1, b2, eps = self._opt_hyper()
+        guard = self.model.err if self.uses_persist else None
+        _lib.ops().optim_record(self._opt_rec, self.lr, b1, b2, eps, self.spec.wd, self.step_count + 1, 1.0, False,
+                                guard)
+        self._rec_step = self.step_count + 1
 
     def set_grad_clip(self, v: Optional[float]) -> None:
         if v is not None:
@@ -133,6 +171,9 @@
                 self._clip = torch.zeros(4, dtype=torch.float32, device=self.device)
                 self._clip_part = torch.zeros(int(T.grad_sumsq_blocks(self.arena.numel)), dtype=torch.float64,
                                               device=self.device)
+        if (v is None) != (self.grad_clip is None):
+            self._graph = None
+            self._g_loss = None
         self.grad_clip = v
 
     def _clip_launch(self, gscale: float):
@@ -176,12 +217,14 @@
             guard = self.model.err if self.uses_persist else None
             zf = A.n_store if Fx.STORE_GRAD else 0
             clip = self._clip_launch(gscale)
+            skip = self._fused or None
+            self._fused = []
             if self.opt == "sgd":
                 T.sgd_step(A.master, A.grad, self.opt_state[0], A.shadow, self.lr, 0.9, self.spec.wd, gscale, False,
-                           True, guard, zf, A.n_decay, clip)
+                           True, guard, zf, A.n_decay, clip, skip)
             else:
                 T.adam_step(A.master, A.grad, self.opt_state[0], self.opt_state[1], A.shadow, self.lr, 0.9, 0.98,
-                            1e-9, self.spec.wd, self.step_count, gscale, True, guard, zf, A.n_decay, clip)
+                            1e-9, self.spec.wd, self.step_count, gscale, True, guard, zf, A.n_decay, clip, skip)
             if self.uses_persist:
                 _lib.ops().lstm_guard_step(self.model.err)
             return
@@ -274,12 +317,14 @@
             self._side = s
             s.wait_stream(torch.cuda.current_stream(self.device))
             with torch.cuda.stream(s):
+                self._write_opt_record()
                 loss = self._fwd_bwd()
                 self._opt_step()
             torch.cuda.current_stream(self.device).wait_stream(s)
             self._warm += 1
             self.last_loss = loss
             return loss
+        self._write_opt_record()
         if self.use_graph:
             loss = self._graph_step()
         else:
@@ -309,7 +354,9 @@
             self.capture_s += time.perf_counter() - tc
             A = self.arena
             self._g_written = [p for p in A.params if p.store_grad and p.gw_epoch == A.grad_epoch]
+            self._g_fused = list(self._fused)
         self._graph.replay()
+        self._fused = list(self._g_fused)
         for p in self._g_written:
             p.gw_epoch = self.arena.grad_epoch
         return self._g_loss
diff --git a/tiresias_amd/ops/arena.py b/tiresias_amd/ops/arena.py
--- a/tiresias_amd/ops/arena.py
+++ b/tiresias_amd/ops/arena.py
@@ -50,6 +50,10 @@
     return (n + _ALIGN - 1) // _ALIGN * _ALIGN
 
 
+def optim_epilogue_ok(ddp, ddp_shard: bool, grad_clip, enabled: bool = True) -> bool:
+    return bool(enabled) and ddp is None and not ddp_shard and grad_clip is None
+
+
 class Arena:
     def __init__(self, device: torch.device | str = "cpu", seed: int = 0):
         self.device = torch.device(device)
@@ -89,6 +93,18 @@
                 self.n_store = off
         self.numel = max(off, _ALIGN)
         return order
+
+    def epilogue_ranges(self, params: Sequence[Param]) -> List[int]:
+        spans = sorted((p.offset, p.offset + _padded(p.numel)) for p in params if p.store_grad and p.arena is self)
+        out: List[int] = []
+        for lo, hi in spans:
+            if hi > self.n_store:
+                raise ValueError(f"store_grad param range [{lo}, {hi}) outside the store region [0, {self.n_store})")
+            if out and lo <= out[-1]:
+                out[-1] = max(out[-1], hi)
+            else:
+                out += [lo, hi]
+        return out
 
     def materialize(self) -> "Arena":
         order = self.layout()
diff --git a/tiresias_amd/ops/functional.py b/tiresias_amd/ops/functional.py
--- a/tiresias_amd/ops/functional.py
+++ b/tiresias_amd/ops/functional.py
@@ -107,7 +107,31 @@
         flush_wgrad()
 
 
+OPTIM_EPILOGUE = os.environ.get("TAM_OPTIM_EPILOGUE", "1") != "0"
+_APPLY = None
+_FUSED: List[Param] = []
+_FINAL = False
+
+
+def set_optim_epilogue(rec, arena=None, opt_state=None) -> None:
+    global _APPLY, _FINAL
+    _APPLY = (rec, arena, list(opt_state)) if rec is not None else None
+    _FINAL = False
+    _FUSED.clear()
+
+
+def final_flush() -> None:
+    global _FINAL
+    _FINAL = True
+
+
+def fused_params() -> List[Param]:
+    return list(_FUSED)
+
+
 def flush_wgrad() -> int:
+    global _FINAL
+    final, _FINAL = _FINAL, False
     if _DEFER_LNRED:
         lnr = list(_DEFER_LNRED)
         _DEFER_LNRED.clear()
@@ -124,9 +148,21 @@
     dys = [it[0] for it in items]
     with _OnWgrad(*dys, *[it[1] for it in items]):
         empty = torch.empty(0, dtype=torch.float32, device=dys[0].device)
-        _T().gemm_wgrad_grouped(dys, [it[1] for it in items], [it[5] if len(it) > 5 else it[2].grad for it in items],
-                                [it[3].grad if it[3] is not None else empty for it in items],
-                                [it[4] for it in items])
+        xs = [it[1] for it in items]
+        dws = [it[5] if len(it) > 5 else it[2].grad for it in items]
+        dbs = [it[3].grad if it[3] is not None else empty for it in items]
+        modes = [it[4] for it in items]
+        fuse = []
+        if final and _APPLY is not None:
+            fuse = [int(it[2].store_grad and it[4] == 0 and len(it) <= 5 and it[2].arena is _APPLY[1])
+                    for it in items]
+        if any(fuse):
+            rec, A, st = _APPLY
+            done = _T().gemm_wgrad_grouped_apply(dys, xs, dws, dbs, modes, fuse, rec, A.grad, A.master, st[0],
+                                                 st[1] if len(st) > 1 else None, A.shadow)
+            _FUSED.extend(it[2] for it, f in zip(items, done) if f)
+        else:
+            _T().gemm_wgrad_grouped(dys, xs, dws, dbs, modes)
     for it in items:
         it[2].grad_ready()
         if it[3] is not None:
```

Measured after the change: 0.1350. No clear change (+0.5%).
